# yunhao-qian/Othello-AlphaZero

Hardware: AMD Instinct MI355X
Metric: MCTS simulations/sec (whole node), 800 sims/move, 128x10b ResNet, 1/2/4/8 GPU (higher is better)
Workload: dtype bf16

## Files before the change

### include/othello_mcts_amd_experimental.h

```cpp
#ifndef OTHELLO_MCTS_AMD_EXPERIMENTAL_H
#define OTHELLO_MCTS_AMD_EXPERIMENTAL_H

#include "othello_mcts_amd.h"

#ifdef __cplusplus
extern "C" {
#endif

int oamd_engine_set_pipeline(oamd_engine *e, int32_t groups);
int oamd_engine_set_nn_chains(oamd_engine *e, int32_t chains);
int oamd_engine_set_chain_split(oamd_engine *e, int32_t budget, int32_t cuts);
int oamd_engine_set_adaptive_extra_rounds(oamd_engine *e, int32_t enable, int32_t min_rounds);
int oamd_engine_set_extra_round_grid(oamd_engine *e, int32_t workgroups);
int oamd_debug_read_stamps(uint64_t *out, int64_t n);
int oamd_debug_tree_stamps(uint64_t *out, int64_t n, int32_t reset);

int oamd_engine_set_free_running(oamd_engine *e, int32_t enable);

int oamd_engine_tree_work(oamd_engine *e, int64_t *levels, int64_t *children_scanned, int64_t *expansions,
                          int64_t *children_created, int64_t *launches);

int oamd_solve_endgames_grid(int32_t device, const oamd_position *pos_dev, int64_t n, int32_t max_empties,
                             int64_t node_limit, int32_t *move_scores_dev, int32_t *score_dev,
                             int32_t *best_action_dev, int32_t *flags_dev, int64_t *nodes_dev,
                             void *workspace_dev, int32_t workgroups, void *stream);

#ifdef __cplusplus
}
#endif

#endif
```

### othello-alphazero_amd/build.py

```python

from __future__ import annotations

import argparse
import concurrent.futures as cf
import os
import subprocess
import sys
import sysconfig
from pathlib import Path

HERE = Path(__file__).resolve().parent
CSRC = HERE / "csrc"
PKG = HERE / "othello_mcts"
INCLUDE = HERE.parent / "include"
BUILD = HERE / "build"
HIPCC = os.environ.get("HIPCC", "/opt/rocm/bin/hipcc")
ARCH = os.environ.get("OAMD_ARCH", "gfx950")

COMMON = ["-O3", "-std=c++17", "-fPIC", f"--offload-arch={ARCH}", "-I", str(CSRC), "-I", str(INCLUDE),
          "-Wall", "-Wno-unused-function", "-fno-gpu-rdc", *os.environ.get("OAMD_EXTRA_FLAGS", "").split()]
EXACT = ["-ffp-contract=off", "-fno-fast-math"]
NO_SCALAR_LOADS = ["-mllvm", "-amdgpu-scalarize-global-loads=false"]
UNITS = {
    "tree.hip": EXACT + NO_SCALAR_LOADS,
    "capi.hip": EXACT,
    "replay.hip": EXACT,
    "resnet.hip": os.environ.get("OAMD_RESNET_FLAGS",
                                 "-mllvm -amdgpu-mfma-vgpr-form=1 -mllvm -amdgpu-sched-strategy=max-ilp").split()
    + ["-Rpass-analysis=kernel-resource-usage"],
    "solver.hip": ["-Rpass-analysis=kernel-resource-usage"],
}


W8_VGPR_LIMIT = 208


def run(cmd: list[str]) -> None:
    r = subprocess.run(cmd, capture_output=True, text=True)
    if r.returncode != 0:
        sys.stderr.write(" ".join(cmd) + "\n" + r.stdout + r.stderr)
        raise SystemExit(f"build failed: {cmd[-1]}")
    if "kernel-resource-usage" in " ".join(cmd):
        unit = next((u for u in RESOURCE_CHECKS if str(CSRC / u) in cmd), None)
        if unit:
            RESOURCE_CHECKS[unit](r.stderr)
    elif r.stderr.strip():
        sys.stderr.write(r.stderr)


def kernel_remarks(remarks: str):
    name = None
    for ln in remarks.splitlines():
        if "Function Name:" in ln:
            name = ln.split("Function Name:")[1].split()[0]
        elif name and "remark:" in ln and ":" in ln.split("remark:")[1]:
            field, _, value = ln.split("remark:")[1].split("[-Rpass")[0].rpartition(":")
            yield name, field.strip(), value.strip()


def check_solver_scratch(remarks: str) -> None:
    seen = 0
    for name, field, value in kernel_remarks(remarks):
        if "k_solve" in name and "reduce" not in name and field.startswith("ScratchSize"):
            seen += 1
            if int(value.split()[0]) != 0:
                raise SystemExit(f"build failed: {name} uses {value} bytes of scratch per lane: "
                                 "the solver's stacks must stay in LDS")
    if not seen:
        raise SystemExit("build failed: no resource remark for k_solve in solver.hip")


def check_w8_vgprs(remarks: str) -> None:
    name = None
    seen = 0
    for ln in remarks.splitlines():
        if "Function Name:" in ln:
            name = ln.split("Function Name:")[1].split()[0]
        elif name and "k_resnet_w8" in name and " VGPRs:" in ln:
            v = int(ln.split("VGPRs:")[1].split()[0])
            seen += 1
            if (v + 7) // 8 * 8 > W8_VGPR_LIMIT and os.environ.get("OAMD_W8_VGPR_CHECK", "1") != "0":
                raise SystemExit(f"build failed: {name} uses {v} VGPRs (> {W8_VGPR_LIMIT}): "
                                 "k_select could no longer co-reside with the ResNet kernel")
    if not seen:
        sys.stderr.write("note: no k_resnet_w8 kernel in this build\n")


RESOURCE_CHECKS = {"resnet.hip": check_w8_vgprs, "solver.hip": check_solver_scratch}


def newer(out: Path, deps: list[Path]) -> bool:
    return out.exists() and all(out.stat().st_mtime >= d.stat().st_mtime for d in deps)


def source_hash_defines() -> list[str]:
    sys.path.insert(0, str(PKG))
    try:
        import provenance
    finally:
        sys.path.pop(0)
    return [f'-DOAMD_SOURCE_HASH_{k.upper()}="{provenance.source_hash(k)}"' for k in provenance.FAMILIES]


def build(jobs: int = 4, force: bool = False) -> None:
    BUILD.mkdir(exist_ok=True)
    headers = list(CSRC.glob("*.h")) + [INCLUDE / "othello_mcts_amd.h", INCLUDE / "othello_mcts_amd_experimental.h"]
    hashes = source_hash_defines()
    objs = []
    todo = []
    all_srcs = [CSRC / u for u in UNITS] + headers
    for unit, extra in UNITS.items():
        src = CSRC / unit
        obj = BUILD / (unit + ".o")
        objs.append(obj)
        deps = all_srcs if unit == "capi.hip" else [src, *headers]
        if force or not newer(obj, [*deps, Path(__file__)]):
            todo.append([HIPCC, *COMMON, *extra, *(hashes if unit == "capi.hip" else []), "-c", str(src),
                         "-o", str(obj)])
    with cf.ThreadPoolExecutor(max_workers=max(1, jobs)) as ex:
        list(ex.map(run, todo))
    lib = PKG / "liboamd.so"
    if force or todo or not lib.exists():
        run([HIPCC, f"--offload-arch={ARCH}", "-shared", "-fPIC", "-o", str(lib), *map(str, objs)])

    import pybind11

    ext = sysconfig.get_config_var("EXT_SUFFIX")
    mod = PKG / f"_othello_mcts_impl{ext}"
    src = CSRC / "pybind_module.cpp"
    if force or not newer(mod, [src, *headers, lib, Path(__file__)]):
        run(["g++", "-O2", "-std=c++17", "-fPIC", "-shared", "-Wall", "-fvisibility=hidden",
             "-I", pybind11.get_include(), "-I", sysconfig.get_paths()["include"], "-I", str(INCLUDE),
             str(src), "-o", str(mod), "-L", str(PKG), "-loamd", "-Wl,-rpath,$ORIGIN"])


if __name__ == "__main__":
    ap = argparse.ArgumentParser()
    ap.add_argument("-j", "--jobs", type=int, default=4)
    ap.add_argument("--force", action="store_true")
    a = ap.parse_args()
    build(a.jobs, a.force)
    print("built", *sorted(p.name for p in PKG.glob("*.so")))
```

### othello-alphazero_amd/csrc/capi.hip

```cpp

#include <hip/hip_runtime.h>

#include <algorithm>
#include <chrono>
#include <cmath>
#include <cstdio>
#include <cstdlib>
#include <cstring>
#include <string>
#include <thread>
#include <vector>

#include "../../include/othello_mcts_amd.h"
#include "../../include/othello_mcts_amd_experimental.h"
#include "bitboard.h"

#include "engine.h"
#include "kernels.h"
#include "replay.h"
#include "schedule.h"
#include "solver.h"
#include "timing.h"

using namespace oamd;
// ... 12 lines not shown
    if (spin_sync()) return hipEventSynchronize(ev);
    for (;;) {
        const hipError_t q = hipEventQuery(ev);
        if (q != hipErrorNotReady) return q;
        std::this_thread::sleep_for(std::chrono::microseconds(100));
    }
}
constexpr int kEvPerBlock = 4;
constexpr int kCounters = 12;

namespace {

thread_local std::string g_err;

int fail(int code, const std::string& msg) {
    g_err = msg;
    return code;
}

#define HIPCHK(expr)                                                                  \
    do {                                                                              \
        hipError_t _e = (expr);                                                       \
        if (_e != hipSuccess)                                                         \
            return fail(OAMD_RUNTIME, std::string(#expr) + ": " + hipGetErrorString(_e)); \
    } while (0)

#define LAUNCHCHK()                                                                       \
    do {                                                                                  \
        hipError_t _e = hipGetLastError();                                                \
        if (_e != hipSuccess) return fail(OAMD_RUNTIME, std::string("kernel launch: ") + hipGetErrorString(_e)); \
    } while (0)

struct DeviceGuard {
    int prev = -1;
    explicit DeviceGuard(int dev) {
        if (hipGetDevice(&prev) != hipSuccess) prev = -1;
        if (prev != dev) (void)hipSetDevice(dev);
    }
    ~DeviceGuard() {
        if (prev >= 0) (void)hipSetDevice(prev);
    }
};

template <typename T>
int dalloc(T** p, size_t n) {
    *p = nullptr;
    if (n == 0) return OAMD_OK;
    hipError_t e = hipMalloc(reinterpret_cast<void**>(p), n * sizeof(T));
    if (e != hipSuccess) return fail(OAMD_RUNTIME, std::string("hipMalloc: ") + hipGetErrorString(e));
    return OAMD_OK;
}

template <typename T>
void dfree(T*& p) {
    if (p) (void)hipFree(p);
    p = nullptr;
}

struct ReadbackSlots {
    static constexpr int kSlots = 4;
    int32_t* dev = nullptr;
    int32_t* host = nullptr;
    hipEvent_t ev[kSlots][kMaxPipeline] = {};
    int ensure(size_t dev_words, size_t host_words, const char* what) {
        if (dev) return OAMD_OK;
        ReadbackSlots t;
        int rc = dalloc(&t.dev, dev_words);
        if (!rc && hipHostMalloc((void**)&t.host, sizeof(int32_t) * host_words) != hipSuccess)
            rc = fail(OAMD_RUNTIME, std::string(what) + ": hipHostMalloc failed");
        for (auto& row : t.ev)
            for (auto& x : row)
                if (!rc && hipEventCreateWithFlags(&x, readback_event_flags()) != hipSuccess)
                    rc = fail(OAMD_RUNTIME, std::string(what) + ": hipEventCreate failed");
        if (rc) t.release();
        else *this = t;
        return rc;
    }
    void release() {
        for (auto& row : ev)
            for (auto x : row)
                if (x) (void)hipEventDestroy(x);
        if (host) (void)hipHostFree(host);
        dfree(dev);
    }
    void destroy() {
        if (!dev) return;
        (void)hipDeviceSynchronize();
        release();
    }
};

std::string fstr(float v) { return std::to_string(v); }

int validate_config(const oamd_search_config* c) {
    if (c->history_size < 1)
        return fail(OAMD_INVALID_ARGUMENT,
                    "Expected history_size >= 1, but got " + std::to_string(c->history_size) + ".");
    if (c->history_size > kMaxHistory)
        return fail(OAMD_INVALID_ARGUMENT, "Expected history_size <= 15 (native engine limit), but got " +
                                               std::to_string(c->history_size) + ".");
    if (c->num_simulations < 1)
        return fail(OAMD_INVALID_ARGUMENT, "Expected num_simulations >= 1, but got " +
                                               std::to_string(c->num_simulations) + ".");
    if (c->num_threads < 1)
        return fail(OAMD_INVALID_ARGUMENT,
                    "Expected num_threads >= 1, but got " + std::to_string(c->num_threads) + ".");
    if (c->batch_size < 1)
        return fail(OAMD_INVALID_ARGUMENT,
                    "Expected batch_size >= 1, but got " + std::to_string(c->batch_size) + ".");
    if ((int64_t)c->num_threads * c->batch_size > kMaxLeaves)
        return fail(OAMD_INVALID_ARGUMENT,
                    "Expected num_threads * batch_size <= 1024 (native engine limit), but got " +
                        std::to_string((int64_t)c->num_threads * c->batch_size) + ".");
    if (!(c->c_puct_base > 0.0f))
        return fail(OAMD_INVALID_ARGUMENT, "Expected c_puct_base > 0.0, but got " + fstr(c->c_puct_base) + ".");
    if (!(c->c_puct_init >= 0.0f))
        return fail(OAMD_INVALID_ARGUMENT, "Expected c_puct_init >= 0.0, but got " + fstr(c->c_puct_init) + ".");
    if (!(0.0f <= c->dirichlet_epsilon && c->dirichlet_epsilon <= 1.0f))
        return fail(OAMD_INVALID_ARGUMENT, "Expected 0.0 <= dirichlet_epsilon <= 1.0, but got " +
                                               fstr(c->dirichlet_epsilon) + ".");
    if (!(c->dirichlet_alpha >= 0.0f))
        return fail(OAMD_INVALID_ARGUMENT,
                    "Expected dirichlet_alpha >= 0.0, but got " + fstr(c->dirichlet_alpha) + ".");
    return OAMD_OK;
}

}

struct oamd_engine {
    int device = 0;
    int G = 0;
    int64_t cap = 0;
    oamd_search_config cfg{};
    hipStream_t stream = nullptr;
    uint64_t seed = 0;

    NodeLink* link = nullptr;
    NodeStat* stat = nullptr;
    NodePos* pos = nullptr;
    GameState* games = nullptr;
    int64_t rows_cap = 0;
    int fw_cap = 0;
    int32_t* leaf = nullptr;
    int32_t* depth = nullptr;
    int32_t* trans = nullptr;
    int32_t* path = nullptr;
    uint64_t* feat = nullptr;
    float* policy = nullptr;
    float* value = nullptr;
    uint8_t* flags = nullptr;
    int32_t* rowlist = nullptr;
    int32_t* rowcount = nullptr;
    int32_t* tstate = nullptr;
    float* explore_tab = nullptr;
    unsigned long long* counters = nullptr;
    int32_t* status_dev = nullptr;
    oamd_root_info* info_dev = nullptr;
    int32_t* visits_dev = nullptr;
    float* q_dev = nullptr;
    float* spd_dev = nullptr;
    int steps_left = 0;
    int steps_total = 0;
    bool exact_interleaving = true;
    int chain_budget = 2;
    int chain_cuts = 64;
    static constexpr int kCutSlots = ReadbackSlots::kSlots;
    AdaptiveRounds adapt;
    int64_t adapt_seq = 0;
    ReadbackSlots cuts;
    int cut_x[kCutSlots] = {-1, -1, -1, -1};
    int cut_groups[kCutSlots] = {};
    bool free_running = true;
    bool throttle_enqueue = !spin_sync();
    static constexpr int kFreeSlots = ReadbackSlots::kSlots;
    static constexpr int kFreeTailRounds = 4;
    ReadbackSlots remaining;
    int ensure_remaining() {
        return remaining.ensure((size_t)kMaxPipeline, (size_t)kFreeSlots * kMaxPipeline, "free-running slots");
    }
    int extra_grid = 128;
    int step_phase = 0;
    int pipeline = 0;
    int nn_batch = 0;
    int n_pipe_streams = 0;
    int n_events = 0;
    hipStream_t pipe_stream[kMaxPipeline] = {};
    hipEvent_t fork_ev = nullptr;
    static constexpr int kMaxChains = 4;
    hipEvent_t nn_token[kMaxChains] = {};
    int nn_chains = 2;
    hipStream_t idle_stream = nullptr;
    hipEvent_t sel_ev[kMaxPipeline] = {};
    hipEvent_t join_ev[kMaxPipeline] = {};
    bool timing = false;
    int timing_stride = 1;
    int64_t search_count = 0;
    std::vector<hipEvent_t> ev[2];
    int ev_blocks[2] = {0, 0};
    int ev_final[2] = {0, 0};
    int64_t ev_launches[2] = {0, 0};
    int64_t ev_rows[2] = {0, 0};
    static constexpr int64_t kSpanChunk = 1 << 15;
    static constexpr int64_t kSpanWindow = 1 << 23;
    struct SpanChunk {
        unsigned long long* p = nullptr;
        int64_t cap = 0, used = 0;
    };
    std::vector<SpanChunk> span_chunks;
    int64_t span_slots = 0;
    int64_t span_dropped = 0;
    size_t span_copied = 0;
    std::vector<std::pair<long long, long long>> span_ticks;
    int ev_cur = 0;
    float nn_ms = 0.0f;
    float select_ms = 0.0f;
    float backup_ms = 0.0f;
    int64_t nn_launches = 0;
    int64_t tree_launches = 0;
    int64_t tree_final_launches = 0;
    int64_t grouped_searches = 0, grouped_rounds = 0;
    int64_t nn_rows = 0;

    int resolve_timing(int p) {
        const int n = ev_blocks[p];
        if (!n) return OAMD_OK;
        for (int i = 0; i < n; ++i) {
            const hipEvent_t* b = &ev[p][kEvPerBlock * i];
            float ms = 0.0f;
            const bool nn = i < ev_final[p];
            HIPCHK(hipEventSynchronize(b[1]));
            if (nn) HIPCHK(hipEventSynchronize(b[3]));
            HIPCHK(hipEventElapsedTime(&ms, b[0], b[1]));
            (i < ev_final[p] ? select_ms : backup_ms) += ms;
            if (nn) {
                HIPCHK(hipEventElapsedTime(&ms, b[2], b[3]));
                nn_ms += ms;
            }
        }

        nn_launches += ev_launches[p];
        tree_launches += ev_final[p];
        tree_final_launches += n - ev_final[p];
        nn_rows += ev_rows[p];
        ev_blocks[p] = 0;
        return OAMD_OK;
    }
    int resolve_all_timing() {
        int rc = resolve_timing(ev_cur ^ 1);
        return rc ? rc : resolve_timing(ev_cur);
    }
    int reserve_spans(int64_t n, unsigned long long** out) {
        *out = nullptr;
        if (!timing || n <= 0) return OAMD_OK;
        if (span_slots + n > kSpanWindow) {
            span_dropped += n;
            return OAMD_OK;
        }
        if (span_chunks.empty() || span_chunks.back().used + n > span_chunks.back().cap) {
            SpanChunk c;
            c.cap = std::max(kSpanChunk, n);
            if (int rc = dalloc(&c.p, (size_t)2 * c.cap)) return rc;
            if (hipMemset(c.p, 0, sizeof(unsigned long long) * 2 * c.cap) != hipSuccess) {
                dfree(c.p);
                return fail(OAMD_RUNTIME, "span window: hipMemset failed");
            }
            span_chunks.push_back(c);
        }
        SpanChunk& c = span_chunks.back();
        *out = c.p + 2 * c.used;
        c.used += n;
        span_slots += n;
        return OAMD_OK;
    }
    int reset_spans() {
        if (span_chunks.empty() && !span_dropped) return OAMD_OK;
        HIPCHK(hipDeviceSynchronize());
        for (auto& c : span_chunks) dfree(c.p);
        span_chunks.clear();
        span_slots = span_dropped = 0;
        span_copied = 0;
        span_ticks.clear();
        return OAMD_OK;
    }
    int span_intervals(std::vector<std::pair<long long, long long>>* iv) {
        HIPCHK(hipDeviceSynchronize());
        auto read = [&](const SpanChunk& c, std::vector<std::pair<long long, long long>>* to) -> int {
            std::vector<unsigned long long> sp((size_t)2 * c.used);
            if (c.used)
                HIPCHK(hipMemcpy(sp.data(), c.p, sizeof(unsigned long long) * 2 * c.used, hipMemcpyDeviceToHost));
            for (int64_t i = 0; i < c.used; ++i)
                if (sp[2 * i + 1]) to->emplace_back((long long)~sp[2 * i], (long long)sp[2 * i + 1]);
            return OAMD_OK;
        };
        for (; span_copied + 1 < span_chunks.size(); ++span_copied) {
            if (int rc = read(span_chunks[span_copied], &span_ticks)) return rc;
            dfree(span_chunks[span_copied].p);
        }
        *iv = span_ticks;
        if (!span_chunks.empty())
            if (int rc = read(span_chunks.back(), iv)) return rc;
        return OAMD_OK;
    }

    int L() const { return cfg.num_threads * cfg.batch_size; }
    int steps() const { return search_steps(cfg.num_simulations, L()); }
    bool thread_split() const {
        static const bool v = [] {
            const char* e = getenv("OAMD_TREE_SPLIT");
            return e ? atoi(e) != 0 : true;
        }();
        return v && thread_split_shape(G, cfg.num_threads);
    }
    int ensure_streams(int K, int nev) {
        if (K <= 1 && nev <= 1) return OAMD_OK;
        if (!fork_ev) HIPCHK(hipEventCreateWithFlags(&fork_ev, hipEventDisableTiming));
        for (int c = 0; c < kMaxChains; ++c)
            if (!nn_token[c]) HIPCHK(hipEventCreateWithFlags(&nn_token[c], hipEventDisableTiming));
        if (!idle_stream) HIPCHK(hipStreamCreateWithFlags(&idle_stream, hipStreamNonBlocking));
        while (n_pipe_streams < K) {
            const int k = n_pipe_streams;
            HIPCHK(hipStreamCreateWithFlags(&pipe_stream[k], hipStreamNonBlocking));
            HIPCHK(hipEventCreateWithFlags(&join_ev[k], hipEventDisableTiming));
            ++n_pipe_streams;
        }
        while (n_events < nev) {
            const int k = n_events;
            HIPCHK(hipEventCreateWithFlags(&sel_ev[k], hipEventDisableTiming | hipEventDisableSystemFence));
            ++n_events;
        }
        return OAMD_OK;
    }
    int FW() const { return feature_words(cfg.history_size); }

    EngineView view() const {
        EngineView E;
        E.G = G;
        E.L = L();
        E.H = cfg.history_size;
        E.FW = FW();
        E.cap = cap;
        E.link = link;
        E.stat = stat;
        E.pos = pos;
        E.games = games;
        E.leaf = leaf;
        E.depth = depth;
        E.trans = trans;
        E.path = path;
        E.feat = feat;
        E.policy = policy;
        E.value = value;
        E.explore_tab = explore_tab;
        E.c_base = cfg.c_puct_base;
        E.c_init = cfg.c_puct_init;
        E.eps = cfg.dirichlet_epsilon;
        E.alpha = cfg.dirichlet_alpha;
        E.counters = counters;
        E.rowlist = rowlist;
        E.tstate = tstate;
        E.steps = steps();
        E.B = cfg.batch_size;
        E.terminal_skip = exact_interleaving ? 1 : 0;
        return E;
    }

    int alloc_rows() {
        const int64_t rows = (int64_t)G * L();
        const int fw = FW();
        if (rows <= rows_cap && fw <= fw_cap) return OAMD_OK;
        dfree(leaf);
        dfree(depth);
        dfree(trans);
        dfree(path);
        dfree(feat);
        dfree(policy);
        dfree(value);
        dfree(flags);
        dfree(rowlist);
        dfree(tstate);
        int rc;
        if ((rc = dalloc(&leaf, rows)) || (rc = dalloc(&depth, rows)) || (rc = dalloc(&trans, rows)) ||
            (rc = dalloc(&path, rows * kMaxDepth)) || (rc = dalloc(&feat, rows * fw)) ||
            (rc = dalloc(&policy, rows * 65)) || (rc = dalloc(&value, rows)) || (rc = dalloc(&flags, rows)) ||
            (rc = dalloc(&rowlist, rows)) || (rc = dalloc(&tstate, rows)))
            return rc;
        HIPCHK(hipMemset(policy, 0, rows * 65 * sizeof(float)));
        HIPCHK(hipMemset(value, 0, rows * sizeof(float)));
        rows_cap = rows;
        fw_cap = fw;
        return OAMD_OK;
    }

    int build_tables() {
        std::vector<float> ex(kExploreTab);
        for (int n = 0; n < kExploreTab; ++n)
            ex[n] = std::log(((float)(1 + n) + cfg.c_puct_base) / cfg.c_puct_base) + cfg.c_puct_init;
        HIPCHK(hipMemcpy(explore_tab, ex.data(), ex.size() * sizeof(float), hipMemcpyHostToDevice));
        return OAMD_OK;
    }

    ~oamd_engine() {
        DeviceGuard dg(device);
        dfree(link);
        dfree(stat);
        dfree(pos);
        dfree(games);
        dfree(leaf);
        dfree(depth);
        dfree(trans);
        dfree(path);
        dfree(feat);
        dfree(policy);
        dfree(value);
        dfree(flags);
        dfree(rowlist);
        dfree(tstate);
        dfree(rowcount);
        dfree(explore_tab);
        dfree(counters);
        dfree(status_dev);
        dfree(info_dev);
        dfree(visits_dev);
        dfree(q_dev);
        dfree(spd_dev);
        for (auto& pool : ev)
            for (auto e : pool) (void)hipEventDestroy(e);
        for (auto& c : span_chunks) dfree(c.p);
        cuts.destroy();
        remaining.destroy();
        for (int k = 0; k < n_pipe_streams; ++k) {
            (void)hipStreamDestroy(pipe_stream[k]);
            (void)hipEventDestroy(join_ev[k]);
        }
        for (int k = 0; k < n_events; ++k) (void)hipEventDestroy(sel_ev[k]);
        if (fork_ev) (void)hipEventDestroy(fork_ev);
        for (int c = 0; c < kMaxChains; ++c)
            if (nn_token[c]) (void)hipEventDestroy(nn_token[c]);
        if (idle_stream) (void)hipStreamDestroy(idle_stream);
    }
};

struct oamd_net {
    int device = 0;
    oamd_net_desc desc{};
    uint16_t* w = nullptr;
    float* bias = nullptr;
    float* head = nullptr;
    uint16_t* hconv = nullptr;
    bool loaded = false;
    std::vector<std::string> keys;
    std::vector<int64_t> numel;

    NetView view() const {
        NetView N;
        N.cin = desc.in_channels;
        N.C = desc.conv_channels;
        N.R = desc.num_residual_blocks;
        N.hidden = desc.value_head_hidden_channels;
        N.dtype = desc.dtype;
        N.w = w;
        N.bias = bias;
        N.head = head;
        N.hconv = hconv;
        return N;
    }
    ~oamd_net() {
        DeviceGuard dg(device);
        dfree(w);
        dfree(bias);
        dfree(head);
        dfree(hconv);
    }
};

extern "C" {

const char* oamd_last_error(void) { return g_err.c_str(); }
int oamd_abi_version(void) { return OAMD_ABI_VERSION; }

#ifndef OAMD_SOURCE_HASH_ALL
#define OAMD_SOURCE_HASH_ALL "unknown"
#define OAMD_SOURCE_HASH_RESNET "unknown"
#define OAMD_SOURCE_HASH_TREE "unknown"
#endif
const char* oamd_source_hash(const char* family) {
    if (!family) return nullptr;
    if (!std::strcmp(family, "all")) return OAMD_SOURCE_HASH_ALL;
    if (!std::strcmp(family, "resnet")) return OAMD_SOURCE_HASH_RESNET;
    if (!std::strcmp(family, "tree")) return OAMD_SOURCE_HASH_TREE;
    return nullptr;
}

int oamd_device_count(int32_t* out) {
    int n = 0;
    if (hipGetDeviceCount(&n) != hipSuccess) n = 0;
    *out = n;
    return OAMD_OK;
}

int oamd_get_legal_moves(const uint64_t* me, const uint64_t* opp, uint64_t* out, int64_t n, void* stream) {
    if (n < 0) return fail(OAMD_INVALID_ARGUMENT, "n must be >= 0");
    launch_legal_moves(me, opp, out, n, (hipStream_t)stream);
    LAUNCHCHK();
    return OAMD_OK;
}

int oamd_get_flips(const uint64_t* mv, const uint64_t* me, const uint64_t* opp, uint64_t* out, int64_t n,
                   void* stream) {
    if (n < 0) return fail(OAMD_INVALID_ARGUMENT, "n must be >= 0");
    launch_flips(mv, me, opp, out, n, (hipStream_t)stream);
    LAUNCHCHK();
    return OAMD_OK;
}

int oamd_apply_action(const oamd_position* in, const int32_t* actions, oamd_position* out, int64_t n,
                      void* stream) {
    static_assert(sizeof(oamd_position) == sizeof(Pos), "layout");
    if (n < 0) return fail(OAMD_INVALID_ARGUMENT, "n must be >= 0");
    launch_apply_positions(reinterpret_cast<const Pos*>(in), actions, reinterpret_cast<Pos*>(out), n,
                           (hipStream_t)stream);
    LAUNCHCHK();
    return OAMD_OK;
}

int oamd_initial_position(oamd_position* out) {
    const Pos p = initial_position();
    std::memcpy(out, &p, sizeof(Pos));
    return OAMD_OK;
}

uint64_t oamd_host_legal_moves(uint64_t me, uint64_t opp) { return legal_moves(me, opp); }
uint64_t oamd_host_flips(uint64_t mv, uint64_t me, uint64_t opp) { return flips(mv, me, opp); }
void oamd_host_apply_action(const oamd_position* in, int32_t action, oamd_position* out) {
    Pos p;
    std::memcpy(&p, in, sizeof(Pos));
    const Pos c = apply_action(p, action);
    std::memcpy(out, &c, sizeof(Pos));
}

int oamd_net_create(int32_t device, const oamd_net_desc* d, oamd_net** out) {
    *out = nullptr;
    if (d->in_channels < 1 || d->in_channels > 31)
        return fail(OAMD_INVALID_ARGUMENT, "in_channels must be in [1, 31], got " + std::to_string(d->in_channels));
    if (d->conv_channels != 128 && d->conv_channels != 256)
        return fail(OAMD_INVALID_ARGUMENT,
                    "conv_channels must be 128 or 256 for the native net, got " + std::to_string(d->conv_channels));
    if (d->num_residual_blocks < 0)
        return fail(OAMD_INVALID_ARGUMENT, "num_residual_blocks must be >= 0");
    if (d->value_head_hidden_channels < 1 || d->value_head_hidden_channels > 1024)
        return fail(OAMD_INVALID_ARGUMENT, "value_head_hidden_channels must be in [1, 1024] for the native net, got " +
                                               std::to_string(d->value_head_hidden_channels));
    if (d->num_squares != 64 || d->num_actions != 65)
        return fail(OAMD_INVALID_ARGUMENT, "num_squares must be 64 and num_actions 65");
    if (d->dtype != OAMD_BF16 && d->dtype != OAMD_FP16)
        return fail(OAMD_INVALID_ARGUMENT, "dtype must be OAMD_BF16 or OAMD_FP16");
    int n = 0;
    if (hipGetDeviceCount(&n) != hipSuccess || n == 0) return fail(OAMD_RUNTIME, "no HIP device available");
    if (device < 0 || device >= n) return fail(OAMD_INVALID_ARGUMENT, "bad device ordinal");
    DeviceGuard dg(device);
    auto* net = new oamd_net();
    net->device = device;
    net->desc = *d;
    const int C = d->conv_channels, R = d->num_residual_blocks, hid = d->value_head_hidden_channels;
    int rc;
    if ((rc = dalloc(&net->w, resnet_packed_weight_alloc_elems(C, R))) ||
        (rc = dalloc(&net->bias, (size_t)(1 + 2 * R) * C)) ||
        (rc = dalloc(&net->head, resnet_head_floats(C, hid))) ||
        (rc = dalloc(&net->hconv, resnet_hconv_elems(C)))) {
        delete net;
        return rc;
    }
    auto conv = [&](const std::string& p, int64_t cout, int64_t cin, int64_t k) {
        net->keys.push_back(p + ".weight");
        net->numel.push_back(cout * cin * k * k);
        net->keys.push_back(p + ".bias");
        net->numel.push_back(cout);
    };
    auto bn = [&](const std::string& p, int64_t c) {
        for (const char* s : {".weight", ".bias", ".running_mean", ".running_var"}) {
            net->keys.push_back(p + s);
            net->numel.push_back(c);
        }
    };
    auto lin = [&](const std::string& p, int64_t fin, int64_t fout) {
        net->keys.push_back(p + ".weight");
        net->numel.push_back(fin * fout);
        net->keys.push_back(p + ".bias");
        net->numel.push_back(fout);
    };
    conv("conv_block.conv", C, d->in_channels, 3);
    bn("conv_block.norm", C);
    for (int i = 0; i < R; ++i) {
        const std::string p = "residual_blocks." + std::to_string(i);
        conv(p + ".conv1", C, C, 3);
        bn(p + ".norm1", C);
        conv(p + ".conv2", C, C, 3);
        bn(p + ".norm2", C);
    }
    conv("policy_head.conv", 2, C, 1);
    bn("policy_head.norm", 2);
    lin("policy_head.linear", 128, 65);
    conv("value_head.conv", 1, C, 1);
    bn("value_head.norm", 1);
    lin("value_head.linear1", 64, hid);
    lin("value_head.linear2", hid, 1);
    *out = net;
    return OAMD_OK;
}

int oamd_net_destroy(oamd_net* net) {
    delete net;
    return OAMD_OK;
}

int oamd_net_state_size(const oamd_net* net, int32_t* n) {
    *n = (int32_t)net->keys.size();
    return OAMD_OK;
}

int oamd_net_state_key(const oamd_net* net, int32_t i, const char** key, int64_t* numel) {
    if (i < 0 || i >= (int32_t)net->keys.size()) return fail(OAMD_OUT_OF_RANGE, "state index out of range");
    *key = net->keys[i].c_str();
    *numel = net->numel[i];
    return OAMD_OK;
}

static uint16_t f32_to_bf16_rne(float f) {
    uint32_t u;
    std::memcpy(&u, &f, 4);
    if ((u & 0x7fffffffu) > 0x7f800000u) return (uint16_t)((u >> 16) | 0x40);
    u += 0x7fffu + ((u >> 16) & 1u);
    return (uint16_t)(u >> 16);
}

static uint16_t f32_to_f16(float f) {
    _Float16 h = (_Float16)f;
    uint16_t u;
    std::memcpy(&u, &h, 2);
    return u;
}

int oamd_net_load_state(oamd_net* net, const float* const* t, int32_t n_tensors) {
    if (n_tensors != (int32_t)net->keys.size())
        return fail(OAMD_INVALID_ARGUMENT, "expected " + std::to_string(net->keys.size()) + " tensors, got " +
                                               std::to_string(n_tensors));
    const auto& d = net->desc;
    const int C = d.conv_channels, R = d.num_residual_blocks, hid = d.value_head_hidden_channels;
    const double eps = 1e-5;
    int ti = 0;
    std::vector<uint16_t> packed(resnet_packed_weight_elems(C, R));
    std::vector<float> bias((size_t)(1 + 2 * R) * C);
    size_t ks_global = 0;
    auto pack_conv = [&](int layer, int cin, bool first) {
        const float* W = t[ti++];
        const float* b = t[ti++];
        const float* g = t[ti++];
        const float* be = t[ti++];
        const float* mu = t[ti++];
        const float* var = t[ti++];
        std::vector<double> scale(C);
        for (int n = 0; n < C; ++n) {
            scale[n] = (double)g[n] / std::sqrt((double)var[n] + eps);
            bias[(size_t)layer * C + n] = (float)(((double)b[n] - (double)mu[n]) * scale[n] + (double)be[n]);
        }
        const int nk = resnet_ksteps(C, first);
        for (int i = 0; i < nk; ++i) {
            int tap, cb;
            bool pad;
            resnet_kstep(C, first, i, &tap, &cb, &pad);
            const size_t ks = ks_global + (size_t)i;
            for (int nt = 0; nt < C / 16; ++nt)
                for (int lane = 0; lane < 64; ++lane)
                    for (int j = 0; j < 8; ++j) {
                        const int ci = cb * 32 + 8 * resnet_kgroup_chunk(lane >> 4) + j;
                        const int n = resnet_out_channel(nt, lane & 15);
                        double v = 0.0;
                        if (!pad && ci < cin) v = (double)W[((size_t)n * cin + ci) * 9 + tap] * scale[n];
                        const size_t idx = (((ks * (C / 16) + nt) * 64) + lane) * 8 + j;
                        packed[idx] = d.dtype == OAMD_BF16 ? f32_to_bf16_rne((float)v) : f32_to_f16((float)v);
                    }
        }
        ks_global += (size_t)nk;
    };
    pack_conv(0, d.in_channels, true);
    for (int i = 0; i < R; ++i) {
        pack_conv(1 + 2 * i, C, false);
        pack_conv(2 + 2 * i, C, false);
    }
    std::vector<float> head(resnet_head_floats(C, hid));
    const int HL_pcw = 0, HL_pcb = HL_pcw + 2 * C, HL_vcw = HL_pcb + 2, HL_vcb = HL_vcw + C,
// ... 235 lines not shown
    if (rows) *rows = e->nn_rows;
    return OAMD_OK;
}

int oamd_engine_nn_busy(const oamd_engine* ce, float* busy_ms, int64_t* launches) {
    oamd_engine* e = const_cast<oamd_engine*>(ce);
    DeviceGuard dg(e->device);
    if (e->span_dropped)
        return fail(OAMD_RUNTIME, "nn_busy: the timing window outgrew its " + std::to_string(oamd_engine::kSpanWindow) +
                                      " slots; " + std::to_string(e->span_dropped) +
                                      " launches were not recorded (restart it with oamd_engine_enable_timing)");
    std::vector<std::pair<long long, long long>> iv;
    if (int rc = e->span_intervals(&iv)) return rc;
    if (busy_ms) *busy_ms = (float)(interval_union(iv) * 1e-5);
    if (launches) *launches = (int64_t)iv.size();
    return OAMD_OK;
}

int oamd_engine_tree_timing(const oamd_engine* ce, float* select_ms, float* backup_ms, int64_t* launches) {
    oamd_engine* e = const_cast<oamd_engine*>(ce);
    if (int rc = e->resolve_all_timing()) return rc;
    if (select_ms) *select_ms = e->select_ms;
    if (backup_ms) *backup_ms = e->backup_ms;
    if (launches) *launches = e->tree_launches;
    return OAMD_OK;
}

struct GroupPlan : GroupSplit {
    hipStream_t st[kMaxPipeline] = {};
    int max_launches = 1;
    int64_t round_launches = 0, round_rows = 0;
};

static int native_search_checks(const oamd_engine* e, const oamd_net* net) {
    if (!net || !net->loaded) return fail(OAMD_INVALID_ARGUMENT, "native net not loaded");
    if (net->device != e->device) return fail(OAMD_INVALID_ARGUMENT, "net and engine on different devices");
    if (net->desc.in_channels != 1 + 2 * e->cfg.history_size)
        return fail(OAMD_INVALID_ARGUMENT, "net in_channels != 1 + 2 * history_size");
    return OAMD_OK;
}

static GroupPlan plan_groups(oamd_engine* e) {
    GroupPlan P;
    static_cast<GroupSplit&>(P) = split_groups(e->G, e->pipeline);
    for (int k = 0; k < P.K; ++k) {
        P.st[k] = P.K == 1 ? e->stream : e->pipe_stream[k];
        const int n = group_launches(P.ng[k], e->L(), e->nn_batch);
        P.max_launches = std::max(P.max_launches, n);
        P.round_launches += n;
        P.round_rows += (int64_t)P.ng[k] * e->L();
    }
    return P;
}

static int extra_rounds(const oamd_engine* e) {
    return extra_round_cap(e->exact_interleaving, e->chain_budget, e->chain_cuts, e->cfg.num_threads, e->steps());
}

static int pick_extra_rounds(oamd_engine* e, int* X) {
    const int cap = extra_rounds(e);
    *X = cap;
    if (cap == 0 || !e->adapt.on) return OAMD_OK;
    if (int rc = e->cuts.ensure((size_t)2 * oamd_engine::kCutSlots * kMaxPipeline,
                                (size_t)2 * oamd_engine::kCutSlots * kMaxPipeline, "cut slots"))
        return rc;
    const int64_t q = e->adapt_seq - 2;
    const int s = q >= 0 ? (int)(q % oamd_engine::kCutSlots) : 0;
    if (q >= 0 && e->cut_x[s] >= 0) {
        int used = 0, empties = 64;
        for (int k = 0; k < e->cut_groups[s]; ++k) {
            HIPCHK(host_wait(e->cuts.ev[s][k]));
            used = std::max(used, (int)e->cuts.host[2 * (s * kMaxPipeline + k)]);
            empties = std::min(empties, (int)e->cuts.host[2 * (s * kMaxPipeline + k) + 1]);
        }
        e->adapt.observe(e->cut_x[s], used, empties, e->chain_cuts);
        static const bool plog = getenv("OAMD_ADAPT_LOG") != nullptr;
        if (plog)
            fprintf(stderr, "adapt search %lld X %d used %d empties %d\n", (long long)q, e->cut_x[s], used, empties);
        e->cut_x[s] = -1;
    }
    *X = e->adapt.pick(cap);
    return OAMD_OK;
}

static int timing_begin(oamd_engine* e, int steps, int NB, bool* timed) {
    *timed = e->timing && (e->search_count++ % e->timing_stride) == 0;
    if (!*timed) return OAMD_OK;
    const int pool = e->ev_cur;
    if (int rc = e->resolve_timing(pool)) return rc;

    while ((int)e->ev[pool].size() < kEvPerBlock * (steps + 1) * NB) {
        hipEvent_t x;
        HIPCHK(hipEventCreate(&x));
        e->ev[pool].push_back(x);
    }
    return OAMD_OK;
}

static void timing_end(oamd_engine* e, int blocks, int first_final, int NB, int64_t round_launches,
                       int64_t round_rows) {
    const int pool = e->ev_cur;
    e->ev_blocks[pool] = blocks;
    e->ev_final[pool] = first_final;
    e->ev_launches[pool] = first_final / NB * round_launches;
    e->ev_rows[pool] = first_final / NB * round_rows;
    e->ev_cur ^= 1;
}
static void timing_end_search(oamd_engine* e, int rounds, const GroupPlan& P) {
    timing_end(e, (rounds + 1) * P.K, rounds * P.K, P.K, P.round_launches, P.round_rows);
}

static int enqueue_group_nn(oamd_engine* e, const EngineView& E, const NetView& N, const GroupPlan& P, int k,
                            bool wait_token, hipEvent_t* ev, int* count, unsigned long long* span, int max_wgs) {
    hipStream_t sk = P.st[k];
    hipEvent_t token = e->nn_token[k % std::min(e->nn_chains, P.K)];
    if (P.K > 1 && wait_token) HIPCHK(hipStreamWaitEvent(sk, token, 0));
    if (ev) HIPCHK(hipEventRecord(ev[2], sk));
    const int grows = P.ng[k] * E.L, cb = launch_rows(grows, e->nn_batch);
    const size_t r0 = (size_t)P.g0[k] * E.L;
    for (int r = 0, j = 0; r < grows; r += cb, ++j)
        launch_resnet_packed(N, E.feat, E.FW, E.H, std::min(cb, grows - r), E.policy, E.value, sk, E.rowlist + r0 + r,
                             count, r, span ? span + (size_t)2 * j : nullptr, max_wgs);
    if (ev) HIPCHK(hipEventRecord(ev[3], sk));
    if (P.K > 1) HIPCHK(hipEventRecord(token, sk));
    return OAMD_OK;
}

static int enqueue_group_rounds(oamd_engine* e, const NetView& N, const GroupPlan& P, int steps, int X, bool timed,
                                bool chained) {
    const EngineView E = e->view();
    const int K = P.K;
    const int T = e->cfg.num_threads, B = e->cfg.batch_size;
    const int pool = e->ev_cur;
    const bool splitting = extra_rounds(e) > 0;
    const int budget = splitting ? e->chain_budget : 0;
    const int S = steps + X;
    const bool adapt = splitting && e->adapt.on;
    const int cs = (int)(e->adapt_seq % oamd_engine::kCutSlots);
    ++e->grouped_searches;
    e->grouped_rounds += S;
    if (adapt) {
        e->cut_x[cs] = X;
        e->cut_groups[cs] = K;
        ++e->adapt_seq;
    }
    const int nlg = P.max_launches;
    unsigned long long* span = nullptr;
    if (int rc = e->reserve_spans((int64_t)K * S * nlg, &span)) return rc;
    for (int s = 0; s <= S; ++s) {
        for (int k = 0; k < K; ++k) {
            hipStream_t sk = P.st[k];
            hipEvent_t* ev = timed ? &e->ev[pool][kEvPerBlock * (s * K + k)] : nullptr;
            if (ev) HIPCHK(hipEventRecord(ev[0], sk));
            int* cnt = e->rowcount + 2 * k;
            int* cuts = adapt ? e->cuts.dev + 2 * (cs * kMaxPipeline + k) : nullptr;
            launch_tree(E, sk, s > 0, s < S, T, B, P.g0[k], P.ng[k], 0, -1, s < S ? cnt + (s & 1) : nullptr,
                        s < S ? cnt + ((s + 1) & 1) : cnt, s == 0, budget, X, timed,
                        s == 0 || s == S ? cuts : nullptr);
            if (ev) HIPCHK(hipEventRecord(ev[1], sk));
            if (s == S) {
                if (adapt) {
                    HIPCHK(hipMemcpyAsync(e->cuts.host + 2 * (cs * kMaxPipeline + k), cuts, 2 * sizeof(int32_t),
                                          hipMemcpyDeviceToHost, sk));
                    HIPCHK(hipEventRecord(e->cuts.ev[cs][k], sk));
                }
                continue;
            }
            const bool first = s == 0 && k < std::min(e->nn_chains, K) && !chained;
            if (int rc = enqueue_group_nn(e, E, N, P, k, !first, ev, cnt + (s & 1),
                                          span ? span + (size_t)2 * ((k * S + s) * nlg) : nullptr,
                                          s >= steps ? e->extra_grid : 0))
                return rc;
        }
    }
    return OAMD_OK;
}

static int fork_streams(oamd_engine* e, const hipStream_t* st, int n) {
    if (n > 1) {
        HIPCHK(hipEventRecord(e->fork_ev, e->stream));
        for (int k = 0; k < n; ++k) HIPCHK(hipStreamWaitEvent(st[k], e->fork_ev, 0));
    }
    return OAMD_OK;
}
static int join_streams(oamd_engine* e, const hipStream_t* st, int n) {
    for (int k = 0; n > 1 && k < n; ++k) {
        HIPCHK(hipEventRecord(e->join_ev[k], st[k]));
        HIPCHK(hipStreamWaitEvent(e->stream, e->join_ev[k], 0));
    }
    return OAMD_OK;
}
static int fork_groups(oamd_engine* e, const GroupPlan& P) { return fork_streams(e, P.st, P.K); }
static int join_groups(oamd_engine* e, const GroupPlan& P) { return join_streams(e, P.st, P.K); }

static int search_thread_split(oamd_engine* e, const NetView& N) {
    const EngineView E = e->view();
    const int steps = e->steps();
    const int T = e->cfg.num_threads, B = e->cfg.batch_size;
    if (int rc = e->ensure_streams(T, T)) return rc;
    bool timed = false;
    if (int rc = timing_begin(e, steps, T, &timed)) return rc;
    const int pool = e->ev_cur;
    unsigned long long* span = nullptr;
    if (int rc = e->reserve_spans((int64_t)T * steps, &span)) return rc;
    if (int rc = fork_streams(e, e->pipe_stream, T)) return rc;
    for (int s = 0; s <= steps; ++s) {
        for (int t = 0; t < T; ++t) {
            hipEvent_t* ev = timed ? &e->ev[pool][kEvPerBlock * (s * T + t)] : nullptr;
            hipStream_t ts = e->pipe_stream[t];
            if (s > 0 || t > 0)
                HIPCHK(hipStreamWaitEvent(ts, e->sel_ev[t > 0 ? t - 1 : T - 1], 0));
            if (ev) HIPCHK(hipEventRecord(ev[0], ts));
            launch_tree(E, ts, s > 0, s < steps, T, B, 0, 1, t, t + 1, nullptr, nullptr, s == 0, 0, 0, timed);
            if (ev) HIPCHK(hipEventRecord(ev[1], ts));
            HIPCHK(hipEventRecord(e->sel_ev[t], ts));
            if (s == steps) continue;
            if (ev) HIPCHK(hipEventRecord(ev[2], ts));
            launch_resnet_packed(N, E.feat + (size_t)t * B * E.FW, E.FW, E.H, B, E.policy + (size_t)t * B * 65,
                                 E.value + (size_t)t * B, ts, nullptr, nullptr, 0,
                                 span ? span + (size_t)2 * (t * steps + s) : nullptr);
            if (ev) HIPCHK(hipEventRecord(ev[3], ts));
        }
    }
    if (int rc = join_streams(e, e->pipe_stream, T)) return rc;
    LAUNCHCHK();
    if (timed) timing_end(e, (steps + 1) * T, steps * T, T, T, e->L());
    return OAMD_OK;
}

static int search_grouped(oamd_engine* e, const NetView& N) {
    const int K = plan_groups(e).K;
    if (int rc = e->ensure_streams(K, K)) return rc;
    const GroupPlan P = plan_groups(e);
    bool timed = false;
    int X = 0;
    if (int rc = pick_extra_rounds(e, &X)) return rc;
    const int steps = e->steps();
    if (int rc = timing_begin(e, steps + X, K, &timed)) return rc;
    if (int rc = fork_groups(e, P)) return rc;
    if (int rc = enqueue_group_rounds(e, N, P, steps, X, timed, false)) return rc;
    LAUNCHCHK();
    if (int rc = join_groups(e, P)) return rc;
    if (timed) timing_end_search(e, steps + X, P);
    return OAMD_OK;
}

int oamd_engine_search(oamd_engine* e, oamd_net* net, int64_t* sims, int64_t* evals) {
    if (int rc = native_search_checks(e, net)) return rc;
    DeviceGuard dg(e->device);
    if (sims || evals) HIPCHK(hipMemsetAsync(e->counters, 0, 2 * sizeof(unsigned long long), e->stream));
    const NetView N = net->view();
    if (int rc = e->thread_split() ? search_thread_split(e, N) : search_grouped(e, N)) return rc;
    if (sims || evals) {
        unsigned long long c[2] = {0, 0};
        HIPCHK(hipMemcpyAsync(c, e->counters, sizeof(c), hipMemcpyDeviceToHost, e->stream));
        HIPCHK(hipStreamSynchronize(e->stream));
        if (sims) *sims = (int64_t)c[0];
        if (evals) *evals = (int64_t)c[1];
    }
    e->step_phase = 0;
    e->steps_left = 0;
    return OAMD_OK;
}

int oamd_engine_work_counters(oamd_engine* e, int64_t* sims, int64_t* evals) {
    DeviceGuard dg(e->device);
    unsigned long long c[2] = {0, 0};
    HIPCHK(hipMemcpyAsync(c, e->counters + 2, sizeof(c), hipMemcpyDeviceToHost, e->stream));
    HIPCHK(hipStreamSynchronize(e->stream));
    if (sims) *sims = (int64_t)c[0];
    if (evals) *evals = (int64_t)c[1];
    return OAMD_OK;
}

int oamd_engine_descent_depths(oamd_engine* e, int64_t* leaves, int64_t* depth_sum, int32_t* depth_max) {
    DeviceGuard dg(e->device);
    unsigned long long c[kCounters] = {};
    HIPCHK(hipMemcpyAsync(c, e->counters, sizeof(c), hipMemcpyDeviceToHost, e->stream));
    HIPCHK(hipStreamSynchronize(e->stream));
    if (leaves) *leaves = (int64_t)c[2];
    if (depth_sum) *depth_sum = (int64_t)c[6];
    if (depth_max) *depth_max = (int32_t)c[7];
    return OAMD_OK;
}

int oamd_engine_tree_work(oamd_engine* e, int64_t* levels, int64_t* scanned, int64_t* expansions, int64_t* created,
                          int64_t* launches) {
    DeviceGuard dg(e->device);
    unsigned long long c[kCounters] = {};
    HIPCHK(hipMemcpyAsync(c, e->counters, sizeof(c), hipMemcpyDeviceToHost, e->stream));
    HIPCHK(hipStreamSynchronize(e->stream));
    if (levels) *levels = (int64_t)c[6];
    if (scanned) *scanned = (int64_t)c[8];
    if (expansions) *expansions = (int64_t)c[9];
    if (created) *created = (int64_t)c[10];
    if (launches) *launches = (int64_t)c[11];
    return OAMD_OK;
}

int oamd_engine_set_pipeline(oamd_engine* e, int32_t groups) {
    if (groups < 0 || groups > kMaxPipeline)
        return fail(OAMD_INVALID_ARGUMENT, "pipeline groups must be in [0, " + std::to_string(kMaxPipeline) + "]");
    e->pipeline = groups;
    return OAMD_OK;
}

int oamd_debug_read_stamps(uint64_t* out, int64_t n) {
    if (!out || n < 0) return fail(OAMD_INVALID_ARGUMENT, "stamps: bad buffer");
    const int rc = resnet_read_stamps(reinterpret_cast<unsigned long long*>(out), (long long)n);
    if (rc == -2) return fail(OAMD_INVALID_ARGUMENT, "built without OAMD_STAMPS");
    return rc ? fail(OAMD_RUNTIME, "stamp copy failed") : OAMD_OK;
}

int oamd_debug_tree_stamps(uint64_t* out, int64_t n, int32_t reset) {
    if (!out || n < 0) return fail(OAMD_INVALID_ARGUMENT, "tree stamps: bad buffer");
    const int rc = tree_read_stamps(reinterpret_cast<unsigned long long*>(out), (long long)n, reset);
    if (rc == -2) return fail(OAMD_INVALID_ARGUMENT, "built without OAMD_TREE_STAMPS");
    return rc ? fail(OAMD_RUNTIME, "tree stamp copy failed") : OAMD_OK;
}

int oamd_engine_set_nn_chains(oamd_engine* e, int32_t chains) {
    if (chains < 1 || chains > oamd_engine::kMaxChains)
        return fail(OAMD_INVALID_ARGUMENT, "nn chains must be in [1, " + std::to_string(oamd_engine::kMaxChains) + "]");
    e->nn_chains = chains;
    return OAMD_OK;
}

int oamd_engine_set_chain_split(oamd_engine* e, int32_t budget, int32_t cuts) {
    if (budget < 0 || cuts < 0 || cuts > 64) return fail(OAMD_INVALID_ARGUMENT, "chain split: budget >= 0, cuts in [0, 64]");
    e->chain_budget = budget;
    e->chain_cuts = cuts;
    return OAMD_OK;
}

int oamd_engine_set_adaptive_extra_rounds(oamd_engine* e, int32_t enable, int32_t min_rounds) {
    if (min_rounds < 0 || min_rounds > 64) return fail(OAMD_INVALID_ARGUMENT, "adaptive extra rounds: min in [0, 64]");
    e->adapt.reset(enable != 0, min_rounds);
    for (int& x : e->cut_x) x = -1;
    return OAMD_OK;
}

int oamd_engine_round_counts(const oamd_engine* ce, int64_t* searches, int64_t* rounds, int64_t* final_launches) {
    oamd_engine* e = const_cast<oamd_engine*>(ce);
    if (int rc = e->resolve_all_timing()) return rc;
    if (searches) *searches = e->grouped_searches;
    if (rounds) *rounds = e->grouped_rounds;
    if (final_launches) *final_launches = e->tree_final_launches;
    return OAMD_OK;
}

int oamd_engine_set_extra_round_grid(oamd_engine* e, int32_t workgroups) {
    if (workgroups < 0) return fail(OAMD_INVALID_ARGUMENT, "extra-round grid must be >= 0");
    e->extra_grid = workgroups;
    return OAMD_OK;
}

int oamd_engine_set_exact_interleaving(oamd_engine* e, int32_t enable) {
    e->exact_interleaving = enable != 0;
    return OAMD_OK;
}

int oamd_engine_set_nn_batch(oamd_engine* e, int32_t rows) {
    if (rows < 0) return fail(OAMD_INVALID_ARGUMENT, "nn batch rows must be >= 0");
    e->nn_batch = rows;
    return OAMD_OK;
}

int oamd_engine_root_info(oamd_engine* e, int32_t game, oamd_root_info* info, int32_t* visits, float* q) {
    if (game < 0 || game >= e->G) return fail(OAMD_OUT_OF_RANGE, "game index out of range");
    DeviceGuard dg(e->device);
    launch_root_stats(e->view(), game, 1, e->info_dev, e->visits_dev, e->q_dev, 0, e->stream);
    LAUNCHCHK();
    oamd_root_info tmp;
    HIPCHK(hipMemcpyAsync(&tmp, e->info_dev, sizeof(tmp), hipMemcpyDeviceToHost, e->stream));
    int32_t v[65];
    float qq[65];
    HIPCHK(hipMemcpyAsync(v, e->visits_dev, sizeof(v), hipMemcpyDeviceToHost, e->stream));
    HIPCHK(hipMemcpyAsync(qq, e->q_dev, sizeof(qq), hipMemcpyDeviceToHost, e->stream));
    HIPCHK(hipStreamSynchronize(e->stream));
    if (info) *info = tmp;
    const int nc = tmp.num_children;
    if (visits) std::memcpy(visits, v, sizeof(int32_t) * nc);
    if (q) std::memcpy(q, qq, sizeof(float) * nc);
    return OAMD_OK;
}

int oamd_engine_status(oamd_engine* e, int32_t* overflow_games, int32_t* depth_capped_games) {
    DeviceGuard dg(e->device);
    HIPCHK(hipMemsetAsync(e->status_dev, 0, 2 * sizeof(int32_t), e->stream));
    launch_status(e->view(), e->status_dev, e->stream);
    LAUNCHCHK();
    int32_t h[2] = {0, 0};
    HIPCHK(hipMemcpyAsync(h, e->status_dev, sizeof(h), hipMemcpyDeviceToHost, e->stream));
    HIPCHK(hipStreamSynchronize(e->stream));
    if (overflow_games) *overflow_games = h[0];
    if (depth_capped_games) *depth_capped_games = h[1];
    return OAMD_OK;
}

int oamd_engine_root_stats(oamd_engine* e, int32_t* visits_dev, float* q_dev, oamd_root_info* info_dev) {
    DeviceGuard dg(e->device);
    launch_root_stats(e->view(), 0, e->G, info_dev ? info_dev : e->info_dev, visits_dev ? visits_dev : e->visits_dev,
                      q_dev ? q_dev : e->q_dev, 1, e->stream);
    LAUNCHCHK();
    return OAMD_OK;
}

int oamd_engine_self_play_data(oamd_engine* e, int32_t game, float* features, float* policy) {
    oamd_root_info info;
    int rc = oamd_engine_root_info(e, game, &info, nullptr, nullptr);
    if (rc) return rc;
    if (info.position.player == 0)
        return fail(OAMD_INVALID_ARGUMENT, "Self-play data cannot be generated from a terminal position.");
    if (info.num_children == 0) return fail(OAMD_INVALID_ARGUMENT, "The root node has not been expanded yet.");
    DeviceGuard dg(e->device);
    const int C = 1 + 2 * e->cfg.history_size;
    float* fd = e->spd_dev;
    float* pd = e->spd_dev + (size_t)8 * C * 64;
    launch_self_play_data(e->view(), game, fd, pd, e->stream);
    LAUNCHCHK();
    HIPCHK(hipMemcpyAsync(features, fd, sizeof(float) * 8 * C * 64, hipMemcpyDeviceToHost, e->stream));
    HIPCHK(hipMemcpyAsync(policy, pd, sizeof(float) * 8 * 65, hipMemcpyDeviceToHost, e->stream));
    HIPCHK(hipStreamSynchronize(e->stream));
    return OAMD_OK;
}

int oamd_engine_apply_action(oamd_engine* e, int32_t game, int32_t action) {
    if (game < 0 || game >= e->G) return fail(OAMD_OUT_OF_RANGE, "game index out of range");
    if (!(0 <= action && action < 65))
        return fail(OAMD_OUT_OF_RANGE, "Expected 0 <= action < 65, but got " + std::to_string(action) + ".");
    oamd_root_info info;
    int rc = oamd_engine_root_info(e, game, &info, nullptr, nullptr);
    if (rc) return rc;
    if (action == 64) {
        if (info.position.player == 0)
            return fail(OAMD_INVALID_ARGUMENT, "Pass is not allowed in a terminal position.");
        if (info.position.legal_moves != 0)
            return fail(OAMD_INVALID_ARGUMENT, "Pass is not allowed when there are legal moves.");
    } else if (((1ULL << (63 - action)) & info.position.legal_moves) == 0) {
        return fail(OAMD_INVALID_ARGUMENT, std::to_string(action) + " is not a legal action.");
    }
    if (info.node_count + 1 > e->cap) return fail(OAMD_CAPACITY, "node pool exhausted");
    DeviceGuard dg(e->device);
    launch_apply_one(e->view(), game, action, e->stream);
    LAUNCHCHK();
    return OAMD_OK;
}

int oamd_engine_apply_actions(oamd_engine* e, const int32_t* actions_dev) {
    DeviceGuard dg(e->device);
    launch_apply_actions(e->view(), actions_dev, e->stream);
    LAUNCHCHK();
    return OAMD_OK;
}

static bool move_cfg_ok(const oamd_selfplay_config* cfg) {
    return cfg->temperature_moves >= 0 && cfg->temperature > 0.0f;
}

static int selfplay_cfg_checks(const oamd_selfplay_config* cfg, const float* features_dev, const float* policy_dev) {
    if (!move_cfg_ok(cfg) || cfg->opening_moves < 0) return fail(OAMD_INVALID_ARGUMENT, "bad self-play config");
    if (cfg->emit_targets && (!features_dev || !policy_dev))
        return fail(OAMD_INVALID_ARGUMENT, "emit_targets needs features and policy buffers");
    return OAMD_OK;
}

static SelfplayParams selfplay_params(const oamd_selfplay_config* cfg) {
    return SelfplayParams{cfg->temperature_moves, cfg->temperature, cfg->opening_moves, cfg->emit_targets};
}

int oamd_engine_selfplay_move(oamd_engine* e, const oamd_selfplay_config* cfg, int32_t* actions_dev,
                              int32_t* finished_dev, float* features_dev, float* policy_dev) {
    if (int rc = selfplay_cfg_checks(cfg, features_dev, policy_dev)) return rc;
    DeviceGuard dg(e->device);
    launch_selfplay_move(e->view(), selfplay_params(cfg), 0, e->G, actions_dev, finished_dev, features_dev, policy_dev,
                         e->stream);
    LAUNCHCHK();
    return OAMD_OK;
}

static int selfplay_steps_free(oamd_engine* e, oamd_net* net, const oamd_selfplay_config* cfg, int n_moves,
                               int per_move, int32_t* actions, int32_t* finished, float* feat, float* pol) {
    if (int rc = e->ensure_remaining()) return rc;
    const GroupPlan P = plan_groups(e);
    const int K = P.K;
    const int T = e->cfg.num_threads, B = e->cfg.batch_size;
    const int steps = e->steps();
    const EngineView E = e->view();
    const NetView N = net->view();
    const SelfplayParams sp = selfplay_params(cfg);
    const int budget = e->exact_interleaving && e->chain_budget > 0 ? e->chain_budget : 0;
    const int nlg = P.max_launches;
    if (int rc = fork_groups(e, P)) return rc;
    int64_t round = 0;
    auto rounds = [&]() -> int {
        for (int k = 0; k < K; ++k) {
            HIPCHK(hipMemsetAsync(e->rowcount + 2 * k, 0, 2 * sizeof(int32_t), P.st[k]));
            HIPCHK(hipMemsetAsync(e->remaining.dev + k, 0, sizeof(int32_t), P.st[k]));
            launch_free_begin(E, P.g0[k], P.ng[k], n_moves, e->remaining.dev + k, actions, finished, per_move, P.st[k]);
        }
        bool gdone[kMaxPipeline] = {};
        const int64_t base_rounds = n_moves > 0 ? (int64_t)n_moves * steps + 1 : 0;
        const int64_t max_rounds = base_rounds + (int64_t)n_moves * ((int64_t)T * steps + 2) + 4 * oamd_engine::kFreeTailRounds;
        for (int64_t chunk = 0; n_moves > 0; ++chunk) {
            int R;
            const bool tail = round >= base_rounds;
            if (!tail) {
                R = (int)std::min<int64_t>(round == 0 ? steps + 1 : steps, base_rounds - round);
                if (chunk >= 2 && e->throttle_enqueue) {
                    const int slot = (int)((chunk - 2) % oamd_engine::kFreeSlots);
                    for (int k = 0; k < K; ++k) HIPCHK(host_wait(e->remaining.ev[slot][k]));
                }
            } else {
                if (chunk >= 2) {
                    const int slot = (int)((chunk - 2) % oamd_engine::kFreeSlots);
                    for (int k = 0; k < K; ++k) {
                        if (gdone[k]) continue;
                        HIPCHK(host_wait(e->remaining.ev[slot][k]));
                        if (e->remaining.host[slot * kMaxPipeline + k] == 0) gdone[k] = true;
                    }
                }
                bool all = true;
                for (int k = 0; k < K; ++k) all = all && gdone[k];
                if (all) break;
                if (round >= max_rounds) return fail(OAMD_RUNTIME, "free-running self-play did not finish");
                R = oamd_engine::kFreeTailRounds;
            }
            bool timed = false;
            if (!tail) {
                if (int rc = timing_begin(e, R, K, &timed)) return rc;
            }
            const int pool = e->ev_cur;
            unsigned long long* span = nullptr;
            if (int rc = e->reserve_spans((int64_t)K * R * nlg, &span)) return rc;
            for (int s = 0; s < R; ++s) {
                const int64_t r = round + s;
                for (int k = 0; k < K; ++k) {
                    if (gdone[k]) continue;
                    hipStream_t sk = P.st[k];
                    hipEvent_t* ev = timed ? &e->ev[pool][kEvPerBlock * (s * K + k)] : nullptr;
                    int* cnt = e->rowcount + 2 * k;
                    if (ev) HIPCHK(hipEventRecord(ev[0], sk));
                    launch_tree_free(E, sk, P.g0[k], P.ng[k], B, cnt + (r & 1), cnt + ((r + 1) & 1), budget, timed, sp,
                                     n_moves, per_move, actions, finished, feat, pol, e->remaining.dev + k);
                    if (ev) HIPCHK(hipEventRecord(ev[1], sk));
                    const bool first = r == 0 && k < std::min(e->nn_chains, K);
                    if (int rc = enqueue_group_nn(e, E, N, P, k, !first, ev, cnt + (r & 1),
                                                  span ? span + (size_t)2 * ((k * R + s) * nlg) : nullptr,
                                                  tail ? e->extra_grid : 0))
                        return rc;
                }
            }
            const int slot = (int)(chunk % oamd_engine::kFreeSlots);
            for (int k = 0; k < K; ++k) {
                if (gdone[k]) continue;
                HIPCHK(hipMemcpyAsync(e->remaining.host + slot * kMaxPipeline + k, e->remaining.dev + k, sizeof(int32_t),
                                      hipMemcpyDeviceToHost, P.st[k]));
                HIPCHK(hipEventRecord(e->remaining.ev[slot][k], P.st[k]));
            }
            if (timed) timing_end(e, R * K, R * K, K, P.round_launches, P.round_rows);
            round += R;
        }
        for (int k = 0; k < K; ++k) HIPCHK(hipMemsetAsync(e->rowcount + 2 * k, 0, 2 * sizeof(int32_t), P.st[k]));
        LAUNCHCHK();
        return OAMD_OK;
    };
    const int rc = rounds();
    const int jrc = join_groups(e, P);
    e->step_phase = 0;
    e->steps_left = 0;
    if (rc) return rc;
    e->grouped_searches += n_moves;
    e->grouped_rounds += round;
    return jrc;
}

int oamd_engine_set_free_running(oamd_engine* e, int32_t enable) {
    e->free_running = enable != 0;
    return OAMD_OK;
}

int oamd_engine_selfplay_steps(oamd_engine* e, oamd_net* net, const oamd_selfplay_config* cfg, int32_t n_moves,
                               int32_t per_move_outputs, int32_t* actions_dev, int32_t* finished_dev,
                               float* features_dev, float* policy_dev) {
    if (n_moves < 0) return fail(OAMD_INVALID_ARGUMENT, "n_moves must be >= 0");
    if (int rc = selfplay_cfg_checks(cfg, features_dev, policy_dev)) return rc;
    if (int rc = native_search_checks(e, net)) return rc;
    DeviceGuard dg(e->device);
    const int G = e->G, C = 1 + 2 * e->cfg.history_size;
    auto out = [&](int i, auto* p, int64_t per_game) { return p ? p + (per_move_outputs ? (int64_t)i * G * per_game : 0) : p; };
    GroupPlan P = plan_groups(e);
    const bool split = e->thread_split();
    if (!split && e->free_running) {
        if (int rc = e->ensure_streams(P.K, P.K)) return rc;
        return selfplay_steps_free(e, net, cfg, n_moves, per_move_outputs, actions_dev, finished_dev, features_dev,
                                   policy_dev);
    }
    if (split || P.K == 1) {
        for (int i = 0; i < n_moves; ++i) {
            if (int rc = oamd_engine_search(e, net, nullptr, nullptr)) return rc;
            if (int rc = oamd_engine_selfplay_move(e, cfg, out(i, actions_dev, 1), out(i, finished_dev, 1),
                                                   out(i, features_dev, 8 * C * 64), out(i, policy_dev, 8 * 65)))
                return rc;
        }
        return OAMD_OK;
    }
// ... 323 lines not shown
```

### othello-alphazero_amd/csrc/kernels.h

```cpp
#pragma once

#include <hip/hip_runtime.h>
#include <stdint.h>

#include "../../include/othello_mcts_amd.h"
#include "bitboard.h"
#include "engine.h"

namespace oamd {

struct SelfplayParams {
    int32_t temperature_moves;
    float temperature;
    int32_t opening_moves;
    int32_t emit_targets;
};

void launch_tree(const EngineView& E, hipStream_t s, bool do_backup, bool do_select, int T, int B,
                 int g0 = 0, int ng = -1, int t0 = 0, int t1 = -1, int* cnt_add = nullptr,
                 int* cnt_reset = nullptr, bool fresh = false, int budget = 0, int max_cuts = 0,
                 bool timed = false, int* cuts_out = nullptr);
void launch_features_f32(const EngineView& E, float* out, int row_begin, int rows, hipStream_t s);
void launch_set_evaluation(const EngineView& E, const float* pol, const float* val, int row_begin,
                           int rows, hipStream_t s);
void launch_leaf_flags(const EngineView& E, uint8_t* flags, hipStream_t s);
void launch_reset(const EngineView& E, int game, uint64_t seed, hipStream_t s);
void launch_apply_actions(const EngineView& E, const int32_t* actions, hipStream_t s);
void launch_apply_one(const EngineView& E, int g, int action, hipStream_t s);
void launch_root_stats(const EngineView& E, int game_begin, int n_games, oamd_root_info* info,
                       int32_t* visits, float* q, int by_action, hipStream_t s);
void launch_self_play_data(const EngineView& E, int g, float* feat, float* pol, hipStream_t s);
void launch_selfplay_move(const EngineView& E, const SelfplayParams& sp, int g0, int ng, int32_t* actions,
                          int32_t* finished, float* feat, float* pol, hipStream_t s);
void launch_random_openings(const EngineView& E, int max_moves, uint64_t seed, hipStream_t s);
void launch_set_active(const EngineView& E, const uint8_t* active, hipStream_t s);
void launch_arena_begin(const EngineView& EA, const EngineView& EB, uint64_t seed_a, uint64_t seed_b,
                        const int32_t* openings, int plies, const uint8_t* a_is_white, hipStream_t s);
void launch_arena_count(const EngineView& EA, int32_t* remaining, hipStream_t s);
void launch_arena_move(const EngineView& EA, const EngineView& EB, const SelfplayParams& sp, int32_t* actions,
                       int32_t* finished, int32_t* discs, int32_t* remaining, hipStream_t s);
void launch_free_begin(const EngineView& E, int g0, int ng, int n_moves, int32_t* remaining, int32_t* actions,
                       int32_t* finished, int per_move, hipStream_t s);
void launch_tree_free(const EngineView& E, hipStream_t s, int g0, int ng, int B, int* cnt_add, int* cnt_reset,
                      int budget, bool timed, const SelfplayParams& sp, int n_moves, int per_move, int32_t* actions,
                      int32_t* finished, float* feat, float* pol, int32_t* remaining);
void launch_status(const EngineView& E, int32_t* out, hipStream_t s);
void launch_legal_moves(const uint64_t* me, const uint64_t* opp, uint64_t* out, int64_t n,
                        hipStream_t s);
void launch_flips(const uint64_t* mv, const uint64_t* me, const uint64_t* opp, uint64_t* out,
                  int64_t n, hipStream_t s);
void launch_apply_positions(const Pos* in, const int32_t* actions, Pos* out, int64_t n,
                            hipStream_t s);

struct NetView {
    int32_t cin;
    int32_t C;
    int32_t R;
    int32_t hidden;
    int32_t dtype;
    const uint16_t* w;
    const float* bias;
    const float* head;
    const uint16_t* hconv;
};

void launch_resnet_packed(const NetView& N, const uint64_t* feat, int fw, int H, int rows,
                          float* policy, float* value, hipStream_t s, const int32_t* rowlist = nullptr,
                          const int32_t* rowcount = nullptr, int list_off = 0,
                          unsigned long long* span = nullptr, int max_wgs = 0);
void launch_resnet_f32(const NetView& N, const float* feat, int rows, float* policy, float* value,
                       hipStream_t s);
size_t resnet_packed_weight_elems(int C, int R);
size_t resnet_packed_weight_alloc_elems(int C, int R);
size_t resnet_head_floats(int C, int hidden);
inline size_t resnet_hconv_elems(int C) { return (size_t)(C / 32) * 64 * 8; }
int resnet_read_stamps(unsigned long long* out, long long n);
int tree_read_stamps(unsigned long long* out, long long n, int reset);
int resnet_ksteps(int C, bool first);
void resnet_kstep(int C, bool first, int i, int* tap, int* cb, bool* pad);
int resnet_kgroup_chunk(int kg);
int resnet_out_channel(int tile, int row);

}
```

### othello-alphazero_amd/csrc/pybind_module.cpp

```cpp

#include <pybind11/numpy.h>
#include <pybind11/pybind11.h>
#include <pybind11/stl.h>

#include <bitset>
#include <cstdio>
#include <cstring>
#include <memory>
#include <cstdint>
#include <stdexcept>
#include <string>
#include <vector>

#include "othello_mcts_amd.h"
#include "othello_mcts_amd_experimental.h"

namespace py = pybind11;
using namespace py::literals;

namespace {

void check(int rc) {
    if (rc == OAMD_OK) return;
    const std::string msg = oamd_last_error();
// ... 82 lines not shown
    }
};

struct Net {
    oamd_net* h = nullptr;
    oamd_net_desc desc{};
    Net(int device, int in_channels, int conv_channels, int num_residual_blocks, int hidden, int dtype) {
        desc = oamd_net_desc{in_channels, conv_channels, num_residual_blocks, hidden, 64, 65, dtype};
        check(oamd_net_create(device, &desc, &h));
    }
    ~Net() {
        if (h) oamd_net_destroy(h);
    }
    std::vector<std::pair<std::string, int64_t>> state_keys() const {
        int32_t n = 0;
        check(oamd_net_state_size(h, &n));
        std::vector<std::pair<std::string, int64_t>> out;
        for (int i = 0; i < n; ++i) {
            const char* k = nullptr;
            int64_t numel = 0;
            check(oamd_net_state_key(h, i, &k, &numel));
            out.emplace_back(k, numel);
        }
        return out;
    }
    void load_state(const std::vector<py::array_t<float, py::array::c_style | py::array::forcecast>>& ts) {
        std::vector<const float*> ptrs;
        ptrs.reserve(ts.size());
        for (auto& t : ts) ptrs.push_back(t.data());
        check(oamd_net_load_state(h, ptrs.data(), (int32_t)ptrs.size()));
    }
    void forward(uintptr_t feat, int rows, uintptr_t pol, uintptr_t val, uintptr_t stream) {
        check(oamd_net_forward(h, reinterpret_cast<const float*>(feat), rows, reinterpret_cast<float*>(pol),
                               reinterpret_cast<float*>(val), reinterpret_cast<void*>(stream)));
    }
    uintptr_t handle() const { return reinterpret_cast<uintptr_t>(h); }
};

struct Engine {
    oamd_engine* h = nullptr;
    int device = 0;
    Engine(int device_, int num_games, int64_t node_capacity, const oamd_search_config& cfg, uint64_t seed)
        : device(device_) {
        check(oamd_engine_create(device, num_games, node_capacity, &cfg, seed, &h));
    }
    ~Engine() {
        if (h) oamd_engine_destroy(h);
    }
    oamd_search_config config() const {
        oamd_search_config c;
        check(oamd_engine_get_config(h, &c));
        return c;
    }
    void set_config(const oamd_search_config& c) { check(oamd_engine_set_config(h, &c)); }
    void check_health() const {
        int32_t over = 0, capped = 0;
        check(oamd_engine_status(h, &over, &capped));
        if (over)
            throw std::runtime_error("node pool exhausted in " + std::to_string(over) +
                                     " game(s): leaves could not be expanded, so the search no longer "
                                     "matches the reference; create the engine with a larger node_capacity");
        if (capped)
            throw std::runtime_error("search path exceeded the depth cap (127 plies below the root) in " +
                                     std::to_string(capped) + " game(s)");
    }
};

oamd_search_config make_config(int history_size, int num_simulations, int num_threads, int batch_size,
                               float c_puct_base, float c_puct_init, float eps, float alpha) {
    return oamd_search_config{history_size, num_simulations, num_threads, batch_size,
                              c_puct_base, c_puct_init, eps, alpha};
}

struct Torch {
    py::module_ torch = py::module_::import("torch");
    py::module_ native = py::module_::import("othello_mcts.native");
    uintptr_t current_stream(int device) {
        return torch.attr("cuda").attr("current_stream")(device).attr("cuda_stream").cast<uintptr_t>();
    }
    static uintptr_t ptr(const py::object& t) { return t.attr("data_ptr")().cast<uintptr_t>(); }
};

int device_count() {
    int32_t n = 0;
    oamd_device_count(&n);
    return n;
}

int engine_device_for(const std::string& torch_device) {
    if (device_count() == 0)
        throw std::runtime_error(
            "othello_mcts (MI355X-native) needs a ROCm GPU: no HIP device is visible. "
            "The search tree and kernels run on the GPU; there is no CPU fallback.");
    if (torch_device.rfind("cuda:", 0) == 0) return std::stoi(torch_device.substr(5));
    py::module_ torch = py::module_::import("torch");
    return torch.attr("cuda").attr("current_device")().cast<int>();
}

class MCTS {
public:
    MCTS(int history_size, std::string torch_device, bool torch_pin_memory, int num_simulations, int num_threads,
         int batch_size, float c_puct_base, float c_puct_init, float dirichlet_epsilon, float dirichlet_alpha,
         int64_t node_capacity, uint64_t seed, bool native_nn, const std::string& nn_dtype)
        : torch_device_(std::move(torch_device)), pin_(torch_pin_memory), native_(native_nn) {
        set_nn_dtype(nn_dtype);
        const oamd_search_config c = make_config(history_size, num_simulations, num_threads, batch_size,
                                                 c_puct_base, c_puct_init, dirichlet_epsilon, dirichlet_alpha);
        device_ = engine_device_for(torch_device_);
        if (seed == 0) {
            py::module_ os = py::module_::import("os");
            py::bytes b = os.attr("urandom")(8);
            std::string s = b;
            std::memcpy(&seed, s.data(), 8);
        }
        if (node_capacity == 0) node_capacity = kSingleGameNodes;
        engine_ = std::make_unique<Engine>(device_, 1, node_capacity, c, seed);
    }
    static constexpr int64_t kSingleGameNodes = (int64_t)1 << 23;

    void reset_position() {
        check(oamd_engine_reset(engine_->h, 0, next_seed()));
        sync();
    }

    Position position() {
        oamd_root_info info;
        check(oamd_engine_root_info(engine_->h, 0, &info, nullptr, nullptr));
        Position p;
        p.p = info.position;
        return p;
    }

    void search(py::object neural_net) {
        Torch T;
        const uintptr_t stream = T.current_stream(device_);
        check(oamd_engine_set_stream(engine_->h, reinterpret_cast<void*>(stream)));
        const oamd_search_config c = engine_->config();
        if (native_) {
            py::object nat = T.native.attr("resolve")(neural_net, device_, c.history_size, nn_dtype_);
            if (!nat.is_none()) {
                auto* net = reinterpret_cast<oamd_net*>(nat.attr("handle").cast<uintptr_t>());
                check(oamd_engine_search(engine_->h, net, nullptr, nullptr));
                engine_->check_health();
                return;
            }
        }
        const int B = c.batch_size, L = c.num_threads * c.batch_size, C = 1 + 2 * c.history_size;
        py::object dev = T.torch.attr("device")("cuda", device_);
        py::object f32 = T.torch.attr("float32");
        py::tuple shape = py::make_tuple(B, C, 8, 8);
        py::object feat_gpu = T.torch.attr("empty")(shape, "dtype"_a = f32, "device"_a = dev);
        const bool on_gpu = torch_device_.rfind("cuda", 0) == 0;
        py::object feat_arg = feat_gpu;
        if (!on_gpu) {
            feat_arg = T.torch.attr("empty")(shape, "dtype"_a = f32, "device"_a = torch_device_,
                                             "pin_memory"_a = pin_);
        }
        int32_t steps = 0;
        check(oamd_engine_search_begin(engine_->h, &steps));
        std::vector<uint8_t> flags(L);
        for (int s = 0; s < steps; ++s) {
            check(oamd_engine_select(engine_->h));
            check(oamd_engine_leaf_flags(engine_->h, flags.data()));
            for (int k = 0; k < c.num_threads; ++k) {
                bool any = false;
                for (int j = 0; j < B; ++j) any |= flags[k * B + j] != 0;
                if (!any) continue;
                check(oamd_engine_features(engine_->h, reinterpret_cast<float*>(T.ptr(feat_gpu)), k * B, B));
                if (!on_gpu) feat_arg.attr("copy_")(feat_gpu);
                py::object out = neural_net(feat_arg);
                py::object pol = out["policy"].attr("detach")().attr("to")("device"_a = dev, "dtype"_a = f32)
                                     .attr("contiguous")();
                py::object val = out["value"].attr("detach")().attr("to")("device"_a = dev, "dtype"_a = f32)
                                     .attr("contiguous")();
                check(oamd_engine_set_evaluation(engine_->h, reinterpret_cast<const float*>(T.ptr(pol)),
                                                 reinterpret_cast<const float*>(T.ptr(val)), k * B, B));
            }
        }
        check(oamd_engine_backup(engine_->h));
        sync();
        engine_->check_health();
    }

    std::vector<int> visit_counts() {
        oamd_root_info info;
        int32_t v[65];
        float q[65];
        check(oamd_engine_root_info(engine_->h, 0, &info, v, q));
        return std::vector<int>(v, v + info.num_children);
    }
    std::vector<float> mean_action_values() {
        oamd_root_info info;
        int32_t v[65];
        float q[65];
        check(oamd_engine_root_info(engine_->h, 0, &info, v, q));
        return std::vector<float>(q, q + info.num_children);
    }
    py::dict self_play_data() {
        const int C = 1 + 2 * engine_->config().history_size;
        py::array_t<float> f({8, C, 8, 8});
        py::array_t<float> p({8, 65});
        check(oamd_engine_self_play_data(engine_->h, 0, f.mutable_data(), p.mutable_data()));
        py::module_ torch = py::module_::import("torch");
        py::object ft = torch.attr("from_numpy")(f);
        py::object pt = torch.attr("from_numpy")(p);
        py::list fl, pl;
        for (int t = 0; t < 8; ++t) {
            fl.append(ft[py::int_(t)].attr("clone")());
            pl.append(pt[py::int_(t)].attr("clone")());
        }
        return py::dict("features"_a = fl, "policy"_a = pl);
    }
    void apply_action(int action) {
        check(oamd_engine_apply_action(engine_->h, 0, action));
        sync();
    }

    int history_size() const { return engine_->config().history_size; }
    void set_history_size(int v) { update([&](oamd_search_config& c) { c.history_size = v; }); }
    std::string torch_device() const { return torch_device_; }
    void set_torch_device(const std::string& v) {
        const int d = engine_device_for(v);
        if (d != device_)
            throw py::value_error("the native engine keeps its search tree on cuda:" + std::to_string(device_) +
                                  "; create a new MCTS to move it to another GPU");
        torch_device_ = v;
    }
    bool torch_pin_memory() const { return pin_; }
    void set_torch_pin_memory(bool v) { pin_ = v; }
    int num_simulations() const { return engine_->config().num_simulations; }
    void set_num_simulations(int v) { update([&](oamd_search_config& c) { c.num_simulations = v; }); }
    int num_threads() const { return engine_->config().num_threads; }
    void set_num_threads(int v) { update([&](oamd_search_config& c) { c.num_threads = v; }); }
    int batch_size() const { return engine_->config().batch_size; }
    void set_batch_size(int v) { update([&](oamd_search_config& c) { c.batch_size = v; }); }
    float c_puct_base() const { return engine_->config().c_puct_base; }
    void set_c_puct_base(float v) { update([&](oamd_search_config& c) { c.c_puct_base = v; }); }
    float c_puct_init() const { return engine_->config().c_puct_init; }
    void set_c_puct_init(float v) { update([&](oamd_search_config& c) { c.c_puct_init = v; }); }
    float dirichlet_epsilon() const { return engine_->config().dirichlet_epsilon; }
    void set_dirichlet_epsilon(float v) { update([&](oamd_search_config& c) { c.dirichlet_epsilon = v; }); }
    float dirichlet_alpha() const { return engine_->config().dirichlet_alpha; }
    void set_dirichlet_alpha(float v) { update([&](oamd_search_config& c) { c.dirichlet_alpha = v; }); }

    bool native_nn() const { return native_; }
    void set_native_nn(bool v) { native_ = v; }
    std::string nn_dtype() const { return nn_dtype_; }
    void set_nn_dtype(const std::string& v) {
        if (v != "bf16" && v != "fp16")
            throw std::invalid_argument("Expected nn_dtype in {'bf16', 'fp16'}, but got '" + v + "'.");
        nn_dtype_ = v;
    }
    int device() const { return device_; }
    uint64_t game_key() {
        uint64_t k = 0;
        check(oamd_engine_game_key(engine_->h, 0, &k));
        return k;
    }
    void reset_seed(uint64_t seed) {
        check(oamd_engine_reset(engine_->h, 0, seed));
        sync();
    }
    py::dict root_info() {
        oamd_root_info info;
        check(oamd_engine_root_info(engine_->h, 0, &info, nullptr, nullptr));
        return py::dict("visit_count"_a = info.visit_count, "num_children"_a = info.num_children,
                        "node_count"_a = info.node_count, "overflow"_a = info.overflow);
    }

private:
    template <typename F>
    void update(F f) {
        oamd_search_config c = engine_->config();
        f(c);
        engine_->set_config(c);
    }
    void sync() {
    }
    uint64_t next_seed() {
        py::module_ os = py::module_::import("os");
        std::string s = py::bytes(os.attr("urandom")(8));
        uint64_t v;
        std::memcpy(&v, s.data(), 8);
        return v;
    }

    std::string torch_device_;
    bool pin_;
    bool native_ = true;
    std::string nn_dtype_ = "fp16";
    int device_ = 0;
    std::unique_ptr<Engine> engine_;
};

}

PYBIND11_MODULE(_othello_mcts_impl, m) {
    m.doc() = "MI355X-native othello_mcts (HIP kernels behind a C ABI)";

    m.def("get_legal_moves", &oamd_host_legal_moves, "player_discs"_a, "opponent_discs"_a);
    m.def("get_flips", &oamd_host_flips, "move_mask"_a, "player_discs"_a, "opponent_discs"_a);
    m.def("device_count", &device_count);
    m.def("abi_version", &oamd_abi_version);
    m.def("source_hash", [](const std::string& family) {
        const char* h = oamd_source_hash(family.c_str());
        if (!h) throw py::value_error("unknown source family: " + family);
        return std::string(h);
    });

    py::class_<Position>(m, "Position")
        .def_static("initial_position", &Position::initial_position)
        .def("player", &Position::player)
        .def("player1_discs", &Position::player1_discs)
        .def("player2_discs", &Position::player2_discs)
        .def("__getitem__", &Position::at)
        .def("legal_moves", &Position::legal_moves)
        .def("is_legal_move", &Position::is_legal_move)
        .def("legal_actions", &Position::legal_actions)
        .def("apply_move", &Position::apply_move)
        .def("apply_pass", &Position::apply_pass)
        .def("apply_action", &Position::apply_action)
        .def("is_terminal", &Position::is_terminal)
        .def("__str__", &Position::to_string)
        .def("next_legal_moves", [](const Position& p) { return p.p.next_legal_moves; })
        .def("__eq__", [](const Position& a, const Position& b) {
            return a.p.player == b.p.player && a.p.player1_discs == b.p.player1_discs &&
                   a.p.player2_discs == b.p.player2_discs && a.p.legal_moves == b.p.legal_moves &&
                   a.p.next_legal_moves == b.p.next_legal_moves;
        })
        .def("__repr__", [](const Position& p) {
            char buf[128];
            std::snprintf(buf, sizeof(buf), "Position(player=%d, player1_discs=0x%016llx, player2_discs=0x%016llx)",
                          p.p.player, (unsigned long long)p.p.player1_discs,
                          (unsigned long long)p.p.player2_discs);
            return std::string(buf);
        });

    py::class_<MCTS>(m, "MCTS")
        .def(py::init<int, std::string, bool, int, int, int, float, float, float, float, int64_t, uint64_t, bool,
                      const std::string&>(),
             "history_size"_a = 4, "torch_device"_a = "cpu", "torch_pin_memory"_a = false,
             "num_simulations"_a = 800, "num_threads"_a = 2, "batch_size"_a = 16, "c_puct_base"_a = 20000.0f,
             "c_puct_init"_a = 2.5f, "dirichlet_epsilon"_a = 0.25f, "dirichlet_alpha"_a = 0.5f,
             "node_capacity"_a = 0, "seed"_a = 0, "native_nn"_a = true, "nn_dtype"_a = "fp16")
        .def("reset_position", &MCTS::reset_position)
        .def("position", &MCTS::position)
        .def("search", &MCTS::search)
        .def("visit_counts", &MCTS::visit_counts)
        .def("mean_action_values", &MCTS::mean_action_values)
        .def("self_play_data", &MCTS::self_play_data)
        .def("apply_action", &MCTS::apply_action)
        .def("history_size", &MCTS::history_size)
        .def("set_history_size", &MCTS::set_history_size)
        .def("torch_device", &MCTS::torch_device)
        .def("set_torch_device", &MCTS::set_torch_device)
        .def("torch_pin_memory", &MCTS::torch_pin_memory)
        .def("set_torch_pin_memory", &MCTS::set_torch_pin_memory)
        .def("num_simulations", &MCTS::num_simulations)
        .def("set_num_simulations", &MCTS::set_num_simulations)
        .def("num_threads", &MCTS::num_threads)
        .def("set_num_threads", &MCTS::set_num_threads)
        .def("batch_size", &MCTS::batch_size)
        .def("set_batch_size", &MCTS::set_batch_size)
        .def("c_puct_base", &MCTS::c_puct_base)
        .def("set_c_puct_base", &MCTS::set_c_puct_base)
        .def("c_puct_init", &MCTS::c_puct_init)
        .def("set_c_puct_init", &MCTS::set_c_puct_init)
        .def("dirichlet_epsilon", &MCTS::dirichlet_epsilon)
        .def("set_dirichlet_epsilon", &MCTS::set_dirichlet_epsilon)
        .def("dirichlet_alpha", &MCTS::dirichlet_alpha)
        .def("set_dirichlet_alpha", &MCTS::set_dirichlet_alpha)
        .def("native_nn", &MCTS::native_nn)
        .def("set_native_nn", &MCTS::set_native_nn)
        .def("nn_dtype", &MCTS::nn_dtype)
        .def("set_nn_dtype", &MCTS::set_nn_dtype)
        .def("device", &MCTS::device)
        .def("game_key", &MCTS::game_key)
        .def("reset_seed", &MCTS::reset_seed)
        .def("root_info", &MCTS::root_info);

    py::class_<oamd_search_config>(m, "SearchConfig")
        .def(py::init(&make_config), "history_size"_a = 8, "num_simulations"_a = 800, "num_threads"_a = 2,
             "batch_size"_a = 16, "c_puct_base"_a = 20000.0f, "c_puct_init"_a = 2.5f, "dirichlet_epsilon"_a = 0.25f,
             "dirichlet_alpha"_a = 0.5f)
        .def_readwrite("history_size", &oamd_search_config::history_size)
        .def_readwrite("num_simulations", &oamd_search_config::num_simulations)
        .def_readwrite("num_threads", &oamd_search_config::num_threads)
        .def_readwrite("batch_size", &oamd_search_config::batch_size)
        .def_readwrite("c_puct_base", &oamd_search_config::c_puct_base)
        .def_readwrite("c_puct_init", &oamd_search_config::c_puct_init)
        .def_readwrite("dirichlet_epsilon", &oamd_search_config::dirichlet_epsilon)
        .def_readwrite("dirichlet_alpha", &oamd_search_config::dirichlet_alpha);

    py::class_<Net>(m, "_Net")
        .def(py::init<int, int, int, int, int, int>(), "device"_a, "in_channels"_a, "conv_channels"_a,
             "num_residual_blocks"_a, "value_head_hidden_channels"_a, "dtype"_a = 0)
        .def("state_keys", &Net::state_keys)
        .def("load_state", &Net::load_state)
        .def("forward", &Net::forward, "features"_a, "rows"_a, "policy"_a, "value"_a, "stream"_a = 0)
        .def_property_readonly("handle", &Net::handle);

    py::class_<Engine>(m, "_Engine")
        .def(py::init<int, int, int64_t, const oamd_search_config&, uint64_t>(), "device"_a, "num_games"_a,
             "node_capacity"_a, "config"_a, "seed"_a)
        .def_readonly("device", &Engine::device)
        .def("config", &Engine::config)
        .def("set_config", &Engine::set_config)
        .def("num_games", [](Engine& e) {
            int32_t n;
            check(oamd_engine_num_games(e.h, &n));
            return n;
        })
        .def("set_stream", [](Engine& e, uintptr_t s) { check(oamd_engine_set_stream(e.h, (void*)s)); })
        .def("reset", [](Engine& e, int game, uint64_t seed) { check(oamd_engine_reset(e.h, game, seed)); })
        .def(
            "search",
            [](Engine& e, uintptr_t net, bool sync) -> py::object {
                if (!sync) {
                    check(oamd_engine_search(e.h, reinterpret_cast<oamd_net*>(net), nullptr, nullptr));
                    return py::none();
                }
                int64_t sims = 0, evals = 0;
                check(oamd_engine_search(e.h, reinterpret_cast<oamd_net*>(net), &sims, &evals));
                return py::make_tuple(sims, evals);
            },
            py::arg("net"), py::arg("sync") = true)
        .def("search_begin",
             [](Engine& e) {
                 int32_t steps = 0;
                 check(oamd_engine_search_begin(e.h, &steps));
                 return steps;
             })
        .def("select", [](Engine& e) { check(oamd_engine_select(e.h)); })
        .def("leaf_flags",
             [](Engine& e) {
                 const oamd_search_config c = e.config();
                 int32_t G;
                 check(oamd_engine_num_games(e.h, &G));
                 py::array_t<uint8_t> a((py::ssize_t)G * c.num_threads * c.batch_size);
                 check(oamd_engine_leaf_flags(e.h, a.mutable_data()));
                 return a;
             })
        .def("features",
             [](Engine& e, uintptr_t out, int row_begin, int rows) {
                 check(oamd_engine_features(e.h, reinterpret_cast<float*>(out), row_begin, rows));
             })
        .def("set_evaluation",
             [](Engine& e, uintptr_t pol, uintptr_t val, int row_begin, int rows) {
                 check(oamd_engine_set_evaluation(e.h, reinterpret_cast<const float*>(pol),
                                                  reinterpret_cast<const float*>(val), row_begin, rows));
             })
        .def("backup", [](Engine& e) { check(oamd_engine_backup(e.h)); })
        .def("status",
             [](Engine& e) {
                 int32_t over = 0, capped = 0;
                 check(oamd_engine_status(e.h, &over, &capped));
                 return py::make_tuple(over, capped);
             })
        .def("check_health", [](Engine& e) { e.check_health(); })
        .def("root_info",
             [](Engine& e, int game) {
                 oamd_root_info info;
                 int32_t v[65];
                 float q[65];
                 check(oamd_engine_root_info(e.h, game, &info, v, q));
                 const int nc = info.num_children;
                 return py::dict("player"_a = info.position.player, "player1_discs"_a = info.position.player1_discs,
                                 "player2_discs"_a = info.position.player2_discs,
                                 "legal_moves"_a = info.position.legal_moves,
                                 "next_legal_moves"_a = info.position.next_legal_moves,
                                 "num_children"_a = nc, "visit_count"_a = info.visit_count,
                                 "overflow"_a = info.overflow, "node_count"_a = info.node_count,
                                 "visit_counts"_a = std::vector<int>(v, v + nc),
                                 "mean_action_values"_a = std::vector<float>(q, q + nc));
             })
        .def("root_stats",
             [](Engine& e, uintptr_t visits, uintptr_t q, uintptr_t info) {
                 check(oamd_engine_root_stats(e.h, reinterpret_cast<int32_t*>(visits), reinterpret_cast<float*>(q),
                                              reinterpret_cast<oamd_root_info*>(info)));
             })
        .def("self_play_data",
             [](Engine& e, int game) {
                 const int C = 1 + 2 * e.config().history_size;
                 py::array_t<float> f({8, C, 8, 8});
                 py::array_t<float> p({8, 65});
                 check(oamd_engine_self_play_data(e.h, game, f.mutable_data(), p.mutable_data()));
                 return py::make_tuple(f, p);
             })
        .def("apply_action", [](Engine& e, int game, int action) { check(oamd_engine_apply_action(e.h, game, action)); })
        .def("apply_actions",
             [](Engine& e, uintptr_t actions) {
                 check(oamd_engine_apply_actions(e.h, reinterpret_cast<const int32_t*>(actions)));
             })
        .def("selfplay_move",
             [](Engine& e, int temperature_moves, float temperature, int opening_moves, bool emit, uintptr_t actions,
                uintptr_t finished, uintptr_t feat, uintptr_t pol) {
                 oamd_selfplay_config c{temperature_moves, temperature, opening_moves, emit ? 1 : 0};
                 check(oamd_engine_selfplay_move(e.h, &c, reinterpret_cast<int32_t*>(actions),
                                                 reinterpret_cast<int32_t*>(finished), reinterpret_cast<float*>(feat),
                                                 reinterpret_cast<float*>(pol)));
             })
        .def("selfplay_steps",
             [](Engine& e, uintptr_t net, int n_moves, int temperature_moves, float temperature, int opening_moves,
                bool emit, bool per_move_outputs, uintptr_t actions, uintptr_t finished, uintptr_t feat, uintptr_t pol) {
                 oamd_selfplay_config c{temperature_moves, temperature, opening_moves, emit ? 1 : 0};
                 check(oamd_engine_selfplay_steps(e.h, reinterpret_cast<oamd_net*>(net), &c, n_moves,
                                                  per_move_outputs ? 1 : 0, reinterpret_cast<int32_t*>(actions),
                                                  reinterpret_cast<int32_t*>(finished), reinterpret_cast<float*>(feat),
                                                  reinterpret_cast<float*>(pol)));
             })
        .def("random_openings",
             [](Engine& e, int max_moves, uint64_t seed) { check(oamd_engine_random_openings(e.h, max_moves, seed)); })
        .def("game_key",
             [](Engine& e, int game) {
                 uint64_t k;
                 check(oamd_engine_game_key(e.h, game, &k));
                 return k;
             })
        .def("set_active",
             [](Engine& e, uintptr_t active) {
                 check(oamd_engine_set_active(e.h, reinterpret_cast<const uint8_t*>(active)));
             })
        .def("arena_begin",
             [](Engine& a, Engine& b, uintptr_t openings, int opening_plies, uintptr_t a_is_white) {
                 check(oamd_arena_begin(a.h, b.h, reinterpret_cast<const int32_t*>(openings), opening_plies,
                                        reinterpret_cast<const uint8_t*>(a_is_white)));
             })
        .def("arena_move",
             [](Engine& a, Engine& b, int temperature_moves, float temperature, uintptr_t actions, uintptr_t finished,
                uintptr_t discs, uintptr_t remaining) {
                 oamd_selfplay_config c{temperature_moves, temperature, 0, 0};
                 check(oamd_arena_move(a.h, b.h, &c, reinterpret_cast<int32_t*>(actions),
                                       reinterpret_cast<int32_t*>(finished), reinterpret_cast<int32_t*>(discs),
                                       reinterpret_cast<int32_t*>(remaining)));
             })
        .def("arena_play",
             [](Engine& a, uintptr_t net_a, Engine& b, uintptr_t net_b, int temperature_moves, float temperature,
                int max_plies, uintptr_t actions, uintptr_t finished, uintptr_t discs) {
                 oamd_selfplay_config c{temperature_moves, temperature, 0, 0};
                 int32_t plies = 0;
                 check(oamd_arena_play(a.h, reinterpret_cast<oamd_net*>(net_a), b.h, reinterpret_cast<oamd_net*>(net_b),
                                       &c, max_plies, reinterpret_cast<int32_t*>(actions),
                                       reinterpret_cast<int32_t*>(finished), reinterpret_cast<int32_t*>(discs), &plies));
                 return plies;
             })
        .def("enable_timing", [](Engine& e, int every) { check(oamd_engine_enable_timing(e.h, every)); },
             py::arg("every") = 1)
        .def("set_pipeline", [](Engine& e, int groups) { check(oamd_engine_set_pipeline(e.h, groups)); })
        .def("set_nn_batch", [](Engine& e, int rows) { check(oamd_engine_set_nn_batch(e.h, rows)); })
        .def("set_nn_chains", [](Engine& e, int chains) { check(oamd_engine_set_nn_chains(e.h, chains)); })
        .def("set_extra_round_grid",
             [](Engine& e, int workgroups) { check(oamd_engine_set_extra_round_grid(e.h, workgroups)); })
        .def("set_chain_split",
             [](Engine& e, int budget, int cuts) { check(oamd_engine_set_chain_split(e.h, budget, cuts)); })
        .def("set_adaptive_extra_rounds",
             [](Engine& e, bool enable, int min_rounds) {
                 check(oamd_engine_set_adaptive_extra_rounds(e.h, enable ? 1 : 0, min_rounds));
             },
             py::arg("enable") = true, py::arg("min_rounds") = 1)
        .def("round_counts", [](Engine& e) {
            int64_t searches = 0, rounds = 0, finals = 0;
            check(oamd_engine_round_counts(e.h, &searches, &rounds, &finals));
            return py::make_tuple(searches, rounds, finals);
        })
        .def("set_free_running",
             [](Engine& e, bool enable) { check(oamd_engine_set_free_running(e.h, enable ? 1 : 0)); })
        .def("set_exact_interleaving",
             [](Engine& e, bool enable) { check(oamd_engine_set_exact_interleaving(e.h, enable ? 1 : 0)); })
        .def("nn_timing", [](Engine& e) {
            float ms;
            int64_t launches, rows;
            check(oamd_engine_nn_timing(e.h, &ms, &launches, &rows));
            return py::make_tuple(ms, launches, rows);
        })
        .def("nn_busy", [](Engine& e) {
            float ms = 0.0f;
            int64_t launches = 0;
            check(oamd_engine_nn_busy(e.h, &ms, &launches));
            return py::make_tuple(ms, launches);
        })
        .def("work_counters", [](Engine& e) {
            int64_t sims = 0, evals = 0;
            check(oamd_engine_work_counters(e.h, &sims, &evals));
            return py::make_tuple(sims, evals);
        })
        .def("descent_depths", [](Engine& e) {
            int64_t leaves = 0, dsum = 0;
            int32_t dmax = 0;
            check(oamd_engine_descent_depths(e.h, &leaves, &dsum, &dmax));
            return py::make_tuple(leaves, dsum, dmax);
        })
        .def("tree_timing", [](Engine& e) {
            float sel, bk;
            int64_t launches;
            check(oamd_engine_tree_timing(e.h, &sel, &bk, &launches));
            return py::make_tuple(sel, bk, launches);
        })
        .def("tree_work", [](Engine& e) {
            int64_t lv = 0, sc = 0, ex = 0, cr = 0, la = 0;
            check(oamd_engine_tree_work(e.h, &lv, &sc, &ex, &cr, &la));
            return py::make_tuple(lv, sc, ex, cr, la);
        });

    py::class_<oamd_replay_view>(m, "_ReplayView")
        .def(py::init([](int device, int num_games, int history_size, int max_moves, int64_t capacity,
                         uintptr_t boards, uintptr_t policy, uintptr_t value, uintptr_t player,
                         uintptr_t stage_boards, uintptr_t stage_policy, uintptr_t stage_player, uintptr_t moves,
                         uintptr_t pending, uintptr_t counters) {
                 return oamd_replay_view{device, num_games, history_size, max_moves, capacity,
                                         reinterpret_cast<uint64_t*>(boards), reinterpret_cast<float*>(policy),
                                         reinterpret_cast<float*>(value), reinterpret_cast<uint8_t*>(player),
                                         reinterpret_cast<uint64_t*>(stage_boards),
                                         reinterpret_cast<float*>(stage_policy),
                                         reinterpret_cast<uint8_t*>(stage_player), reinterpret_cast<int32_t*>(moves),
                                         reinterpret_cast<int32_t*>(pending), reinterpret_cast<int64_t*>(counters)};
             }),
             "device"_a, "num_games"_a, "history_size"_a, "max_moves"_a, "capacity"_a, "boards"_a, "policy"_a,
             "value"_a, "player"_a, "stage_boards"_a, "stage_policy"_a, "stage_player"_a, "moves"_a, "pending"_a,
             "counters"_a)
        .def("add",
             [](const oamd_replay_view& v, int n_moves, uintptr_t actions, uintptr_t finished, uintptr_t feat,
                uintptr_t pol, uintptr_t stream) {
                 check(oamd_replay_add(&v, n_moves, reinterpret_cast<const int32_t*>(actions),
                                       reinterpret_cast<const int32_t*>(finished), reinterpret_cast<const float*>(feat),
                                       reinterpret_cast<const float*>(pol), reinterpret_cast<void*>(stream)));
             })
        .def("add_tracked",
             [](const oamd_replay_view& v, uintptr_t exact, int n_moves, uintptr_t actions, uintptr_t finished,
                uintptr_t feat, uintptr_t pol, uintptr_t stream) {
                 check(oamd_replay_add_tracked(&v, reinterpret_cast<int8_t*>(exact), n_moves,
                                               reinterpret_cast<const int32_t*>(actions),
                                               reinterpret_cast<const int32_t*>(finished),
                                               reinterpret_cast<const float*>(feat),
                                               reinterpret_cast<const float*>(pol), reinterpret_cast<void*>(stream)));
             })
        .def("relabel",
             [](const oamd_replay_view& v, uintptr_t exact, uintptr_t relabel_counters, int max_empties,
                int64_t budget, int64_t node_limit, int policy_mode, bool retry, uintptr_t workspace,
                uintptr_t stream) {
                 check(oamd_replay_relabel_endgames(&v, reinterpret_cast<int8_t*>(exact),
                                                    reinterpret_cast<int64_t*>(relabel_counters), max_empties, budget,
                                                    node_limit, policy_mode, retry ? 1 : 0,
                                                    reinterpret_cast<void*>(workspace),
                                                    reinterpret_cast<void*>(stream)));
             })
        .def("gather",
             [](const oamd_replay_view& v, uintptr_t ids, int64_t n, uintptr_t feat, uintptr_t pol, uintptr_t val,
                uintptr_t stream) {
                 check(oamd_replay_gather(&v, reinterpret_cast<const int64_t*>(ids), n, reinterpret_cast<float*>(feat),
                                          reinterpret_cast<float*>(pol), reinterpret_cast<float*>(val),
                                          reinterpret_cast<void*>(stream)));
             })
        .def("counters", [](const oamd_replay_view& v, uintptr_t stream) {
            int64_t size = 0, head = 0, games = 0;
            int32_t flags = 0;
            check(oamd_replay_counters(&v, &size, &head, &games, &flags, reinterpret_cast<void*>(stream)));
            return py::make_tuple(size, head, games, flags);
        });

    m.def("_host_solve", [](int player, uint64_t p1, uint64_t p2, int max_empties, int64_t node_limit) {
        oamd_position p{};
        p.player = player;
        p.player1_discs = p1;
        p.player2_discs = p2;
        int32_t ms[65], score = 0, best = 0, flags = 0;
        int64_t nodes = 0;
        check(oamd_host_solve_endgame(&p, max_empties, node_limit, ms, &score, &best, &flags, &nodes));
        return py::make_tuple(std::vector<int>(ms, ms + 65), score, best, flags, nodes);
    });
    m.def("_relabel_workspace_bytes", [](int64_t budget) {
        int64_t bytes = 0;
        check(oamd_replay_relabel_workspace_bytes(budget, &bytes));
        return bytes;
    });
    m.def("_solve_workspace_bytes", [](int64_t n) {
        int64_t bytes = 0;
        check(oamd_solve_workspace_bytes(n, &bytes));
        return bytes;
    });
    m.def("_gpu_solve", [](int device, uintptr_t pos, int64_t n, int max_empties, int64_t node_limit,
                           uintptr_t move_scores, uintptr_t score, uintptr_t best, uintptr_t flags, uintptr_t nodes,
                           uintptr_t workspace, int workgroups, uintptr_t stream) {
        auto* P = reinterpret_cast<const oamd_position*>(pos);
        auto* ms = reinterpret_cast<int32_t*>(move_scores);
        auto* sc = reinterpret_cast<int32_t*>(score);
        auto* be = reinterpret_cast<int32_t*>(best);
        auto* fl = reinterpret_cast<int32_t*>(flags);
        auto* no = reinterpret_cast<int64_t*>(nodes);
        void* ws = reinterpret_cast<void*>(workspace);
        void* st = reinterpret_cast<void*>(stream);
        if (workgroups == 0)
            check(oamd_solve_endgames(device, P, n, max_empties, node_limit, ms, sc, be, fl, no, ws, st));
        else
            check(oamd_solve_endgames_grid(device, P, n, max_empties, node_limit, ms, sc, be, fl, no, ws, workgroups,
                                           st));
    });

    m.def("_gpu_legal_moves", [](uintptr_t me, uintptr_t opp, uintptr_t out, int64_t n, uintptr_t stream) {
        check(oamd_get_legal_moves((const uint64_t*)me, (const uint64_t*)opp, (uint64_t*)out, n, (void*)stream));
    });
    m.def("_gpu_flips", [](uintptr_t mv, uintptr_t me, uintptr_t opp, uintptr_t out, int64_t n, uintptr_t stream) {
        check(oamd_get_flips((const uint64_t*)mv, (const uint64_t*)me, (const uint64_t*)opp, (uint64_t*)out, n,
                             (void*)stream));
    });
    m.def("_gpu_apply_action", [](uintptr_t in, uintptr_t actions, uintptr_t out, int64_t n, uintptr_t stream) {
        check(oamd_apply_action((const oamd_position*)in, (const int32_t*)actions, (oamd_position*)out, n,
                                (void*)stream));
    });
}
```

### othello-alphazero_amd/csrc/resnet.hip

```cpp

#include <hip/hip_runtime.h>

#include <cstdlib>
#include <type_traits>

#include "bitboard.h"
#include "kernels.h"

namespace oamd {

typedef __attribute__((ext_vector_type(8))) __bf16 bf16x8_t;
typedef __attribute__((ext_vector_type(8))) _Float16 f16x8_t;
typedef __attribute__((ext_vector_type(2))) __bf16 bf16x2_t;
typedef __attribute__((ext_vector_type(2))) _Float16 f16x2_t;
typedef __attribute__((ext_vector_type(2))) float f32x2_t;
typedef __attribute__((ext_vector_type(2))) short i16x2_t;
typedef __attribute__((ext_vector_type(4))) float f32x4_t;
typedef __attribute__((ext_vector_type(4))) unsigned int u32x4_t;
typedef __attribute__((ext_vector_type(2))) unsigned int u32x2_t;
typedef __attribute__((address_space(3))) void lds_void_t;

constexpr int kLdsBytes = 160 * 1024;
#ifdef OAMD_STAMPS
constexpr int kMaxStampWgs = 1 << 16;
constexpr int kStampStride = 24;
#endif
constexpr int kStageBytes = 16384;
#ifndef OAMD_C128_STAGE
#define OAMD_C128_STAGE 16384
#endif
#ifndef OAMD_C128_RING
#define OAMD_C128_RING 3
#endif
#ifndef OAMD_C256_STAGE
#define OAMD_C256_STAGE 16384
#endif
#ifndef OAMD_C256_RING
#define OAMD_C256_RING 4
#endif
constexpr int kWeightQueue = 4;
constexpr int kStageBytesMax = 32768;
__host__ __device__ constexpr int stage_bytes(int C) { return C == 256 ? OAMD_C256_STAGE : OAMD_C128_STAGE; }
#ifndef OAMD_VGPR_CAP
#define OAMD_VGPR_CAP 104
#endif
__host__ __device__ constexpr int wide_cb(int J) { return J / 3; }
__host__ __device__ constexpr int wide_dy(int J) { return J % 3 - 1; }
__host__ __device__ constexpr int wide_new(int J) { return J % 3 == 0 ? 0xFE : (J % 3 == 1 ? 0x100 : 0); }
#ifndef OAMD_EPI_NOBAR
#define OAMD_EPI_NOBAR 1
#endif
template <bool ENABLE>
__host__ __device__ constexpr int wide_new_last(int J, int NJ) {
    return !ENABLE || J < NJ - 3 ? wide_new(J) : (J % 3 == 0 ? 0x1FE : 0);
}

struct HeadLayout {
    int pcw, pcb, vcw, vcb, plw, plb, v1w, v1b, v2w, v2b, total;
    __host__ __device__ HeadLayout(int C, int hidden) {
        pcw = 0;
        pcb = pcw + 2 * C;
        vcw = pcb + 2;
        vcb = vcw + C;
        plw = vcb + 1;
        plb = plw + 128 * 65;
        v1w = plb + 65;
        v1b = v1w + 64 * hidden;
        v2w = v1b + hidden;
        v2b = v2w + hidden;
        total = v2b + 1;
    }
};

size_t resnet_head_floats(int C, int hidden) { return (size_t)HeadLayout(C, hidden).total; }

__host__ __device__ constexpr int ksteps_per_stage(int C) {
    return stage_bytes(C) / (32 * C * 2);
}
__host__ __device__ constexpr int ksteps_first(int C) {
    return (9 + ksteps_per_stage(C) - 1) / ksteps_per_stage(C) * ksteps_per_stage(C);
}
__host__ __device__ constexpr int ksteps_tower(int C) { return 9 * (C / 32); }
__host__ __device__ constexpr int kgroup_chunk(int kg) { return ((kg & 1) << 1) | (kg >> 1); }
__host__ __device__ constexpr int out_chan(int tile, int kg, int k) {
    return 32 * (tile >> 1) + 8 * kg + 4 * (tile & 1) + k;
}

int resnet_ksteps(int C, bool first) { return first ? ksteps_first(C) : ksteps_tower(C); }
void resnet_kstep(int C, bool first, int i, int* tap, int* cb, bool* pad) {
    if (first) {
        *tap = i < 9 ? i : 8;
        *cb = 0;
        *pad = i >= 9;
    } else {
        const int dxi = i / (3 * (C / 32)), J = i % (3 * (C / 32));
        *tap = dxi + 3 * (wide_dy(J) + 1);
        *cb = wide_cb(J);
        *pad = false;
    }
}
int resnet_kgroup_chunk(int kg) { return kgroup_chunk(kg); }
int resnet_out_channel(int tile, int row) { return out_chan(tile, row >> 2, row & 3); }
size_t resnet_packed_weight_elems(int C, int R) {
    return (size_t)(ksteps_first(C) + 2 * R * ksteps_tower(C)) * 32 * C;
}
size_t resnet_packed_weight_alloc_elems(int C, int R) { return resnet_packed_weight_elems(C, R) + 4 * kStageBytesMax / 2; }

__host__ __device__ constexpr int pad_row(int p) { return ((p >> 3) + 1) * 10 + (p & 7) + 1; }

struct TilePos {
    unsigned char p[64];
};
constexpr TilePos make_tile_pos() {
    TilePos t{};
    for (int n = 0; n < 16; ++n) {
        const int k = n < 4 ? n : (n < 12 ? n - 4 : n - 8);
        const int r = (n < 4 || n >= 12) ? 2 * k + 1 : 2 * k;
        int m = 0;
        for (int p = 0; p < 64; ++p)
            if (pad_row(p) % 16 == r) t.p[16 * (m++) + n] = (unsigned char)p;
    }
    return t;
}
__constant__ TilePos kTilePos = make_tile_pos();

template <class G>
__host__ __device__ constexpr int edge_tile_row(int q, int m, int j) {
    constexpr int NP = G::NPAIR > 0 ? G::NPAIR : 1;
    const int P = q % NP, h = q / NP;
    const int y = 4 * h + m;
    const int r0 = (P * G::BROWS + G::ROW0 + y * 10 + 1) & 15;
    const int oddcol = (j < 4 || j >= 12) ? 1 : 0;
    const int b = j < 8 ? P : P + NP;
    const int x = 2 * (j & 3) + ((r0 & 1) ^ oddcol);
    return b * G::BROWS + G::ROW0 + y * 10 + x + 1;
}

template <int C_, int BOARDS_, int WC_, int RING_MAX_, int STAGE_ = stage_bytes(C_), int PW_ = 64>
struct GeoT {
    static constexpr int C = C_;
    static constexpr int BOARDS = BOARDS_;
    static constexpr int WC = WC_;
    static constexpr int NT = WC / 16;
    static constexpr int WN = C / WC;
    static constexpr int PW = PW_;
    static constexpr int MT = PW / 16;
    static constexpr int WAVES = BOARDS * 64 / PW * WN;
    static constexpr int WPB = WAVES / BOARDS;
    static constexpr int THREADS = WAVES * 64;
    static constexpr int RP = 2 * C + 16;
    static constexpr int NPAIR = BOARDS / 2;
    static constexpr bool EDGE = BOARDS >= 2 && BOARDS % 2 == 0 && WC_ == 32 && PW_ == 128;
    static constexpr int ROW0 = EDGE ? 0 : 10;
    static constexpr int BROWS = !EDGE ? 100 : (NPAIR == 1 ? 88 : 84);
    __host__ __device__ static constexpr int prow(int p) { return ROW0 + (p >> 3) * 10 + (p & 7) + 1; }
    static constexpr int ACT_BYTES = BOARDS * BROWS * RP;
    static constexpr bool DIRECT = EDGE && C == 256;
    static constexpr int WQ = kWeightQueue;
    static constexpr int KSTEP_BYTES = 32 * C * 2;
    static constexpr int STAGE = STAGE_;
    static constexpr int KS = STAGE / KSTEP_BYTES;
    static constexpr int DPT = STAGE / 16 / THREADS;
    static constexpr int RING_FIT = (kLdsBytes - ACT_BYTES) / STAGE;
    static constexpr int RING = RING_FIT < RING_MAX_ ? RING_FIT : RING_MAX_;
    static constexpr int LDS = ACT_BYTES + RING * STAGE;
    static constexpr int AHEAD = RING - 1;
    static constexpr bool SPLIT_DMA = WAVES == 8 && KS == 2 && DPT == 2;
    static constexpr int VM_OPEN = (AHEAD - 1) * DPT;
    static constexpr int VM_LAYER = SPLIT_DMA ? AHEAD * DPT - 1 : AHEAD * DPT;
    static constexpr int OPEN_PART = SPLIT_DMA ? 0 : -1;
    static constexpr int MID_PART = 1;
    static_assert(RING >= 2 && LDS <= kLdsBytes && STAGE == KS * KSTEP_BYTES, "LDS budget");
    static_assert(KS == 1 || KS == 2 || KS == 4, "K-steps per stage");
    static_assert(ksteps_first(C) % KS == 0 && ksteps_tower(C) % KS == 0, "whole stages per layer");
    static_assert(THREADS >= BOARDS * 64 && DPT >= 1 && VM_LAYER <= 63, "decomposition");
    static_assert(!EDGE || ((NPAIR * BROWS) % 16 == 8 && WAVES == 8), "edge tiles: pair boards 8 rows apart mod 16");
    static_assert(!DIRECT || ((3 * (C / 32)) % WQ == 0 && WQ >= 2), "register queue: whole queues per dx");
};
template <int C>
using Geo = GeoT<C, 512 / C, 32, C == 128 ? OAMD_C128_RING : OAMD_C256_RING, stage_bytes(C), 128>;
template <int C>
using GeoS = GeoT<C, 1, C / 8, 4, kStageBytes>;

template <int DT>
__device__ __forceinline__ uint32_t to_act(float v) {
    if constexpr (DT == OAMD_BF16) {
        return __builtin_bit_cast(uint16_t, (__bf16)v);
    } else {
        return __builtin_bit_cast(uint16_t, (_Float16)v);
    }
}

template <int DT>
__device__ __forceinline__ float from_act(uint32_t u) {
    if constexpr (DT == OAMD_BF16) {
        return __uint_as_float(u << 16);
    } else {
        return (float)__builtin_bit_cast(_Float16, (uint16_t)u);
    }
}

template <int DT>
__device__ __forceinline__ uint32_t pack_relu(float a, float b) {
    i16x2_t s;
    if constexpr (DT == OAMD_BF16) {
        s = __builtin_bit_cast(i16x2_t, __builtin_convertvector((f32x2_t){a, b}, bf16x2_t));
    } else {
        s = __builtin_bit_cast(i16x2_t, __builtin_convertvector((f32x2_t){a, b}, f16x2_t));
    }
    return __builtin_bit_cast(uint32_t, __builtin_elementwise_max(s, (i16x2_t){0, 0}));
}

template <int DT>
__device__ __forceinline__ f32x4_t mfma(u32x4_t a, u32x4_t b, f32x4_t c) {
    if constexpr (DT == OAMD_BF16) {
        return __builtin_amdgcn_mfma_f32_16x16x32_bf16(__builtin_bit_cast(bf16x8_t, a),
                                                       __builtin_bit_cast(bf16x8_t, b), c, 0, 0, 0);
    } else {
        return __builtin_amdgcn_mfma_f32_16x16x32_f16(__builtin_bit_cast(f16x8_t, a),
                                                      __builtin_bit_cast(f16x8_t, b), c, 0, 0, 0);
    }
}

enum InputKind { kPacked = 0, kF32 = 1 };

struct RowMap {
    const int32_t* list;
    const int32_t* count;
    int off;
    int rows;
    unsigned long long* span;
};
__device__ __forceinline__ int map_row(const RowMap& M, int r) {
    if (r >= M.rows) return -1;
    return M.list ? M.list[r] : r;
}

template <int NT, int MT = 4>
struct Frags {
    u32x4_t w[NT];
    u32x4_t x[MT];
};

template <int C>
__device__ __forceinline__ int first_kstep_offset(int i) {
    const int tap = i < 9 ? i : 8;
    const int dy = tap / 3 - 1, dx = tap - 3 * (tap / 3) - 1;
    return (dy * 10 + dx) * Geo<C>::RP;
}
template <int C>
__device__ __forceinline__ int tower_kstep0_offset() {
    return (-10 - 1) * Geo<C>::RP;
}

template <int NT, int MT>
__device__ __forceinline__ void load_wfrags(Frags<NT, MT>& f, const unsigned char* wk, int wl) {
    const unsigned char* wp = wk + wl;
#pragma unroll
    for (int n = 0; n < NT; ++n) f.w[n] = *reinterpret_cast<const u32x4_t*>(wp + n * 1024);
}

template <int NT, int MT>
__device__ __forceinline__ void load_xfrags(Frags<NT, MT>& f, const unsigned char* act, int aoff, const int (&rd)[MT]) {
    const unsigned char* ap = act + aoff;
#pragma unroll
    for (int m = 0; m < MT; ++m) f.x[m] = *reinterpret_cast<const u32x4_t*>(ap + rd[m]);
}

template <int NT, int MT>
__device__ __forceinline__ void load_frags(Frags<NT, MT>& f, const unsigned char* act, const unsigned char* wk,
                                           int aoff, const int (&rd)[MT], int wl) {
    load_wfrags(f, wk, wl);
    load_xfrags(f, act, aoff, rd);
}

template <int N, class F>
__device__ __forceinline__ void static_for(F&& f) {
    if constexpr (N > 0) {
        static_for<N - 1>(f);
        f(std::integral_constant<int, N - 1>{});
    }
}

template <int DT, int NT, int MT>
__device__ __forceinline__ void mfma_frags(f32x4_t (&acc)[NT][MT], const Frags<NT, MT>& f) {
#pragma unroll
    for (int n = 0; n < NT; ++n)
#pragma unroll
        for (int m = 0; m < MT; ++m) acc[n][m] = mfma<DT>(f.w[n], f.x[m], acc[n][m]);
}

template <class G, int PART = -1>
__device__ __forceinline__ void issue_stage_dma(const unsigned char* src, unsigned char* ring, int slot, int tid) {
    unsigned char* dst = ring + slot * G::STAGE;
    const int wave = tid >> 6, lane = tid & 63;
#pragma unroll
    for (int i = 0; i < G::DPT; ++i) {
        if (PART >= 0 && i != PART) continue;
        const int q = i * G::THREADS + wave * 64;
        __builtin_amdgcn_global_load_lds(src + (size_t)(q + lane) * 16, (lds_void_t*)(dst + q * 16), 16, 0, 0);
    }
}

template <int N>
__device__ __forceinline__ void wait_vm() {
    static_assert(N >= 0 && N < 64, "vmcnt");
    __builtin_amdgcn_s_waitcnt((N & 15) | ((N >> 4) << 14) | 0x0F70);
    asm volatile("" ::: "memory");
}

__device__ __forceinline__ void lds_barrier() {
    asm volatile("s_waitcnt lgkmcnt(0)" ::: "memory");
    __builtin_amdgcn_s_barrier();
    asm volatile("" ::: "memory");
}

constexpr int kMaxValueHidden = 1024;
template <int B>
__host__ __device__ constexpr int head_scratch_floats(int hidden) {
    return 128 * B + 64 * B + 4 * B * 64 + 2 * B * ((hidden + 63) / 64) * 64;
}

#ifdef OAMD_STAMPS
__device__ unsigned long long g_oamd_stamps[kMaxStampWgs * kStampStride];
__device__ __forceinline__ void stamp(int slot, int wave, int lane) {
    if (wave == 0 && lane == 0 && blockIdx.x < kMaxStampWgs) {
        __builtin_amdgcn_sched_barrier(0);
        g_oamd_stamps[blockIdx.x * kStampStride + slot] = __builtin_amdgcn_s_memrealtime();
        if (slot == 1 || slot == 2) g_oamd_stamps[blockIdx.x * kStampStride + 4 + slot] = __builtin_amdgcn_s_memtime();
        if (slot == 0) {
            unsigned id;
            asm volatile("s_getreg_b32 %0, hwreg(HW_REG_HW_ID)" : "=s"(id));
            unsigned xcc;
            asm volatile("s_getreg_b32 %0, hwreg(HW_REG_XCC_ID)" : "=s"(xcc));
            g_oamd_stamps[blockIdx.x * kStampStride + 4] = ((unsigned long long)xcc << 32) | id;
        }
        __builtin_amdgcn_sched_barrier(0);
    }
}
#define OAMD_STAMP(slot) stamp(slot, wave, lane)
#else
#define OAMD_STAMP(slot) ((void)0)
#endif

template <int B>
__device__ __forceinline__ void dot32(float (&acc)[B], const float (&w)[32], const float* x) {
#pragma unroll
    for (int k0 = 0; k0 < 32; k0 += 8) {
        __builtin_amdgcn_sched_barrier(0);
#pragma unroll
        for (int k = k0; k < k0 + 8; ++k)
#pragma unroll
            for (int b = 0; b < B; ++b) acc[b] = __builtin_fmaf(w[k], x[k * B + b], acc[b]);
    }
}

template <class G, int DT>
__device__ __forceinline__ void heads(const NetView& N, const unsigned char* act, unsigned char* scratch, int wave,
                                      int lane, int row0, const RowMap& M, float* __restrict__ policy,
                                      float* __restrict__ value) {
    constexpr int C = G::C;
    constexpr int B = G::BOARDS;
    constexpr int NW = G::WAVES;
    static_assert(head_scratch_floats<B>(kMaxValueHidden) * 4 <= G::RING * G::STAGE, "head scratch");
    asm volatile("" : "+v"(lane));
    const HeadLayout HL(C, N.hidden);
    const float* hp = N.head;
    const int hid = N.hidden;
    const int nvs = (hid + 63) / 64;
    float* sp = reinterpret_cast<float*>(scratch);
    float* sv = sp + 128 * B;
    float* pp = sv + 64 * B;
    float* pv = pp + 4 * B * 64;

    auto task_weights = [&](int task, float (&wv)[32]) {
        const float* w;
        int stride;
        if (task < 4) {
            w = hp + HL.plw + task * 32 * 65 + lane;
            stride = 65;
        } else {
            const int t = task - 4, c = t & 1, j = (t >> 1) * 64 + lane;
            w = hp + HL.v1w + c * 32 * hid + (j < hid ? j : hid - 1);
            stride = hid;
        }
#pragma unroll
        for (int k = 0; k < 32; ++k) wv[k] = w[k * stride];
    };
    const int ntask = 4 + 2 * nvs;
    float wv[32];
    if (wave % G::WPB != 0 && wave < ntask) task_weights(wave, wv);
    OAMD_STAMP(8);
    if (wave % G::WPB == 0) {
        const int b = wave / G::WPB;
        u32x4_t hw[C / 32];
#pragma unroll
        for (int cb = 0; cb < C / 32; ++cb)
            hw[cb] = *reinterpret_cast<const u32x4_t*>(N.hconv + ((size_t)cb * 64 + lane) * 8);
        int rd[4];
#pragma unroll
        for (int m = 0; m < 4; ++m)
            rd[m] = (b * G::BROWS + G::prow(kTilePos.p[16 * m + (lane & 15)])) * G::RP + kgroup_chunk(lane >> 4) * 16;
        f32x4_t d[4];
#pragma unroll
        for (int m = 0; m < 4; ++m) d[m] = f32x4_t{0.0f, 0.0f, 0.0f, 0.0f};
#pragma unroll
        for (int cb = 0; cb < C / 32; ++cb)
#pragma unroll
            for (int m = 0; m < 4; ++m)
                d[m] = mfma<DT>(hw[cb], *reinterpret_cast<const u32x4_t*>(act + rd[m] + cb * 64), d[m]);
        if (lane < 16) {
            const float pb0 = hp[HL.pcb + 0], pb1 = hp[HL.pcb + 1], vb = hp[HL.vcb];
#pragma unroll
            for (int m = 0; m < 4; ++m) {
                const int pos = kTilePos.p[16 * m + lane];
                sp[pos * B + b] = fmaxf(d[m][0] + pb0, 0.0f);
                sp[(64 + pos) * B + b] = fmaxf(d[m][1] + pb1, 0.0f);
                sv[pos * B + b] = fmaxf(d[m][2] + vb, 0.0f);
            }
        }
    }
    __syncthreads();
    OAMD_STAMP(9);
    for (int task = wave; task < ntask; task += NW) {
        float acc[B];
#pragma unroll
        for (int b = 0; b < B; ++b) acc[b] = 0.0f;
        if (task != wave || wave % G::WPB == 0) task_weights(task, wv);
        if (task < 4) {
            const float* x = sp + task * 32 * B;
            dot32<B>(acc, wv, x);
#pragma unroll
            for (int b = 0; b < B; ++b) pp[(task * B + b) * 64 + lane] = acc[b];
        } else {
            const int t = task - 4, c = t & 1, q = t >> 1;
            const int j = q * 64 + lane;
            const float* x = sv + c * 32 * B;
            dot32<B>(acc, wv, x);
#pragma unroll
            for (int b = 0; b < B; ++b) pv[(c * B + b) * nvs * 64 + j] = acc[b];
        }
    }
    __syncthreads();
    OAMD_STAMP(10);
    for (int job = wave; job < 2 * B; job += NW) {
        const int b = job % B;
        const int gr = map_row(M, row0 + b);
        if (gr < 0) continue;
        if (job < B) {
            const float o = hp[HL.plb + lane] + (((pp[(0 * B + b) * 64 + lane] + pp[(1 * B + b) * 64 + lane]) +
                                                  pp[(2 * B + b) * 64 + lane]) +
                                                 pp[(3 * B + b) * 64 + lane]);
            const float u0 = hp[HL.plw + lane * 65 + 64], u1 = hp[HL.plw + (64 + lane) * 65 + 64];
            float o64 = __builtin_fmaf(u1, sp[(64 + lane) * B + b], u0 * sp[lane * B + b]);
#pragma unroll
            for (int off = 32; off > 0; off >>= 1) o64 += __shfl_xor(o64, off);
            o64 += hp[HL.plb + 64];
            float m = o;
#pragma unroll
            for (int off = 32; off > 0; off >>= 1) m = fmaxf(m, __shfl_xor(m, off));
            m = fmaxf(m, o64);
            const float e = __expf(o - m);
            const float e64 = __expf(o64 - m);
            float ssum = e;
#pragma unroll
            for (int off = 32; off > 0; off >>= 1) ssum += __shfl_xor(ssum, off);
            ssum += e64;
            const float inv = 1.0f / ssum;
            policy[(size_t)gr * 65 + lane] = e * inv;
            if (lane == 0) policy[(size_t)gr * 65 + 64] = e64 * inv;
        } else {
            float part = 0.0f;
            for (int q = 0; q < nvs; ++q) {
                const int j = q * 64 + lane;
                if (j < hid) {
                    const float h = hp[HL.v1b + j] + (pv[(0 * B + b) * nvs * 64 + j] + pv[(1 * B + b) * nvs * 64 + j]);
                    part = __builtin_fmaf(fmaxf(h, 0.0f), hp[HL.v2w + j], part);
                }
            }
#pragma unroll
            for (int off = 32; off > 0; off >>= 1) part += __shfl_xor(part, off);
            if (lane == 0) value[gr] = tanhf(part + hp[HL.v2b]);
        }
    }
}

template <class G>
__device__ __forceinline__ void load_bias(float4 (&bv)[G::NT], const NetView& N, int layer, int wn, int lane) {
#pragma unroll
    for (int n = 0; n < G::NT; ++n)
        bv[n] = *reinterpret_cast<const float4*>(N.bias + (size_t)layer * G::C + out_chan(wn * G::NT + n, lane >> 4, 0));
}

template <class G, int DT, int IN>
__device__ __forceinline__ void resnet_body(NetView N, const void* __restrict__ feat_in, int fw, int H, RowMap M,
                                            float* __restrict__ policy, float* __restrict__ value, int wg) {
    constexpr int C = G::C;
    constexpr int kNT = G::NT;
    constexpr int kMT = G::MT;
    extern __shared__ __attribute__((aligned(16))) unsigned char smem[];
    unsigned char* act = smem;
    unsigned char* ring = smem + G::ACT_BYTES;

    const int tid = threadIdx.x;
    const int wave = tid >> 6;
    const int lane = tid & 63;
    const int wm = wave / G::WN;
    const int wn = wave % G::WN;
    const int kg = lane >> 4;
    const int row0 = wg * G::BOARDS;
    if (M.list) {
        const int filled = *M.count - M.off;
        M.rows = filled < M.rows ? (filled > 0 ? filled : 0) : M.rows;
        if (row0 >= M.rows) return;
    }
    OAMD_STAMP(0);
#ifdef OAMD_STAMPS
    unsigned long long ep_sum[3] = {0, 0, 0}, ep_t = 0;
    unsigned long long wt_sum[3] = {0, 0, 0};
    unsigned long long pw[4] = {0, 0, 0, 0};
    bool pw_on = false, pw_open = false;
#define OAMD_EP_MARK(k)                                                          \
    do {                                                                         \
        __builtin_amdgcn_sched_barrier(0);                                       \
        const unsigned long long t_ = __builtin_amdgcn_s_memtime();              \
        if ((k) > 0) ep_sum[(k) - 1] += t_ - ep_t;                               \
        ep_t = t_;                                                               \
        __builtin_amdgcn_sched_barrier(0);                                       \
    } while (0)
#define OAMD_T() __builtin_amdgcn_s_memtime()
#define OAMD_STEP_WAIT(stmt)                                                     \
    do {                                                                         \
        __builtin_amdgcn_sched_barrier(0);                                       \
        const unsigned long long w0_ = OAMD_T();                                 \
        stmt;                                                                    \
        if (pw_on) {                                                             \
            wt_sum[0] += pw[1] - pw[0];                                          \
            if (pw_open) {                                                       \
                wt_sum[1] += pw[2] - pw[1];                                      \
                wt_sum[2] += pw[3] - pw[2];                                      \
            }                                                                    \
        }                                                                        \
        pw[0] = w0_;                                                             \
        pw[1] = OAMD_T();                                                        \
        pw_on = true;                                                            \
        pw_open = false;                                                         \
        __builtin_amdgcn_sched_barrier(0);                                       \
    } while (0)
#define OAMD_OPEN_WAIT(vmstmt, barstmt)                                          \
    do {                                                                         \
        vmstmt;                                                                  \
        pw[2] = OAMD_T();                                                        \
        barstmt;                                                                 \
        pw[3] = OAMD_T();                                                        \
        pw_open = true;                                                          \
    } while (0)
#else
#define OAMD_EP_MARK(k) ((void)0)
#define OAMD_STEP_WAIT(stmt) stmt
#define OAMD_OPEN_WAIT(vmstmt, barstmt) \
    do {                                 \
        vmstmt;                          \
        barstmt;                         \
    } while (0)
#endif
    const unsigned char* wsrc = reinterpret_cast<const unsigned char*>(N.w);

    const unsigned char* wcur = wsrc + G::AHEAD * G::STAGE;
    if constexpr (!G::DIRECT) {
#pragma unroll
        for (int s = 0; s < G::AHEAD; ++s) issue_stage_dma<G>(wsrc + s * G::STAGE, ring, s, tid);
        issue_stage_dma<G, G::OPEN_PART>(wcur, ring, G::AHEAD, tid);
    }

    float4 bv[kNT];
    load_bias<G>(bv, N, 0, wn, lane);

    int rd[kMT], wr[kMT];
    const int erow0 = G::EDGE ? edge_tile_row<G>(wm, 0, lane & 15) * G::RP : 0;
#pragma unroll
    for (int m = 0; m < kMT; ++m) {
        const int rowb = G::EDGE ? erow0 + m * 10 * G::RP
                                 : (wm * G::BROWS + G::prow(kTilePos.p[16 * m + (lane & 15)])) * G::RP;
        rd[m] = rowb + kgroup_chunk(kg) * 16;
        wr[m] = rowb;
    }
    const int wl = (wn * kNT * 64 + lane) * 16;

    constexpr int WQ = G::DIRECT ? G::WQ : 1;
    constexpr int WOFF = ksteps_first(C) % WQ;
    u32x4_t wq[WQ][kNT];
    const unsigned char* wgp = wsrc;
    auto wload = [&](auto SLOT) {
        constexpr int q = decltype(SLOT)::value % WQ;
#pragma unroll
        for (int n = 0; n < kNT; ++n) wq[q][n] = *reinterpret_cast<const u32x4_t*>(wgp + wl + n * 1024);
        wgp += G::KSTEP_BYTES;
    };
    if constexpr (G::DIRECT) static_for<WQ - 1>([&](auto I) { wload(I); });

    constexpr int NBC = G::ROW0 ? 36 : 16;
    for (int w = tid; w < G::BOARDS * NBC * (C / 8); w += G::THREADS) {
        const int c = w % (C / 8), k = (w / (C / 8)) % NBC, b = w / (C / 8) / NBC;
        const int r = G::ROW0 ? (k < 10 ? k : (k < 20 ? 80 + k : ((k - 20) >> 1) * 10 + 10 + ((k & 1) ? 9 : 0)))
                              : (k >> 1) * 10 + ((k & 1) ? 9 : 0);
        *reinterpret_cast<u32x4_t*>(act + (b * G::BROWS + r) * G::RP + c * 16) = u32x4_t{0u, 0u, 0u, 0u};
    }
    if (tid < G::BOARDS * 64) {
        const int b = tid >> 6, p = tid & 63;
        const int gr = map_row(M, row0 + b);
        const uint32_t one = to_act<DT>(1.0f);
        uint32_t words[16];
        if constexpr (IN == kPacked) {
            uint32_t mask = 0;
            if (gr >= 0) {
                const uint64_t* fr = reinterpret_cast<const uint64_t*>(feat_in) + (size_t)gr * fw;
                const uint64_t wj = fr[p < fw ? p : fw - 1];
                const uint32_t lo = (uint32_t)wj, hi = (uint32_t)(wj >> 32);
                auto word = [&](int j) {
                    return ((uint64_t)(uint32_t)__builtin_amdgcn_readlane((int)hi, j) << 32) |
                           (uint32_t)__builtin_amdgcn_readlane((int)lo, j);
                };
                const uint64_t meta = word(0);
                if ((meta >> 16) & 1ULL) {
                    const int t = (int)((meta >> 8) & 7ULL);
                    const int src = inverse_transform(p, t);
                    mask = (uint32_t)(meta & 1ULL);
                    for (int h = 0; h < H; ++h) {
                        mask |= (uint32_t)((word(2 + 2 * h) >> (63 - src)) & 1ULL) << (1 + 2 * h);
                        mask |= (uint32_t)((word(3 + 2 * h) >> (63 - src)) & 1ULL) << (2 + 2 * h);
                    }
                }
            }
#pragma unroll
            for (int w = 0; w < 16; ++w) {
                const uint32_t lo = ((mask >> (2 * w)) & 1u) ? one : 0u;
                const uint32_t hi = ((mask >> (2 * w + 1)) & 1u) ? one : 0u;
                words[w] = lo | (hi << 16);
            }
        } else {
            float v[32];
#pragma unroll
            for (int c = 0; c < 32; ++c) v[c] = 0.0f;
            if (gr >= 0) {
                const float* fr = reinterpret_cast<const float*>(feat_in) + (size_t)gr * N.cin * 64;
#pragma unroll
                for (int c = 0; c < 32; ++c) v[c] = fr[(c < N.cin ? c : N.cin - 1) * 64 + p];
            }
#pragma unroll
            for (int w = 0; w < 16; ++w) {
                const int c0 = 2 * w, c1 = 2 * w + 1;
                const uint32_t lo = c0 < N.cin ? to_act<DT>(v[c0]) : 0u;
                const uint32_t hi = c1 < N.cin ? to_act<DT>(v[c1]) : 0u;
                words[w] = lo | (hi << 16);
            }
        }
        unsigned char* dst = act + (b * G::BROWS + G::prow(p)) * G::RP;
#pragma unroll
        for (int c = 0; c < 4; ++c)
            *reinterpret_cast<u32x4_t*>(dst + c * 16) =
                u32x4_t{words[4 * c], words[4 * c + 1], words[4 * c + 2], words[4 * c + 3]};
    }

    f32x4_t acc[kNT][kMT];
    u32x2_t skip[kNT][kMT];

    Frags<kNT, kMT> fa, fb;
    constexpr bool kWide = G::EDGE;
    u32x4_t win0[kWide ? 9 : 1], win1[kWide ? 9 : 1];
    const int sb0 = rd[0] - 10 * G::RP - G::RP;
    int slot = 0;

    OAMD_STAMP(7);
    if constexpr (IN == kPacked) {
        bool live = false;
#pragma unroll
        for (int b = 0; b < G::BOARDS; ++b) {
            const int gr = map_row(M, row0 + b);
            if (gr >= 0) live |= ((reinterpret_cast<const uint64_t*>(feat_in)[(size_t)gr * fw] >> 16) & 1ULL) != 0;
        }
        if (!live) {
            wait_vm<0>();
            return;
        }
    }
    if constexpr (!G::DIRECT) wait_vm<G::VM_LAYER>();
    lds_barrier();
    if constexpr (!G::DIRECT) load_wfrags(fa, ring, wl);
#pragma unroll
    for (int m = kWide ? 1 : 0; m < kMT; ++m)
        fa.x[m] = *reinterpret_cast<const u32x4_t*>(act + first_kstep_offset<C>(0) + rd[m]);
    OAMD_STAMP(1);
#ifdef OAMD_STAMPS
    const unsigned long long tower_t0 = __builtin_amdgcn_s_memtime();
#endif
    if constexpr (G::BOARDS > 1) __builtin_amdgcn_s_setprio(1);

    const int nlayers = 1 + 2 * N.R;
    auto conv = [&](auto KIND, int layer) {
        constexpr int kind = decltype(KIND)::value;
        constexpr bool first = kind == 0;
        constexpr int nk = first ? ksteps_first(C) : ksteps_tower(C);

#pragma unroll
        for (int n = 0; n < kNT; ++n)
#pragma unroll
            for (int m = 0; m < kMT; ++m) {
                f32x4_t a = f32x4_t{bv[n].x, bv[n].y, bv[n].z, bv[n].w};
                if constexpr (kind == 2) {
                    const u32x2_t r = skip[n][m];
                    a[0] += from_act<DT>(r.x & 0xffffu);
                    a[1] += from_act<DT>(r.x >> 16);
                    a[2] += from_act<DT>(r.y & 0xffffu);
                    a[3] += from_act<DT>(r.y >> 16);
                }
                acc[n][m] = a;
            }

        auto step = [&](auto KIS, auto TILES, auto GI, const Frags<kNT, kMT>& cur, Frags<kNT, kMT>& nxt, int xoff) {
            constexpr int kis = decltype(KIS)::value;
            constexpr int gi = decltype(GI)::value;
            constexpr bool open = kis == 0 && !G::DIRECT;
            constexpr int tl = decltype(TILES)::value;
            constexpr int xlo = tl & 15, xhi = (tl >> 4) & 15, mlo = (tl >> 8) & 15, mhi = (tl >> 12) & 15;
            __builtin_amdgcn_sched_barrier(0);
            OAMD_STEP_WAIT(__builtin_amdgcn_s_waitcnt(0xC07F));
            {
                const unsigned char* ap = act + xoff;
#pragma unroll
                for (int m = xlo; m < xhi; ++m) nxt.x[m] = *reinterpret_cast<const u32x4_t*>(ap + rd[m]);
            }
            if constexpr (open) {
                OAMD_OPEN_WAIT(wait_vm<G::VM_OPEN>(), __builtin_amdgcn_s_barrier());
                const int sp = (slot + G::AHEAD + 1) % G::RING;
                wcur += G::STAGE;
                issue_stage_dma<G, G::OPEN_PART>(wcur, ring, sp, tid);
                slot = slot == G::RING - 1 ? 0 : slot + 1;
            } else if constexpr (G::SPLIT_DMA && !G::DIRECT) {
                int sa = slot + G::AHEAD;
                sa = sa >= G::RING ? sa - G::RING : sa;
                issue_stage_dma<G, G::MID_PART>(wcur, ring, sa, tid);
            }
            if constexpr (G::DIRECT) wload(std::integral_constant<int, gi + WQ - 1>{});
            else load_wfrags(nxt, ring + slot * G::STAGE + kis * G::KSTEP_BYTES, wl);
#pragma unroll
            for (int n = 0; n < kNT; ++n)
#pragma unroll
                for (int m = mlo; m < mhi; ++m) {
                    if constexpr (G::DIRECT) acc[n][m] = mfma<DT>(wq[gi % WQ][n], cur.x[m], acc[n][m]);
                    else acc[n][m] = mfma<DT>(cur.w[n], cur.x[m], acc[n][m]);
                }
            if constexpr (G::DIRECT) {
                constexpr int nds = xhi - xlo;
                constexpr int nm = kNT * (mhi - mlo);
                static_for<nds>([&](auto I) {
                    constexpr int i = decltype(I)::value;
                    __builtin_amdgcn_sched_group_barrier(0x100, 1, 0);
                    __builtin_amdgcn_sched_group_barrier(0x008, (i + 1) * nm / nds - i * nm / nds, 0);
                });
            } else if constexpr (kMT != 4) {
                constexpr int nds = open ? kNT : kNT + (xhi - xlo);
                constexpr int nm = kNT * (mhi - mlo);
                static_for<nds>([&](auto I) {
                    constexpr int i = decltype(I)::value;
                    __builtin_amdgcn_sched_group_barrier(0x100, 1, 0);
                    __builtin_amdgcn_sched_group_barrier(0x008, (i + 1) * nm / nds - i * nm / nds, 0);
                });
            } else {
                constexpr int nds = open ? 4 : 8;
                static_for<nds>([&](auto) {
                    __builtin_amdgcn_sched_group_barrier(0x100, 1, 0);
                    __builtin_amdgcn_sched_group_barrier(0x008, 16 / nds, 0);
                });
            }
        };
        using AllTiles = std::integral_constant<int, kMT << 4 | kMT << 12>;
        if constexpr (first) {
            auto tiles = [](int i) {
                const int dy = (i < 9 ? i : 8) / 3 - 1;
                const int lo = kWide && dy < 0 ? 1 : 0, hi = kWide && dy > 0 ? kMT - 1 : kMT;
                return lo | hi << 4 | lo << 8 | hi << 12;
            };
            static_for<nk - 1>([&](auto II) {
                constexpr int i1 = decltype(II)::value + 1;
                constexpr int tl = (tiles(i1) & 0xFF) | (tiles(i1 - 1) & 0xFF00);
                using GI = std::integral_constant<int, i1 - 1>;
                if constexpr (i1 % 2 == 1) step(std::integral_constant<int, i1 % G::KS>{},
                                                std::integral_constant<int, tl>{}, GI{}, fa, fb, first_kstep_offset<C>(i1));
                else step(std::integral_constant<int, i1 % G::KS>{}, std::integral_constant<int, tl>{}, GI{}, fb, fa,
                          first_kstep_offset<C>(i1));
            });
            constexpr int ml = tiles(nk - 1) >> 8 & 15, mh = tiles(nk - 1) >> 12 & 15;
            const Frags<kNT, kMT>& last = (nk - 1) % 2 == 1 ? fb : fa;
            if constexpr (G::DIRECT) wload(std::integral_constant<int, nk - 1 + WQ - 1>{});
#pragma unroll
            for (int n = 0; n < kNT; ++n)
#pragma unroll
                for (int m = ml; m < mh; ++m) {
                    if constexpr (G::DIRECT) acc[n][m] = mfma<DT>(wq[(nk - 1) % WQ][n], last.x[m], acc[n][m]);
                    else acc[n][m] = mfma<DT>(last.w[n], last.x[m], acc[n][m]);
                }
        } else if constexpr (kWide) {
            constexpr int KPT = C / 32;
            static_assert(kNT == 2 && kMT == 8 && KPT % 2 == 0 && (3 * KPT) % G::KS == 0, "wide geometry");
            constexpr int NJ = 3 * KPT;
            constexpr int RS = 10 * G::RP;
            auto wstep = [&](auto JJ, auto LASTDX, const Frags<kNT, kMT>& wc, Frags<kNT, kMT>& wn, int sbn) {
                constexpr int J = decltype(JJ)::value;
                constexpr int Jn = (J + 1) % NJ;
                constexpr bool open = Jn % G::KS == 0 && !G::DIRECT;
                constexpr int newmask =
                    decltype(LASTDX)::value ? wide_new_last<OAMD_EPI_NOBAR && !G::DIRECT>(Jn, NJ) : wide_new(Jn);
                constexpr int dy = wide_dy(J), cbn = wide_cb(Jn), nnew = __builtin_popcount(newmask);
                constexpr int mlo = dy < 0 ? 1 : 0, mhi = dy > 0 ? 7 : 8;
                auto& Wc = [&]() -> u32x4_t(&)[9] {
                    if constexpr (wide_cb(J) % 2 == 0) return win0; else return win1;
                }();
                auto& Wn = [&]() -> u32x4_t(&)[9] {
                    if constexpr (cbn % 2 == 0) return win0; else return win1;
                }();
                __builtin_amdgcn_sched_barrier(0);
                OAMD_STEP_WAIT(__builtin_amdgcn_s_waitcnt(0xC07F));
                static_for<9>([&](auto I) {
                    constexpr int i = decltype(I)::value;
                    if constexpr ((newmask >> i) & 1)
                        Wn[i] = *reinterpret_cast<const u32x4_t*>(act + sbn + i * RS + cbn * 64);
                });
                if constexpr (open) {
                    OAMD_OPEN_WAIT(wait_vm<G::VM_OPEN>(), __builtin_amdgcn_s_barrier());
                    const int sp = (slot + G::AHEAD + 1) % G::RING;
                    wcur += G::STAGE;
                    issue_stage_dma<G, G::OPEN_PART>(wcur, ring, sp, tid);
                    slot = slot == G::RING - 1 ? 0 : slot + 1;
                } else if constexpr (G::SPLIT_DMA && !G::DIRECT) {
                    int sa = slot + G::AHEAD;
                    sa = sa >= G::RING ? sa - G::RING : sa;
                    issue_stage_dma<G, G::MID_PART>(wcur, ring, sa, tid);
                }
                if constexpr (G::DIRECT) wload(std::integral_constant<int, WOFF + J + WQ - 1>{});
                else load_wfrags(wn, ring + slot * G::STAGE + (Jn % G::KS) * G::KSTEP_BYTES, wl);
#pragma unroll
                for (int n = 0; n < kNT; ++n)
#pragma unroll
                    for (int m = mlo; m < mhi; ++m) {
                        if constexpr (G::DIRECT) acc[n][m] = mfma<DT>(wq[(WOFF + J) % WQ][n], Wc[m + 1 + dy], acc[n][m]);
                        else acc[n][m] = mfma<DT>(wc.w[n], Wc[m + 1 + dy], acc[n][m]);
                    }
                constexpr int nds = G::DIRECT ? nnew : (open ? kNT : kNT + nnew);
                constexpr int nm = kNT * (mhi - mlo);
                static_for<nds>([&](auto I) {
                    constexpr int i = decltype(I)::value;
                    __builtin_amdgcn_sched_group_barrier(0x100, 1, 0);
                    __builtin_amdgcn_sched_group_barrier(0x008, (i + 1) * nm / nds - i * nm / nds, 0);
                });
            };
            auto dx_wide = [&](int dxi, auto LASTDX) {
                constexpr bool lastdx = decltype(LASTDX)::value;
                const int sb = sb0 + dxi * G::RP;
                static_for<lastdx ? NJ - 1 : NJ>([&](auto JJ) {
                    constexpr int J = decltype(JJ)::value;
                    const int sbn = J == NJ - 1 ? sb + G::RP : sb;
                    if constexpr (J % 2 == 0) wstep(JJ, LASTDX, fa, fb, sbn);
                    else wstep(JJ, LASTDX, fb, fa, sbn);
                });
                if constexpr (lastdx) {
                    if constexpr (G::DIRECT) wload(std::integral_constant<int, WOFF + NJ - 1 + WQ - 1>{});
#pragma unroll
                    for (int n = 0; n < kNT; ++n)
#pragma unroll
                        for (int m = 0; m < 7; ++m) {
                            if constexpr (G::DIRECT) acc[n][m] = mfma<DT>(wq[(WOFF + NJ - 1) % WQ][n], win1[m + 2], acc[n][m]);
                            else acc[n][m] = mfma<DT>(fb.w[n], win1[m + 2], acc[n][m]);
                        }
                }
            };
#pragma nounroll
            for (int dxi = 0; dxi < 2; ++dxi) dx_wide(dxi, std::false_type{});
            dx_wide(2, std::true_type{});
        } else {
            constexpr int KPT = C / 32;
            static_assert(KPT % 2 == 0, "whole block pairs");
            constexpr int NJ = 3 * KPT;
            auto xoff_of = [](int dxi, int J) { return (wide_dy(J) * 10 + dxi - 1) * G::RP + wide_cb(J) * 64; };
            auto dx_steps = [&](int dxi, auto LASTDX) {
                constexpr bool lastdx = decltype(LASTDX)::value;
                static_for<lastdx ? NJ - 1 : NJ>([&](auto JJ) {
                    constexpr int J = decltype(JJ)::value;
                    using KIS = std::integral_constant<int, (J + 1) % G::KS>;
                    const int xo = J == NJ - 1 ? xoff_of(dxi + 1, 0) : xoff_of(dxi, J + 1);
                    if constexpr (J % 2 == 0) step(KIS{}, AllTiles{}, std::integral_constant<int, 0>{}, fa, fb, xo);
                    else step(KIS{}, AllTiles{}, std::integral_constant<int, 0>{}, fb, fa, xo);
                });
            };
#pragma nounroll
            for (int dxi = 0; dxi < 2; ++dxi) dx_steps(dxi, std::false_type{});
            dx_steps(2, std::true_type{});
            mfma_frags<DT>(acc, fb);
        }

        const bool more = layer + 1 < nlayers;
        if (more) load_bias<G>(bv, N, layer + 1, wn, lane);
#ifdef OAMD_STAMPS
        OAMD_STEP_WAIT(asm volatile("s_waitcnt lgkmcnt(0)" ::: "memory"));
        pw_on = false;
#endif
        OAMD_EP_MARK(0);
        constexpr bool nobar = OAMD_EPI_NOBAR && kWide && !first && !G::DIRECT;
        const int last_slot = slot;
        if constexpr (!nobar) {
            lds_barrier();
        }
        OAMD_EP_MARK(1);
        if constexpr (!G::DIRECT && !nobar) {
            wcur += G::STAGE;
            issue_stage_dma<G, G::OPEN_PART>(wcur, ring, (slot + G::AHEAD + 1) % G::RING, tid);
        }
        if constexpr (kNT == 2) {
            const int co = 2 * out_chan(wn * 2, kg, 0);
#pragma unroll
            for (int m = 0; m < kMT; ++m) {
                u32x4_t* p = reinterpret_cast<u32x4_t*>(act + wr[m] + co);
                if constexpr (kind == 1) {
                    const u32x4_t v = *p;
                    skip[0][m] = u32x2_t{v.x, v.y};
                    skip[1][m] = u32x2_t{v.z, v.w};
                }
                const f32x4_t a = acc[0][m], b = acc[1][m];
                *p = u32x4_t{pack_relu<DT>(a[0], a[1]), pack_relu<DT>(a[2], a[3]), pack_relu<DT>(b[0], b[1]),
                             pack_relu<DT>(b[2], b[3])};
            }
        } else {
#pragma unroll
            for (int n = 0; n < kNT; ++n)
#pragma unroll
                for (int m = 0; m < kMT; ++m) {
                    u32x2_t* p = reinterpret_cast<u32x2_t*>(act + wr[m] + 2 * out_chan(wn * kNT + n, kg, 0));
                    if constexpr (kind == 1) skip[n][m] = *p;
                    const f32x4_t a = acc[n][m];
                    *p = u32x2_t{pack_relu<DT>(a[0], a[1]), pack_relu<DT>(a[2], a[3])};
                }
        }
        slot = slot == G::RING - 1 ? 0 : slot + 1;
        OAMD_EP_MARK(2);
        if (more) {
            if constexpr (!G::DIRECT) wait_vm<nobar ? G::VM_LAYER - 1 : G::VM_LAYER>();
            lds_barrier();
            if constexpr (!G::DIRECT && nobar) {
                wcur += G::STAGE;
                issue_stage_dma<G, G::OPEN_PART>(wcur, ring, (last_slot + G::AHEAD + 1) % G::RING, tid);
            }
            if constexpr (kWide) {
                if constexpr (!G::DIRECT) load_wfrags(fa, ring + slot * G::STAGE, wl);
#pragma unroll
                for (int i = 1; i < 8; ++i) win0[i] = *reinterpret_cast<const u32x4_t*>(act + sb0 + i * 10 * G::RP);
            } else {
                load_frags(fa, act, ring + slot * G::STAGE, tower_kstep0_offset<C>(), rd, wl);
            }
#ifdef OAMD_STAMPS
            asm volatile("s_waitcnt lgkmcnt(0)" ::: "memory");
#endif
        }
        OAMD_EP_MARK(3);
    };
    conv(std::integral_constant<int, 0>{}, 0);
    for (int blk = 0; blk < N.R; ++blk) {
        conv(std::integral_constant<int, 1>{}, 1 + 2 * blk);
        conv(std::integral_constant<int, 2>{}, 2 + 2 * blk);
    }
    __syncthreads();
    OAMD_STAMP(2);
#ifdef OAMD_STAMPS
    const unsigned long long tower_cyc = __builtin_amdgcn_s_memtime() - tower_t0;
#endif
#ifdef OAMD_STAMPS
    if (wave == 0 && lane == 0 && blockIdx.x < kMaxStampWgs)
        for (int i = 0; i < 3; ++i) g_oamd_stamps[blockIdx.x * kStampStride + 11 + i] = ep_sum[i];
    if (lane == 0 && blockIdx.x < kMaxStampWgs) {
        unsigned long long* q = g_oamd_stamps + blockIdx.x * kStampStride + 16;
        for (int i = 0; i < 3; ++i) atomicAdd(q + i, wt_sum[i]);
        for (int i = 0; i < 3; ++i) atomicAdd(q + 3 + i, ep_sum[i]);
        atomicAdd(q + 6, tower_cyc);
    }
#endif
    heads<G, DT>(N, act, ring, wave, lane, row0, M, policy, value);
    OAMD_STAMP(3);
}

template <class G, int DT, int IN>
__global__ __launch_bounds__(512) __attribute__((amdgpu_num_vgpr(OAMD_VGPR_CAP))) void k_resnet_w8(
    NetView N, const void* __restrict__ feat_in, int fw, int H, RowMap M, float* __restrict__ policy,
    float* __restrict__ value) {
    if (M.span && threadIdx.x == 0) atomicMax(M.span, ~(unsigned long long)__builtin_amdgcn_s_memrealtime());
    resnet_body<G, DT, IN>(N, feat_in, fw, H, M, policy, value, blockIdx.x);
    if (M.span) {
        __syncthreads();
        if (threadIdx.x == 0) atomicMax(M.span + 1, (unsigned long long)__builtin_amdgcn_s_memrealtime());
    }
}

template <class G, int DT, int IN>
__global__ __launch_bounds__(512) __attribute__((amdgpu_num_vgpr(OAMD_VGPR_CAP))) void k_resnet_w8_loop(
    NetView N, const void* __restrict__ feat_in, int fw, int H, RowMap M, float* __restrict__ policy,
    float* __restrict__ value) {
    if (M.span && threadIdx.x == 0) atomicMax(M.span, ~(unsigned long long)__builtin_amdgcn_s_memrealtime());
    int rows = M.rows;
    if (M.list) {
        const int filled = *M.count - M.off;
        rows = filled < rows ? (filled > 0 ? filled : 0) : rows;
    }
    for (int wg = blockIdx.x; wg * G::BOARDS < rows; wg += gridDim.x) {
        resnet_body<G, DT, IN>(N, feat_in, fw, H, M, policy, value, wg);
        __syncthreads();
    }
    if (M.span) {
        __syncthreads();
        if (threadIdx.x == 0) atomicMax(M.span + 1, (unsigned long long)__builtin_amdgcn_s_memrealtime());
    }
}

template <class G, int DT, int IN>
static void launch_t(const NetView& N, const void* feat, int fw, int H, const RowMap& M, float* pol, float* val,
                     hipStream_t s, int max_wgs) {
    const int rows = M.rows;
    static_assert(G::THREADS == 512, "k_resnet_w8 geometries");
    const unsigned grid = (unsigned)((rows + G::BOARDS - 1) / G::BOARDS);
    constexpr auto kern = &k_resnet_w8<G, DT, IN>;
    static bool configured = false;
    if (!configured) {
        (void)hipFuncSetAttribute(reinterpret_cast<const void*>(kern), hipFuncAttributeMaxDynamicSharedMemorySize,
                                  G::LDS);
        configured = true;
    }
    if constexpr (IN == kPacked) {
        if (max_wgs > 0 && grid > (unsigned)max_wgs) {
            constexpr auto lk = &k_resnet_w8_loop<G, DT, IN>;
            static bool lconfigured = false;
            if (!lconfigured) {
                (void)hipFuncSetAttribute(reinterpret_cast<const void*>(lk),
                                          hipFuncAttributeMaxDynamicSharedMemorySize, G::LDS);
                lconfigured = true;
            }
            hipLaunchKernelGGL(lk, dim3(max_wgs), dim3(G::THREADS), G::LDS, s, N, feat, fw, H, M, pol, val);
            return;
        }
    }
    hipLaunchKernelGGL(kern, dim3(grid), dim3(G::THREADS), G::LDS, s, N, feat, fw, H, M, pol, val);
}

constexpr int kSmallBatchRows = 1024;

template <int IN>
static void dispatch(const NetView& N, const void* feat, int fw, int H, const RowMap& M, float* pol, float* val,
                     hipStream_t s, int max_wgs = 0) {
    const int rows = M.rows;
    if (rows <= 0) return;
    const bool small = rows < kSmallBatchRows;
    const bool fp16 = N.dtype == OAMD_FP16;
    if (N.C == 128) {
        if (small) {
            if (fp16) launch_t<GeoS<128>, OAMD_FP16, IN>(N, feat, fw, H, M, pol, val, s, max_wgs);
            else launch_t<GeoS<128>, OAMD_BF16, IN>(N, feat, fw, H, M, pol, val, s, max_wgs);
        } else {
            if (fp16) launch_t<Geo<128>, OAMD_FP16, IN>(N, feat, fw, H, M, pol, val, s, max_wgs);
            else launch_t<Geo<128>, OAMD_BF16, IN>(N, feat, fw, H, M, pol, val, s, max_wgs);
        }
    } else {
        if (small) {
            if (fp16) launch_t<GeoS<256>, OAMD_FP16, IN>(N, feat, fw, H, M, pol, val, s, max_wgs);
            else launch_t<GeoS<256>, OAMD_BF16, IN>(N, feat, fw, H, M, pol, val, s, max_wgs);
        } else {
            if (fp16) launch_t<Geo<256>, OAMD_FP16, IN>(N, feat, fw, H, M, pol, val, s, max_wgs);
            else launch_t<Geo<256>, OAMD_BF16, IN>(N, feat, fw, H, M, pol, val, s, max_wgs);
        }
    }
}

void launch_resnet_packed(const NetView& N, const uint64_t* feat, int fw, int H, int rows,
                          float* policy, float* value, hipStream_t s, const int32_t* rowlist,
                          const int32_t* rowcount, int list_off, unsigned long long* span, int max_wgs) {
    dispatch<kPacked>(N, feat, fw, H, RowMap{rowlist, rowcount, list_off, rows, span}, policy, value, s, max_wgs);
}

void launch_resnet_f32(const NetView& N, const float* feat, int rows, float* policy, float* value,
                       hipStream_t s) {
    dispatch<kF32>(N, feat, 0, 0, RowMap{nullptr, nullptr, 0, rows, nullptr}, policy, value, s);
}

int resnet_read_stamps(unsigned long long* out, long long n) {
#ifdef OAMD_STAMPS
    if (n > (long long)kMaxStampWgs * kStampStride) n = (long long)kMaxStampWgs * kStampStride;
    return hipMemcpyFromSymbol(out, HIP_SYMBOL(g_oamd_stamps), (size_t)n * 8, 0, hipMemcpyDeviceToHost) == hipSuccess
               ? 0
               : -1;
#else
    (void)out;
    (void)n;
    return -2;
#endif
}

}
```

### othello-alphazero_amd/othello_mcts/native.py

```python

from __future__ import annotations

import json
import os
import warnings
import weakref
from pathlib import Path

import numpy as np
import torch

from ._othello_mcts_impl import _Net
from .synthetic import net_config_from_state_dict

_DTYPES = {"bf16": 0, "bfloat16": 0, "fp16": 1, "float16": 1}
_DTYPES_NAME = {0: "bf16", 1: "fp16"}


def _to_numpy_state(sd) -> dict[str, np.ndarray]:
    out = {}
    for k, v in sd.items():
        if isinstance(v, torch.Tensor):
            v = v.detach().to("cpu", torch.float32).numpy()
        out[k] = np.ascontiguousarray(np.asarray(v, dtype=np.float32))
    return out


def load_checkpoint(checkpoint_dir) -> tuple[dict, dict]:
    checkpoint_dir = Path(checkpoint_dir)
    with (checkpoint_dir / "config.json").open(encoding="utf-8") as f:
        config = json.load(f)
    in_channels = config["neural_net"]["in_channels"]
    if in_channels % 2 != 1:
        raise ValueError(f"Expected in_channels to be odd, but got {in_channels}.")
    history_size = (in_channels - 1) // 2
    if history_size < 1:
        raise ValueError(f"Expected history_size to be positive, but got {history_size}.")
    sd = torch.load(checkpoint_dir / "neural_net.pth", map_location="cpu", weights_only=True)
    got = net_config_from_state_dict(sd)
    for k, v in config["neural_net"].items():
        if k in got and got[k] != v:
            raise ValueError(f"config.json neural_net.{k} = {v} but neural_net.pth has {got[k]}")
    return config, sd


class NativeNet:

    @classmethod
    def from_checkpoint(cls, checkpoint_dir, device: int | str | torch.device | None = None,
                        dtype: str = "bf16") -> "NativeNet":
        _, sd = load_checkpoint(checkpoint_dir)
        return cls(sd, device=device, dtype=dtype)

    def __init__(self, net_or_state_dict, device: int | str | torch.device | None = None,
                 dtype: str = "bf16") -> None:
        if hasattr(net_or_state_dict, "state_dict"):
            mod = getattr(net_or_state_dict, "_orig_mod", net_or_state_dict)
            sd = mod.state_dict()
        else:
            sd = net_or_state_dict
        self.config = net_config_from_state_dict(sd)
        if dtype not in _DTYPES:
            raise ValueError(f"dtype must be one of {sorted(_DTYPES)}, got {dtype!r}")
        self.dtype = dtype
        if device is None:
            device = torch.cuda.current_device()
        self.device = torch.device("cuda", device if isinstance(device, int) else torch.device(device).index or 0)
        c = self.config
        self._net = _Net(self.device.index, c["in_channels"], c["conv_channels"], c["num_residual_blocks"],
                         c["value_head_hidden_channels"], _DTYPES[dtype])
        self.load_state_dict(sd)

    def load_state_dict(self, sd) -> None:
        arrs = _to_numpy_state(sd)
        tensors = []
        for key, numel in self._net.state_keys():
            a = arrs[key].reshape(-1)
            if a.size != numel:
                raise ValueError(f"{key}: expected {numel} elements, got {a.size}")
            tensors.append(a)
        self._net.load_state(tensors)

    @property
    def handle(self) -> int:
        return self._net.handle

    @property
    def history_size(self) -> int:
        return (self.config["in_channels"] - 1) // 2

    def __call__(self, features: torch.Tensor) -> dict[str, torch.Tensor]:
        x = features.to(self.device, torch.float32).contiguous()
        rows = x.shape[0]
        policy = torch.empty((rows, 65), dtype=torch.float32, device=self.device)
        value = torch.empty((rows,), dtype=torch.float32, device=self.device)
        stream = torch.cuda.current_stream(self.device).cuda_stream
        self._net.forward(x.data_ptr(), rows, policy.data_ptr(), value.data_ptr(), stream)
        return {"policy": policy, "value": value}


FP16_MAX = 65504.0
FP16_HEADROOM = 16.0


@torch.no_grad()
def fp16_headroom(sd, history_size: int, positions: int = 32, device="cpu") -> float:
    import torch.nn.functional as F

    from .synthetic import calibration_features

    t = {k: torch.as_tensor(np.asarray(v, np.float32) if not isinstance(v, torch.Tensor) else v)
         .to(device=device, dtype=torch.float32) for k, v in sd.items() if not k.endswith("num_batches_tracked")}
    x = torch.from_numpy(calibration_features(positions, history_size, 11)).to(device)
    peak = 0.0

    def bn(h, p):
        return F.batch_norm(h, t[p + ".running_mean"], t[p + ".running_var"], t[p + ".weight"], t[p + ".bias"],
                            training=False, eps=1e-5)

    def conv(h, p, norm, pad=1):
        nonlocal peak
        y = bn(F.conv2d(h, t[p + ".weight"], t[p + ".bias"], padding=pad), norm)
        peak = max(peak, float(y.abs().max()))
        return y

    h = F.relu(conv(x, "conv_block.conv", "conv_block.norm"))
    i = 0
    while f"residual_blocks.{i}.conv1.weight" in t:
        p = f"residual_blocks.{i}"
        a = F.relu(conv(h, p + ".conv1", p + ".norm1"))
        h = conv(a, p + ".conv2", p + ".norm2") + h
        peak = max(peak, float(h.abs().max()))
        h = F.relu(h)
        i += 1
    conv(h, "policy_head.conv", "policy_head.norm", 0)
    conv(h, "value_head.conv", "value_head.norm", 0)
    return FP16_MAX / max(peak, 1e-30) if np.isfinite(peak) else 0.0


def _looks_like_alphazero(m) -> bool:
    if not all(hasattr(m, a) for a in ("conv_block", "residual_blocks", "policy_head", "value_head")):
        return False
    for cls in type(m).__mro__:
        if "forward" in vars(cls):
            return cls.__name__ == "AlphaZeroNet"
    return False


_warned: set = set()


def _warn_once(m, dtype: str, note: str = "") -> None:
    key = (id(type(m)), dtype, note)
    if key in _warned:
        return
    _warned.add(key)
    warnings.warn(
        f"othello_mcts: evaluating {type(m).__name__} with the native fused kernel in {dtype} "
        "(the reference calls the module's own fp32 forward); near-tied visit counts can differ "
        "(DESIGN.md §9: from the same positions and random streams the fp16 search picks the fp32 search's "
        "move in ~86 % of positions, the fp32 search itself in ~71 % under another symmetry stream). "
        "MCTS(..., native_nn=False) / set_native_nn(False) or OTHELLO_MCTS_NATIVE_NN=0 keeps the "
        "module's forward." + note,
        RuntimeWarning, stacklevel=3)


_cache: "weakref.WeakKeyDictionary" = weakref.WeakKeyDictionary()


def _signature(m) -> tuple:
    sig = []
    for t in list(m.parameters()) + list(m.buffers()):
        sig.append((t.data_ptr(), t._version))
    return tuple(sig)


def resolve(neural_net, device: int, history_size: int, dtype: str = "fp16"):
    if isinstance(neural_net, NativeNet):
        if neural_net.device.index != device:
            raise ValueError(f"NativeNet lives on cuda:{neural_net.device.index}, the search on cuda:{device}")
        if neural_net.history_size != history_size:
            raise ValueError("NativeNet in_channels does not match 1 + 2 * history_size")
        return neural_net
    if os.environ.get("OTHELLO_MCTS_NATIVE_NN", "1") == "0":
        return None
    if dtype not in _DTYPES:
        raise ValueError(f"nn_dtype must be one of {sorted(_DTYPES)}, got {dtype!r}")
    m = getattr(neural_net, "_orig_mod", neural_net)
    if not isinstance(m, torch.nn.Module) or not _looks_like_alphazero(m) or m.training:
        return None
    try:
        cfg = net_config_from_state_dict(m.state_dict())
    except (KeyError, AttributeError):
        return None
    if cfg["conv_channels"] not in (128, 256) or cfg["in_channels"] != 1 + 2 * history_size:
        return None
    if cfg["num_squares"] != 64 or cfg["num_actions"] != 65:
        return None
    sig = _signature(m)
    hit = _cache.get(m)
    if hit is not None and hit[0] == sig and hit[1].device.index == device and hit[2] == dtype:
        return hit[1]
    use, note = _DTYPES_NAME[_DTYPES[dtype]], ""
    if use == "fp16":
        room = fp16_headroom(m.state_dict(), history_size, device=torch.device("cuda", device))
        if room < FP16_HEADROOM:
            use = "bf16"
            note = (f" fp16 was requested, but the net's largest activation on real positions leaves only "
                    f"{room:.1f}x headroom below the fp16 maximum (< {FP16_HEADROOM:g}x): bf16 is used.")
    _warn_once(m, use, note)
    nn_ = NativeNet(m, device=device, dtype=use)
    _cache[m] = (sig, nn_, dtype)
    return nn_
```

Measured before the change: 5.808 million.

## Add four-wave C128 ResNet kernel with two board pairs per wave and no weight ring

Adds a new 256-thread ResNet geometry for 128-channel nets, on by default, in which each wave handles two edge-tile board pairs (PW 256). Weights stream straight into registers instead of through an LDS ring, so LDS only holds activations plus head scratch. The intent is a smaller footprint per workgroup so tree-search waves can share the CU with the network, and more reuse of each loaded weight across twice the boards. The cost is higher register pressure, capped at 208 VGPRs and checked at build time for scratch spills. It also adds guard words after the policy and value buffers with a debug check for overruns.

```diff
diff --git a/include/othello_mcts_amd_experimental.h b/include/othello_mcts_amd_experimental.h
--- a/include/othello_mcts_amd_experimental.h
+++ b/include/othello_mcts_amd_experimental.h
@@ -12,7 +12,10 @@
 int oamd_engine_set_chain_split(oamd_engine *e, int32_t budget, int32_t cuts);
 int oamd_engine_set_adaptive_extra_rounds(oamd_engine *e, int32_t enable, int32_t min_rounds);
 int oamd_engine_set_extra_round_grid(oamd_engine *e, int32_t workgroups);
+int oamd_set_resnet_c128_four_wave(int32_t enable);
+int oamd_resnet_c128_four_wave(void);
 int oamd_debug_read_stamps(uint64_t *out, int64_t n);
+int oamd_debug_eval_guards(oamd_engine *e, int32_t *intact);
 int oamd_debug_tree_stamps(uint64_t *out, int64_t n, int32_t reset);
 
 int oamd_engine_set_free_running(oamd_engine *e, int32_t enable);
diff --git a/othello-alphazero_amd/build.py b/othello-alphazero_amd/build.py
--- a/othello-alphazero_amd/build.py
+++ b/othello-alphazero_amd/build.py
@@ -33,6 +33,7 @@
 
 
 W8_VGPR_LIMIT = 208
+W4_VGPR_LIMIT = 416
 
 
 def run(cmd: list[str]) -> None:
@@ -86,7 +87,29 @@
         sys.stderr.write("note: no k_resnet_w8 kernel in this build\n")
 
 
-RESOURCE_CHECKS = {"resnet.hip": check_w8_vgprs, "solver.hip": check_solver_scratch}
+def check_w4_resources(remarks: str) -> None:
+    regs: dict[str, int] = {}
+    for name, field, value in kernel_remarks(remarks):
+        if "k_resnet_w4" not in name or "k_resnet_w4_loop" in name:
+            continue
+        if field in ("VGPRs", "AGPRs"):
+            regs[name] = regs.get(name, 0) + (int(value.split()[0]) + 7) // 8 * 8
+        elif field.startswith("ScratchSize") and int(value.split()[0]) != 0:
+            raise SystemExit(f"build failed: {name} uses {value} bytes of scratch per lane")
+    for name, v in regs.items():
+        if v > W4_VGPR_LIMIT:
+            raise SystemExit(f"build failed: {name} uses {v} VGPRs + AGPRs (> {W4_VGPR_LIMIT}): "
+                             "a k_tree wave could no longer co-reside with the ResNet kernel")
+    if not regs:
+        raise SystemExit("build failed: no resource remark for k_resnet_w4 in resnet.hip")
+
+
+def check_resnet(remarks: str) -> None:
+    check_w8_vgprs(remarks)
+    check_w4_resources(remarks)
+
+
+RESOURCE_CHECKS = {"resnet.hip": check_resnet, "solver.hip": check_solver_scratch}
 
 
 def newer(out: Path, deps: list[Path]) -> bool:
diff --git a/othello-alphazero_amd/csrc/capi.hip b/othello-alphazero_amd/csrc/capi.hip
--- a/othello-alphazero_amd/csrc/capi.hip
+++ b/othello-alphazero_amd/csrc/capi.hip
@@ -338,6 +338,8 @@
         return OAMD_OK;
     }
 
+    static constexpr int kEvalGuard = 16;
+    static constexpr int kEvalGuardByte = 0x5A;
     int L() const { return cfg.num_threads * cfg.batch_size; }
     int steps() const { return search_steps(cfg.num_simulations, L()); }
     bool thread_split() const {
@@ -417,11 +419,14 @@
         int rc;
         if ((rc = dalloc(&leaf, rows)) || (rc = dalloc(&depth, rows)) || (rc = dalloc(&trans, rows)) ||
             (rc = dalloc(&path, rows * kMaxDepth)) || (rc = dalloc(&feat, rows * fw)) ||
-            (rc = dalloc(&policy, rows * 65)) || (rc = dalloc(&value, rows)) || (rc = dalloc(&flags, rows)) ||
+            (rc = dalloc(&policy, rows * 65 + kEvalGuard)) || (rc = dalloc(&value, rows + kEvalGuard)) ||
+            (rc = dalloc(&flags, rows)) ||
             (rc = dalloc(&rowlist, rows)) || (rc = dalloc(&tstate, rows)))
             return rc;
         HIPCHK(hipMemset(policy, 0, rows * 65 * sizeof(float)));
         HIPCHK(hipMemset(value, 0, rows * sizeof(float)));
+        HIPCHK(hipMemset(policy + rows * 65, kEvalGuardByte, kEvalGuard * sizeof(float)));
+        HIPCHK(hipMemset(value + rows, kEvalGuardByte, kEvalGuard * sizeof(float)));
         rows_cap = rows;
         fw_cap = fw;
         return OAMD_OK;
@@ -1263,6 +1268,28 @@
     if (groups < 0 || groups > kMaxPipeline)
         return fail(OAMD_INVALID_ARGUMENT, "pipeline groups must be in [0, " + std::to_string(kMaxPipeline) + "]");
     e->pipeline = groups;
+    return OAMD_OK;
+}
+
+int oamd_set_resnet_c128_four_wave(int32_t enable) {
+    resnet_set_c128_four_wave(enable);
+    return OAMD_OK;
+}
+
+int oamd_resnet_c128_four_wave(void) { return resnet_c128_four_wave(); }
+
+int oamd_debug_eval_guards(oamd_engine* e, int32_t* intact) {
+    if (!e || !intact) return fail(OAMD_INVALID_ARGUMENT, "eval guards: null argument");
+    DeviceGuard dg(e->device);
+    *intact = 1;
+    if (!e->policy || !e->value) return OAMD_OK;
+    HIPCHK(hipDeviceSynchronize());
+    unsigned char g[2][oamd_engine::kEvalGuard * sizeof(float)];
+    HIPCHK(hipMemcpy(g[0], e->policy + e->rows_cap * 65, sizeof(g[0]), hipMemcpyDeviceToHost));
+    HIPCHK(hipMemcpy(g[1], e->value + e->rows_cap, sizeof(g[1]), hipMemcpyDeviceToHost));
+    for (auto& b : g)
+        for (unsigned char c : b)
+            if (c != oamd_engine::kEvalGuardByte) *intact = 0;
     return OAMD_OK;
 }
 
diff --git a/othello-alphazero_amd/csrc/kernels.h b/othello-alphazero_amd/csrc/kernels.h
--- a/othello-alphazero_amd/csrc/kernels.h
+++ b/othello-alphazero_amd/csrc/kernels.h
@@ -74,6 +74,8 @@
 size_t resnet_packed_weight_alloc_elems(int C, int R);
 size_t resnet_head_floats(int C, int hidden);
 inline size_t resnet_hconv_elems(int C) { return (size_t)(C / 32) * 64 * 8; }
+void resnet_set_c128_four_wave(int enable);
+int resnet_c128_four_wave();
 int resnet_read_stamps(unsigned long long* out, long long n);
 int tree_read_stamps(unsigned long long* out, long long n, int reset);
 int resnet_ksteps(int C, bool first);
diff --git a/othello-alphazero_amd/csrc/pybind_module.cpp b/othello-alphazero_amd/csrc/pybind_module.cpp
--- a/othello-alphazero_amd/csrc/pybind_module.cpp
+++ b/othello-alphazero_amd/csrc/pybind_module.cpp
@@ -408,6 +408,8 @@
     m.def("get_flips", &oamd_host_flips, "move_mask"_a, "player_discs"_a, "opponent_discs"_a);
     m.def("device_count", &device_count);
     m.def("abi_version", &oamd_abi_version);
+    m.def("set_resnet_c128_four_wave", [](bool enable) { check(oamd_set_resnet_c128_four_wave(enable ? 1 : 0)); });
+    m.def("resnet_c128_four_wave", []() { return oamd_resnet_c128_four_wave() != 0; });
     m.def("source_hash", [](const std::string& family) {
         const char* h = oamd_source_hash(family.c_str());
         if (!h) throw py::value_error("unknown source family: " + family);
@@ -669,6 +671,11 @@
             check(oamd_engine_round_counts(e.h, &searches, &rounds, &finals));
             return py::make_tuple(searches, rounds, finals);
         })
+        .def("eval_guards_intact", [](Engine& e) {
+            int32_t ok = 0;
+            check(oamd_debug_eval_guards(e.h, &ok));
+            return ok != 0;
+        })
         .def("set_free_running",
              [](Engine& e, bool enable) { check(oamd_engine_set_free_running(e.h, enable ? 1 : 0)); })
         .def("set_exact_interleaving",
diff --git a/othello-alphazero_amd/csrc/resnet.hip b/othello-alphazero_amd/csrc/resnet.hip
--- a/othello-alphazero_amd/csrc/resnet.hip
+++ b/othello-alphazero_amd/csrc/resnet.hip
@@ -1,6 +1,7 @@
 
 #include <hip/hip_runtime.h>
 
+#include <atomic>
 #include <cstdlib>
 #include <type_traits>
 
@@ -124,11 +125,19 @@
 }
 __constant__ TilePos kTilePos = make_tile_pos();
 
+constexpr int kMaxValueHidden = 1024;
+template <int B>
+__host__ __device__ constexpr int head_scratch_floats(int hidden) {
+    return 128 * B + 64 * B + 4 * B * 64 + 2 * B * ((hidden + 63) / 64) * 64;
+}
+
 template <class G>
 __host__ __device__ constexpr int edge_tile_row(int q, int m, int j) {
     constexpr int NP = G::NPAIR > 0 ? G::NPAIR : 1;
-    const int P = q % NP, h = q / NP;
-    const int y = 4 * h + m;
+    constexpr int PPW = G::MT >= 8 ? G::MT / 8 : 1;
+    const int g = q * PPW + m / 8;
+    const int P = g % NP, h = g / NP;
+    const int y = 4 * h + m % 8;
     const int r0 = (P * G::BROWS + G::ROW0 + y * 10 + 1) & 15;
     const int oddcol = (j < 4 || j >= 12) ? 1 : 0;
     const int b = j < 8 ? P : P + NP;
@@ -150,12 +159,15 @@
     static constexpr int THREADS = WAVES * 64;
     static constexpr int RP = 2 * C + 16;
     static constexpr int NPAIR = BOARDS / 2;
-    static constexpr bool EDGE = BOARDS >= 2 && BOARDS % 2 == 0 && WC_ == 32 && PW_ == 128;
+    static constexpr bool EDGE = BOARDS >= 2 && BOARDS % 2 == 0 && WC_ == 32 && (PW_ == 128 || PW_ == 256);
+    static constexpr int PAIRS = EDGE ? PW_ / 128 : 1;
     static constexpr int ROW0 = EDGE ? 0 : 10;
     static constexpr int BROWS = !EDGE ? 100 : (NPAIR == 1 ? 88 : 84);
     __host__ __device__ static constexpr int prow(int p) { return ROW0 + (p >> 3) * 10 + (p & 7) + 1; }
     static constexpr int ACT_BYTES = BOARDS * BROWS * RP;
-    static constexpr bool DIRECT = EDGE && C == 256;
+    static constexpr bool DIRECT = EDGE && (C == 256 || PAIRS == 2);
+    static constexpr bool NORING = PAIRS == 2;
+    static constexpr int SCRATCH = head_scratch_floats<BOARDS_>(kMaxValueHidden) * 4;
     static constexpr int WQ = kWeightQueue;
     static constexpr int KSTEP_BYTES = 32 * C * 2;
     static constexpr int STAGE = STAGE_;
@@ -163,7 +175,7 @@
     static constexpr int DPT = STAGE / 16 / THREADS;
     static constexpr int RING_FIT = (kLdsBytes - ACT_BYTES) / STAGE;
     static constexpr int RING = RING_FIT < RING_MAX_ ? RING_FIT : RING_MAX_;
-    static constexpr int LDS = ACT_BYTES + RING * STAGE;
+    static constexpr int LDS = ACT_BYTES + (NORING ? SCRATCH : RING * STAGE);
     static constexpr int AHEAD = RING - 1;
     static constexpr bool SPLIT_DMA = WAVES == 8 && KS == 2 && DPT == 2;
     static constexpr int VM_OPEN = (AHEAD - 1) * DPT;
@@ -174,11 +186,13 @@
     static_assert(KS == 1 || KS == 2 || KS == 4, "K-steps per stage");
     static_assert(ksteps_first(C) % KS == 0 && ksteps_tower(C) % KS == 0, "whole stages per layer");
     static_assert(THREADS >= BOARDS * 64 && DPT >= 1 && VM_LAYER <= 63, "decomposition");
-    static_assert(!EDGE || ((NPAIR * BROWS) % 16 == 8 && WAVES == 8), "edge tiles: pair boards 8 rows apart mod 16");
+    static_assert(!EDGE || ((NPAIR * BROWS) % 16 == 8 && WAVES * PAIRS == 8), "edge tiles: pair boards 8 rows apart mod 16");
+    static_assert(!NORING || (DIRECT && NPAIR == 2 && BROWS % 2 == 0 && ACT_BYTES % 16 == 0), "two pairs per wave");
     static_assert(!DIRECT || ((3 * (C / 32)) % WQ == 0 && WQ >= 2), "register queue: whole queues per dx");
 };
 template <int C>
 using Geo = GeoT<C, 512 / C, 32, C == 128 ? OAMD_C128_RING : OAMD_C256_RING, stage_bytes(C), 128>;
+using GeoW4 = GeoT<128, 4, 32, OAMD_C128_RING, stage_bytes(128), 256>;
 template <int C>
 using GeoS = GeoT<C, 1, C / 8, 4, kStageBytes>;
 
@@ -315,11 +329,6 @@
     asm volatile("" ::: "memory");
 }
 
-constexpr int kMaxValueHidden = 1024;
-template <int B>
-__host__ __device__ constexpr int head_scratch_floats(int hidden) {
-    return 128 * B + 64 * B + 4 * B * 64 + 2 * B * ((hidden + 63) / 64) * 64;
-}
 
 #ifdef OAMD_STAMPS
 __device__ unsigned long long g_oamd_stamps[kMaxStampWgs * kStampStride];
@@ -362,7 +371,7 @@
     constexpr int C = G::C;
     constexpr int B = G::BOARDS;
     constexpr int NW = G::WAVES;
-    static_assert(head_scratch_floats<B>(kMaxValueHidden) * 4 <= G::RING * G::STAGE, "head scratch");
+    static_assert(head_scratch_floats<B>(kMaxValueHidden) * 4 <= G::LDS - G::ACT_BYTES, "head scratch");
     asm volatile("" : "+v"(lane));
     const HeadLayout HL(C, N.hidden);
     const float* hp = N.head;
@@ -576,11 +585,17 @@
     float4 bv[kNT];
     load_bias<G>(bv, N, 0, wn, lane);
 
+    constexpr int kPT = G::EDGE ? 8 : kMT;
+    constexpr int kNP = kMT / kPT;
+    constexpr int kPairB = G::BROWS * G::RP;
+    static_assert(kNP == 1 || (edge_tile_row<G>(0, 8, 0) == edge_tile_row<G>(0, 0, 0) + G::BROWS &&
+                               edge_tile_row<G>(0, 15, 13) == edge_tile_row<G>(0, 7, 13) + G::BROWS),
+                  "pair bases one board apart");
     int rd[kMT], wr[kMT];
     const int erow0 = G::EDGE ? edge_tile_row<G>(wm, 0, lane & 15) * G::RP : 0;
 #pragma unroll
     for (int m = 0; m < kMT; ++m) {
-        const int rowb = G::EDGE ? erow0 + m * 10 * G::RP
+        const int rowb = G::EDGE ? erow0 + (m / kPT) * kPairB + (m % kPT) * 10 * G::RP
                                  : (wm * G::BROWS + G::prow(kTilePos.p[16 * m + (lane & 15)])) * G::RP;
         rd[m] = rowb + kgroup_chunk(kg) * 16;
         wr[m] = rowb;
@@ -667,7 +682,7 @@
 
     Frags<kNT, kMT> fa, fb;
     constexpr bool kWide = G::EDGE;
-    u32x4_t win0[kWide ? 9 : 1], win1[kWide ? 9 : 1];
+    u32x4_t win0[kNP][kWide ? 9 : 1], win1[kNP][kWide ? 9 : 1];
     const int sb0 = rd[0] - 10 * G::RP - G::RP;
     int slot = 0;
 
@@ -688,8 +703,10 @@
     lds_barrier();
     if constexpr (!G::DIRECT) load_wfrags(fa, ring, wl);
 #pragma unroll
-    for (int m = kWide ? 1 : 0; m < kMT; ++m)
-        fa.x[m] = *reinterpret_cast<const u32x4_t*>(act + first_kstep_offset<C>(0) + rd[m]);
+    for (int p = 0; p < kNP; ++p)
+#pragma unroll
+        for (int m = kWide ? 1 : 0; m < kPT; ++m)
+            fa.x[p * kPT + m] = *reinterpret_cast<const u32x4_t*>(act + first_kstep_offset<C>(0) + rd[p * kPT + m]);
     OAMD_STAMP(1);
 #ifdef OAMD_STAMPS
     const unsigned long long tower_t0 = __builtin_amdgcn_s_memtime();
@@ -728,7 +745,10 @@
             {
                 const unsigned char* ap = act + xoff;
 #pragma unroll
-                for (int m = xlo; m < xhi; ++m) nxt.x[m] = *reinterpret_cast<const u32x4_t*>(ap + rd[m]);
+                for (int p = 0; p < kNP; ++p)
+#pragma unroll
+                    for (int m = xlo; m < xhi; ++m)
+                        nxt.x[p * kPT + m] = *reinterpret_cast<const u32x4_t*>(ap + rd[p * kPT + m]);
             }
             if constexpr (open) {
                 OAMD_OPEN_WAIT(wait_vm<G::VM_OPEN>(), __builtin_amdgcn_s_barrier());
@@ -746,13 +766,15 @@
 #pragma unroll
             for (int n = 0; n < kNT; ++n)
 #pragma unroll
-                for (int m = mlo; m < mhi; ++m) {
-                    if constexpr (G::DIRECT) acc[n][m] = mfma<DT>(wq[gi % WQ][n], cur.x[m], acc[n][m]);
-                    else acc[n][m] = mfma<DT>(cur.w[n], cur.x[m], acc[n][m]);
-                }
+                for (int p = 0; p < kNP; ++p)
+#pragma unroll
+                    for (int m = p * kPT + mlo; m < p * kPT + mhi; ++m) {
+                        if constexpr (G::DIRECT) acc[n][m] = mfma<DT>(wq[gi % WQ][n], cur.x[m], acc[n][m]);
+                        else acc[n][m] = mfma<DT>(cur.w[n], cur.x[m], acc[n][m]);
+                    }
             if constexpr (G::DIRECT) {
-                constexpr int nds = xhi - xlo;
-                constexpr int nm = kNT * (mhi - mlo);
+                constexpr int nds = kNP * (xhi - xlo);
+                constexpr int nm = kNP * kNT * (mhi - mlo);
                 static_for<nds>([&](auto I) {
                     constexpr int i = decltype(I)::value;
                     __builtin_amdgcn_sched_group_barrier(0x100, 1, 0);
@@ -774,11 +796,11 @@
                 });
             }
         };
-        using AllTiles = std::integral_constant<int, kMT << 4 | kMT << 12>;
+        using AllTiles = std::integral_constant<int, kPT << 4 | kPT << 12>;
         if constexpr (first) {
             auto tiles = [](int i) {
                 const int dy = (i < 9 ? i : 8) / 3 - 1;
-                const int lo = kWide && dy < 0 ? 1 : 0, hi = kWide && dy > 0 ? kMT - 1 : kMT;
+                const int lo = kWide && dy < 0 ? 1 : 0, hi = kWide && dy > 0 ? kPT - 1 : kPT;
                 return lo | hi << 4 | lo << 8 | hi << 12;
             };
             static_for<nk - 1>([&](auto II) {
@@ -796,13 +818,15 @@
 #pragma unroll
             for (int n = 0; n < kNT; ++n)
 #pragma unroll
-                for (int m = ml; m < mh; ++m) {
-                    if constexpr (G::DIRECT) acc[n][m] = mfma<DT>(wq[(nk - 1) % WQ][n], last.x[m], acc[n][m]);
-                    else acc[n][m] = mfma<DT>(last.w[n], last.x[m], acc[n][m]);
-                }
+                for (int p = 0; p < kNP; ++p)
+#pragma unroll
+                    for (int m = p * kPT + ml; m < p * kPT + mh; ++m) {
+                        if constexpr (G::DIRECT) acc[n][m] = mfma<DT>(wq[(nk - 1) % WQ][n], last.x[m], acc[n][m]);
+                        else acc[n][m] = mfma<DT>(last.w[n], last.x[m], acc[n][m]);
+                    }
         } else if constexpr (kWide) {
             constexpr int KPT = C / 32;
-            static_assert(kNT == 2 && kMT == 8 && KPT % 2 == 0 && (3 * KPT) % G::KS == 0, "wide geometry");
+            static_assert(kNT == 2 && kPT == 8 && KPT % 2 == 0 && (3 * KPT) % G::KS == 0, "wide geometry");
             constexpr int NJ = 3 * KPT;
             constexpr int RS = 10 * G::RP;
             auto wstep = [&](auto JJ, auto LASTDX, const Frags<kNT, kMT>& wc, Frags<kNT, kMT>& wn, int sbn) {
@@ -813,18 +837,18 @@
                     decltype(LASTDX)::value ? wide_new_last<OAMD_EPI_NOBAR && !G::DIRECT>(Jn, NJ) : wide_new(Jn);
                 constexpr int dy = wide_dy(J), cbn = wide_cb(Jn), nnew = __builtin_popcount(newmask);
                 constexpr int mlo = dy < 0 ? 1 : 0, mhi = dy > 0 ? 7 : 8;
-                auto& Wc = [&]() -> u32x4_t(&)[9] {
+                auto& Wc = [&]() -> u32x4_t(&)[kNP][9] {
                     if constexpr (wide_cb(J) % 2 == 0) return win0; else return win1;
                 }();
-                auto& Wn = [&]() -> u32x4_t(&)[9] {
+                auto& Wn = [&]() -> u32x4_t(&)[kNP][9] {
                     if constexpr (cbn % 2 == 0) return win0; else return win1;
                 }();
                 __builtin_amdgcn_sched_barrier(0);
                 OAMD_STEP_WAIT(__builtin_amdgcn_s_waitcnt(0xC07F));
-                static_for<9>([&](auto I) {
-                    constexpr int i = decltype(I)::value;
+                static_for<9 * kNP>([&](auto I) {
+                    constexpr int p = decltype(I)::value / 9, i = decltype(I)::value % 9;
                     if constexpr ((newmask >> i) & 1)
-                        Wn[i] = *reinterpret_cast<const u32x4_t*>(act + sbn + i * RS + cbn * 64);
+                        Wn[p][i] = *reinterpret_cast<const u32x4_t*>(act + sbn + p * kPairB + i * RS + cbn * 64);
                 });
                 if constexpr (open) {
                     OAMD_OPEN_WAIT(wait_vm<G::VM_OPEN>(), __builtin_amdgcn_s_barrier());
@@ -842,12 +866,15 @@
 #pragma unroll
                 for (int n = 0; n < kNT; ++n)
 #pragma unroll
-                    for (int m = mlo; m < mhi; ++m) {
-                        if constexpr (G::DIRECT) acc[n][m] = mfma<DT>(wq[(WOFF + J) % WQ][n], Wc[m + 1 + dy], acc[n][m]);
-                        else acc[n][m] = mfma<DT>(wc.w[n], Wc[m + 1 + dy], acc[n][m]);
-                    }
-                constexpr int nds = G::DIRECT ? nnew : (open ? kNT : kNT + nnew);
-                constexpr int nm = kNT * (mhi - mlo);
+                    for (int p = 0; p < kNP; ++p)
+#pragma unroll
+                        for (int m = mlo; m < mhi; ++m) {
+                            f32x4_t& a = acc[n][p * kPT + m];
+                            if constexpr (G::DIRECT) a = mfma<DT>(wq[(WOFF + J) % WQ][n], Wc[p][m + 1 + dy], a);
+                            else a = mfma<DT>(wc.w[n], Wc[p][m + 1 + dy], a);
+                        }
+                constexpr int nds = G::DIRECT ? kNP * nnew : (open ? kNT : kNT + nnew);
+                constexpr int nm = kNP * kNT * (mhi - mlo);
                 static_for<nds>([&](auto I) {
                     constexpr int i = decltype(I)::value;
                     __builtin_amdgcn_sched_group_barrier(0x100, 1, 0);
@@ -868,10 +895,13 @@
 #pragma unroll
                     for (int n = 0; n < kNT; ++n)
 #pragma unroll
-                        for (int m = 0; m < 7; ++m) {
-                            if constexpr (G::DIRECT) acc[n][m] = mfma<DT>(wq[(WOFF + NJ - 1) % WQ][n], win1[m + 2], acc[n][m]);
-                            else acc[n][m] = mfma<DT>(fb.w[n], win1[m + 2], acc[n][m]);
-                        }
+                        for (int p = 0; p < kNP; ++p)
+#pragma unroll
+                            for (int m = 0; m < 7; ++m) {
+                                f32x4_t& a = acc[n][p * kPT + m];
+                                if constexpr (G::DIRECT) a = mfma<DT>(wq[(WOFF + NJ - 1) % WQ][n], win1[p][m + 2], a);
+                                else a = mfma<DT>(fb.w[n], win1[p][m + 2], a);
+                            }
                 }
             };
 #pragma nounroll
@@ -906,6 +936,7 @@
 #endif
         OAMD_EP_MARK(0);
         constexpr bool nobar = OAMD_EPI_NOBAR && kWide && !first && !G::DIRECT;
+        static_assert(!nobar || G::KS <= 2, "OAMD_EPI_NOBAR: at most 2 K-steps per stage");
         const int last_slot = slot;
         if constexpr (!nobar) {
             lds_barrier();
@@ -952,7 +983,10 @@
             if constexpr (kWide) {
                 if constexpr (!G::DIRECT) load_wfrags(fa, ring + slot * G::STAGE, wl);
 #pragma unroll
-                for (int i = 1; i < 8; ++i) win0[i] = *reinterpret_cast<const u32x4_t*>(act + sb0 + i * 10 * G::RP);
+                for (int p = 0; p < kNP; ++p)
+#pragma unroll
+                    for (int i = 1; i < 8; ++i)
+                        win0[p][i] = *reinterpret_cast<const u32x4_t*>(act + sb0 + p * kPairB + i * 10 * G::RP);
             } else {
                 load_frags(fa, act, ring + slot * G::STAGE, tower_kstep0_offset<C>(), rd, wl);
             }
@@ -1018,13 +1052,54 @@
     }
 }
 
+#ifndef OAMD_W4_VGPR_CAP
+#define OAMD_W4_VGPR_CAP 208
+#endif
+template <class G, int DT, int IN>
+__global__ __launch_bounds__(256) __attribute__((amdgpu_num_vgpr(OAMD_W4_VGPR_CAP))) void k_resnet_w4(
+    NetView N, const void* __restrict__ feat_in, int fw, int H, RowMap M, float* __restrict__ policy,
+    float* __restrict__ value) {
+    if (M.span && threadIdx.x == 0) atomicMax(M.span, ~(unsigned long long)__builtin_amdgcn_s_memrealtime());
+    resnet_body<G, DT, IN>(N, feat_in, fw, H, M, policy, value, blockIdx.x);
+    if (M.span) {
+        __syncthreads();
+        if (threadIdx.x == 0) atomicMax(M.span + 1, (unsigned long long)__builtin_amdgcn_s_memrealtime());
+    }
+}
+
+template <class G, int DT, int IN>
+__global__ __launch_bounds__(256) __attribute__((amdgpu_num_vgpr(OAMD_W4_VGPR_CAP))) void k_resnet_w4_loop(
+    NetView N, const void* __restrict__ feat_in, int fw, int H, RowMap M, float* __restrict__ policy,
+    float* __restrict__ value) {
+    if (M.span && threadIdx.x == 0) atomicMax(M.span, ~(unsigned long long)__builtin_amdgcn_s_memrealtime());
+    int rows = M.rows;
+    if (M.list) {
+        const int filled = *M.count - M.off;
+        rows = filled < rows ? (filled > 0 ? filled : 0) : rows;
+    }
+    for (int wg = blockIdx.x; wg * G::BOARDS < rows; wg += gridDim.x) {
+        resnet_body<G, DT, IN>(N, feat_in, fw, H, M, policy, value, wg);
+        __syncthreads();
+    }
+    if (M.span) {
+        __syncthreads();
+        if (threadIdx.x == 0) atomicMax(M.span + 1, (unsigned long long)__builtin_amdgcn_s_memrealtime());
+    }
+}
+
+template <class G, int DT, int IN, bool LOOP>
+static constexpr auto kernel_of() {
+    if constexpr (G::THREADS == 256) return LOOP ? &k_resnet_w4_loop<G, DT, IN> : &k_resnet_w4<G, DT, IN>;
+    else return LOOP ? &k_resnet_w8_loop<G, DT, IN> : &k_resnet_w8<G, DT, IN>;
+}
+
 template <class G, int DT, int IN>
 static void launch_t(const NetView& N, const void* feat, int fw, int H, const RowMap& M, float* pol, float* val,
                      hipStream_t s, int max_wgs) {
     const int rows = M.rows;
-    static_assert(G::THREADS == 512, "k_resnet_w8 geometries");
+    static_assert(G::THREADS == 512 || (G::THREADS == 256 && G::NORING), "k_resnet_w8 / k_resnet_w4 geometries");
     const unsigned grid = (unsigned)((rows + G::BOARDS - 1) / G::BOARDS);
-    constexpr auto kern = &k_resnet_w8<G, DT, IN>;
+    constexpr auto kern = kernel_of<G, DT, IN, false>();
     static bool configured = false;
     if (!configured) {
         (void)hipFuncSetAttribute(reinterpret_cast<const void*>(kern), hipFuncAttributeMaxDynamicSharedMemorySize,
@@ -1033,7 +1108,7 @@
     }
     if constexpr (IN == kPacked) {
         if (max_wgs > 0 && grid > (unsigned)max_wgs) {
-            constexpr auto lk = &k_resnet_w8_loop<G, DT, IN>;
+            constexpr auto lk = kernel_of<G, DT, IN, true>();
             static bool lconfigured = false;
             if (!lconfigured) {
                 (void)hipFuncSetAttribute(reinterpret_cast<const void*>(lk),
@@ -1048,6 +1123,13 @@
 }
 
 constexpr int kSmallBatchRows = 1024;
+
+#ifndef OAMD_C128_W4
+#define OAMD_C128_W4 1
+#endif
+static std::atomic<int> g_c128_w4{OAMD_C128_W4};
+void resnet_set_c128_four_wave(int enable) { g_c128_w4.store(enable != 0, std::memory_order_relaxed); }
+int resnet_c128_four_wave() { return g_c128_w4.load(std::memory_order_relaxed); }
 
 template <int IN>
 static void dispatch(const NetView& N, const void* feat, int fw, int H, const RowMap& M, float* pol, float* val,
@@ -1060,6 +1142,9 @@
         if (small) {
             if (fp16) launch_t<GeoS<128>, OAMD_FP16, IN>(N, feat, fw, H, M, pol, val, s, max_wgs);
             else launch_t<GeoS<128>, OAMD_BF16, IN>(N, feat, fw, H, M, pol, val, s, max_wgs);
+        } else if (resnet_c128_four_wave()) {
+            if (fp16) launch_t<GeoW4, OAMD_FP16, IN>(N, feat, fw, H, M, pol, val, s, max_wgs);
+            else launch_t<GeoW4, OAMD_BF16, IN>(N, feat, fw, H, M, pol, val, s, max_wgs);
         } else {
             if (fp16) launch_t<Geo<128>, OAMD_FP16, IN>(N, feat, fw, H, M, pol, val, s, max_wgs);
             else launch_t<Geo<128>, OAMD_BF16, IN>(N, feat, fw, H, M, pol, val, s, max_wgs);
diff --git a/othello-alphazero_amd/othello_mcts/native.py b/othello-alphazero_amd/othello_mcts/native.py
--- a/othello-alphazero_amd/othello_mcts/native.py
+++ b/othello-alphazero_amd/othello_mcts/native.py
@@ -10,7 +10,7 @@
 import numpy as np
 import torch
 
-from ._othello_mcts_impl import _Net
+from ._othello_mcts_impl import _Net, resnet_c128_four_wave, set_resnet_c128_four_wave
 from .synthetic import net_config_from_state_dict
 
 _DTYPES = {"bf16": 0, "bfloat16": 0, "fp16": 1, "float16": 1}
@@ -99,6 +99,16 @@
         return {"policy": policy, "value": value}
 
 
+def set_c128_four_wave(enable: bool) -> bool:
+    old = resnet_c128_four_wave()
+    set_resnet_c128_four_wave(bool(enable))
+    return old
+
+
+def c128_four_wave() -> bool:
+    return resnet_c128_four_wave()
+
+
 FP16_MAX = 65504.0
 FP16_HEADROOM = 16.0
 
```

Measured after the change: 5.907 million, median of 6. +1.7%, better.
